# johncai117/Meta-Fine-Tuning

Measured on AMD Instinct MI355X. Metric: episodes/sec at 5-way N-shot (ResNet10+GNN) per GPU and 1/2/4/8-GPU node, higher is better.
Workload: dtype f32

## Files before the change

include/mft_hip.h:

```cpp
#ifndef MFT_HIP_H
#define MFT_HIP_H

#ifdef __cplusplus
extern "C" {
#endif

#define MFT_EINVAL (-22)

enum { MFT_ACT_NONE = 0, MFT_ACT_RELU = 1, MFT_ACT_LRELU = 2 };
enum { MFT_BN_AFFINE_FMA = 0x100 };

int mft_version(void);
int mft_device_info(int* cu_count, int* gcn_arch_is_gfx950);

int mft_stream_create_cumask(const unsigned* mask_words, int n_words, void** stream_out);
int mft_stream_create_priority(int priority, void** stream_out, int* range_out);
int mft_stream_destroy(void* stream);
int mft_stream_probe(float* w, float* m, float* v, long long n, void* stream);
int mft_event_create(void** event_out);
int mft_event_record(void* event, void* stream);
int mft_event_elapsed_ms(void* start, void* stop, float* ms_out);
int mft_event_destroy(void* event);
int mft_probe_placement(unsigned* out, int n_blocks, int spin_cycles, void* stream);

int mft_augment_views(const unsigned char* src, int n_img, int Hs, int Ws, const float* params, int n_views, float* out,
                      long long view_stride, long long img_stride, int size, const float* mean3, const float* std3,
                      void* stream);

int mft_nchw_to_nhwc(const float* src, float* dst, int n_img, int C, int H, int W, void* stream);

long long mft_conv2d_wgrad_adam_dgrad_ws_floats(int n_img, int H, int W, int Cin);
int mft_conv2d_wgrad_adam_dgrad_nhwc(const float* x, int ldx, const float* dy, int ldy, float* w, float* m, float* v,
                                     float* dx_partials, int n_img, int H, int W, int Cin, int Cout, int imgs_per_group,
                                     long long group_stride, int step, float lr, float beta1, float beta2, float eps, void* stream);
int mft_conv2d_wgrad_adam_dgrad_nhwc_dev(const float* x, int ldx, const float* dy, int ldy, float* w, float* m, float* v,
                                         float* dx_partials, int n_img, int H, int W, int Cin, int Cout, int imgs_per_group,
                                         long long group_stride, const float* hyper, float beta1, float beta2, float eps,
                                         void* stream);
int mft_col2im_bn_backward_small(const float* dx_partials, const float* x_raw, const float* relu_out, float* dx, int n_img, int H,
                                 int W, int C, int imgs_per_group, const float* mean, const float* rstd, const float* gamma,
                                 long long gb_group_stride, float* dgamma, float* dbeta, void* stream);

int mft_ce_pool_bn_backward2(const float* feat, const int* labels, int imgs_per_group, int n_groups, int C, int hw,
                             const float* out, const float* xa, const float* xb, float* dxa, float* dxb, const float* mean_a,
                             const float* rstd_a, const float* gamma_a, const float* mean_b, const float* rstd_b,
                             const float* gamma_b, long long gb_group_stride, float* dgamma_a, float* dbeta_a, float* dgamma_b,
                             float* dbeta_b, float* loss, void* stream);

int mft_stem_cache_fill(const float* in, const float* w, int w_ld, int n_img, int H, int W, float* pmax, float* pmin,
                        float* mean_img, float* m2_img, void* stream);
int mft_pool_window_minmax(const float* x, float* ymax, float* ymin, long long n_img, int H, int W, int C, void* stream);
int mft_bn_relu_pooled_gather(const float* pmax, const float* pmin, const int* src_idx, float* y, int n_img, int OH, int OW, int C,
                              int imgs_per_group, const float* mean, const float* rstd, const float* gamma, const float* beta,
                              void* stream);

int mft_bn_apply_planes(const float* x, int ldx, float* y, int ldy, unsigned short* planes, long long plane_stride, int C,
                        int rows_per_group, int n_groups, const float* mean, const float* rstd, const float* gamma,
                        const float* beta, long long gb_group_stride, const float* res, int ldr, const float* res_mean,
                        const float* res_rstd, const float* res_gamma, const float* res_beta, int act, float slope,
                        void* stream);
int mft_bn_relu_maxpool_gather_planes(const float* x, const int* src_idx, float* y, unsigned short* planes,
                                      long long plane_stride, int n_img, int H, int W, int C, int imgs_per_group,
                                      const float* mean, const float* rstd, const float* gamma, const float* beta, void* stream);
int mft_conv2d_nhwc_x3p_bnstats(const unsigned short* in_planes, long long in_plane_elems, int ldi, const unsigned short* w3,
                                long long plane_elems, float* out, int ldo, int n_img, int H, int W, int Cin, int Cout, int KH,
                                int KW, int stride, int pad, int imgs_per_group, float eps, float* stats_ws, float* mean,
                                float* rstd, void* stream);

int mft_ingest_episode_views(const float* const* views, int n_views, int double_first, int n_way, int per_class, int n_support,
                             int C, int H, int W, float* support_store, float* all_store, void* stream);
int mft_pack_oihw(const float* w_oihw, float* w_pk, int Cout, int Cin, int KH, int KW, int k_pad, void* stream);
int mft_pack_oihw_multi(const void* jobs, int n_jobs, long long total_elements, void* stream);
int mft_unpack_oihw(const float* w_pk, float* w_oihw, int Cout, int Cin, int KH, int KW, int k_pad, void* stream);
int mft_pack_dgrad(const float* w_pk, float* wt_pk, int Cout, int Cin, int KH, int KW,
                   int groups, long long w_stride, long long wt_stride, void* stream);

int mft_conv2d_nhwc(const float* in, int ldi, const float* w, const float* bias, float* out, int ldo,
                    int n_img, int H, int W, int Cin, int Cout, int KH, int KW, int stride, int pad,
                    int imgs_per_group, long long w_group_stride, void* stream);

int mft_split_bf16x3(const float* w, unsigned short* planes, long long n, void* stream);
int mft_split_bf16x3_multi(const void* jobs, int n_jobs, long long total_elements, void* stream);
int mft_conv2d_nhwc_x3(const float* in, int ldi, const unsigned short* w3, long long plane_elems, float* out, int ldo,
                       int n_img, int H, int W, int Cin, int Cout, int KH, int KW, int stride, int pad, void* stream);
long long mft_conv2d_x3_stats_ws_floats(int n_img, int H, int W, int Cout, int KH, int KW, int stride, int pad);
int mft_conv2d_nhwc_x3_bnstats(const float* in, int ldi, const unsigned short* w3, long long plane_elems, float* out, int ldo,
                               int n_img, int H, int W, int Cin, int Cout, int KH, int KW, int stride, int pad,
                               int imgs_per_group, float eps, float* stats_ws, float* mean, float* rstd, void* stream);
int mft_conv2d_nhwc_x3_bnin_bnstats(const float* in, int ldi, const float* in_ws, const float* in_gamma, const float* in_beta,
                                    const unsigned short* w3, long long plane_elems, float* out, int ldo, int n_img, int H, int W,
                                    int Cin, int Cout, int imgs_per_group, float eps, float* stats_ws, float* mean, float* rstd,
                                    void* stream);
int mft_split_f16x2(const float* w, unsigned short* planes, long long n, void* stream);
int mft_conv2d_nhwc_h2(const float* in, int ldi, const unsigned short* w2, long long plane_elems, float* out, int ldo,
                       int n_img, int H, int W, int Cin, int Cout, int KH, int KW, int stride, int pad, void* stream);
int mft_conv2d_nhwc_h2_bnstats(const float* in, int ldi, const unsigned short* w2, long long plane_elems, float* out, int ldo,
                               int n_img, int H, int W, int Cin, int Cout, int KH, int KW, int stride, int pad,
                               int imgs_per_group, float eps, float* stats_ws, float* mean, float* rstd, void* stream);
int mft_conv2d_nhwc_h2_bnin_bnstats(const float* in, int ldi, const float* in_ws, const float* in_gamma, const float* in_beta,
                                    const unsigned short* w2, long long plane_elems, float* out, int ldo, int n_img, int H, int W,
                                    int Cin, int Cout, int imgs_per_group, float eps, float* stats_ws, float* mean, float* rstd,
                                    void* stream);
int mft_bn_apply_x3ws(const float* x, int ldx, float* y, int ldy, int C, int rows_per_group, int n_groups, const float* ws,
                      const float* gamma, const float* beta, const float* res, int ldr, const float* res_ws,
                      const float* res_gamma, const float* res_beta, int act, float slope, float eps, float* mean, float* rstd,
                      float* res_mean, float* res_rstd, void* stream);
int mft_bn_running_ema(const float* mean_a, const float* rstd_a, int rows_a, const float* mean_b, const float* rstd_b, int rows_b,
                       const int* order, int n_steps, int C, float eps, float momentum, float* running_mean, float* running_var,
                       void* stream);
int mft_bn_apply_x3ws_fits(int C, int rows_per_group, int with_res_bn);
int mft_bn_relu_pooled_gather_moments(const float* pmax, const float* pmin, const int* src_idx, float* y, int n_img, int OH, int OW,
                                      int C, int imgs_per_group, const float* mean_img, const float* m2_img, int rows_per_img,
                                      float eps, const float* gamma, const float* beta, float* mean, float* rstd, void* stream);

int mft_has_experiments(void);

int mft_conv2d_dgrad_nhwc(const float* dy, int ldy, const float* w, float* dx, int ldx,
                          int n_img, int H, int W, int Cin, int Cout, int KH, int KW, int stride, int pad,
                          int imgs_per_group, long long w_group_stride, void* stream);

long long mft_conv_ksplit_ws_floats(long long rows, int cols, int K);
long long mft_conv_ksplit_grouped_ws_floats(long long rows_per_group, int cols, int K, int groups);
int mft_conv2d_nhwc_ksplit_grouped(const float* in, int ldi, const float* w, float* out, int ldo, int n_img, int H, int W, int Cin,
                                   int Cout, int KH, int KW, int stride, int pad, int imgs_per_group, long long w_group_stride,
                                   float* ws, void* stream);
int mft_conv2d_dgrad_nhwc_ksplit_grouped(const float* dy, int ldy, const float* w, float* dx, int ldx, int n_img, int H, int W, int Cin,
                                         int Cout, int KH, int KW, int stride, int pad, int imgs_per_group, long long w_group_stride,
                                         float* ws, void* stream);
int mft_conv2d_nhwc_ksplit(const float* in, int ldi, const float* w, const float* bias, float* out, int ldo, int n_img, int H, int W,
                           int Cin, int Cout, int KH, int KW, int stride, int pad, float* ws, void* stream);
int mft_conv2d_dgrad_nhwc_ksplit(const float* dy, int ldy, const float* w, float* dx, int ldx, int n_img, int H, int W, int Cin,
                                 int Cout, int KH, int KW, int stride, int pad, float* ws, void* stream);
long long mft_conv2d_wgrad_ws_floats(int n_img, int H, int W, int Cin, int Cout, int KH, int KW, int stride, int pad,
                                     int imgs_per_group);
int mft_conv2d_wgrad_nhwc(const float* in, int ldi, const float* dy, int ldy, float* dw,
                          int n_img, int H, int W, int Cin, int Cout, int KH, int KW, int stride, int pad,
                          int imgs_per_group, long long dw_group_stride, float* ws, void* stream);

long long mft_conv2d_wgrad_oihw_ws_floats(int n_img, int H, int W, int Cin, int Cout, int KH, int KW, int stride, int pad);
int mft_conv2d_wgrad_oihw(const float* in, int ldi, const float* dy, int ldy, float* dw_oihw, int n_img, int H, int W, int Cin,
                          int Cout, int KH, int KW, int stride, int pad, int cin_valid, int cout_valid, float* ws, void* stream);

typedef struct MftWgradJob {
    const float* in; const float* dy; float* dw_oihw; float* ws;
    int ldi, ldy, n_img, H, W, Cin, Cout, KH, KW, stride, pad, cin_valid, cout_valid, reserved;
} MftWgradJob;
int mft_conv2d_wgrad_oihw_multi(const MftWgradJob* jobs, int n_jobs, void* stream);

int mft_conv2d_wgrad_adam_nhwc(const float* in, int ldi, const float* dy, int ldy, float* w, float* m, float* v,
                               float* dw_or_null, int n_img, int H, int W, int Cin, int Cout, int KH, int KW,
                               int stride, int pad, int imgs_per_group, long long group_stride,
                               int step, float lr, float beta1, float beta2, float eps, void* stream);

int mft_wgrad_adam_next_forward(const float* x, int ldx, const float* dy, int ldy, float* w, float* m, float* v,
                                float* dw_or_null, int n_img, int H, int W, int Cin, int Cout, int KH, int KW, int stride,
                                int pad, int imgs_per_group, long long group_stride, int step, const float* hyper, float lr,
                                float beta1, float beta2, float eps, const float* x_next, int mode, float* raw, float* act,
                                const float* gamma, const float* beta, long long gb_group_stride, float* mean, float* rstd,
                                const float* sc_raw, const float* gamma_s, const float* beta_s, float* mean_s, float* rstd_s,
                                float* pooled, float bn_eps, void* stream);


// ... 211 lines not shown
```

meta-fine-tuning_amd/_lib.py:

```python
import ctypes
import os

PKG = os.path.dirname(os.path.abspath(__file__))
LIB_PATH = os.path.join(PKG, "libmft_hip.so")

_P = ctypes.c_void_p
_I = ctypes.c_int
_L = ctypes.c_longlong
_F = ctypes.c_float

SIGNATURES = {
    "mft_version": [],
    "mft_device_info": [_P, _P],
    "mft_stream_create_cumask": [_P, _I, _P],
    "mft_stream_destroy": [_P],
    "mft_stream_probe": [_P, _P, _P, _L, _P],
    "mft_probe_placement": [_P, _I, _I, _P],
    "mft_event_create": [_P],
    "mft_event_record": [_P, _P],
    "mft_event_elapsed_ms": [_P, _P, _P],
    "mft_event_destroy": [_P],
    "mft_augment_views": [_P, _I, _I, _I, _P, _I, _P, _L, _L, _I, _P, _P, _P],
    "mft_nchw_to_nhwc": [_P, _P, _I, _I, _I, _I, _P],
    "mft_pack_oihw": [_P, _P, _I, _I, _I, _I, _I, _P],
# ... 14 lines not shown
    "mft_conv2d_nhwc_ksplit": [_P, _I, _P, _P, _P, _I, _I, _I, _I, _I, _I, _I, _I, _I, _I, _P, _P],
    "mft_conv2d_dgrad_nhwc_ksplit": [_P, _I, _P, _P, _I, _I, _I, _I, _I, _I, _I, _I, _I, _I, _P, _P],
    "mft_conv2d_wgrad_oihw_ws_floats": [_I, _I, _I, _I, _I, _I, _I, _I, _I],
    "mft_conv2d_wgrad_oihw": [_P, _I, _P, _I, _P, _I, _I, _I, _I, _I, _I, _I, _I, _I, _I, _I, _P, _P],
    "mft_conv2d_wgrad_oihw_multi": [_P, _I, _P],
    "mft_conv2d_wgrad_ws_floats": [_I, _I, _I, _I, _I, _I, _I, _I, _I, _I],
    "mft_conv2d_wgrad_nhwc": [_P, _I, _P, _I, _P, _I, _I, _I, _I, _I, _I, _I, _I, _I, _I, _L, _P, _P],
    "mft_conv2d_wgrad_adam_nhwc": [_P, _I, _P, _I, _P, _P, _P, _P, _I, _I, _I, _I, _I, _I, _I, _I, _I, _I, _L, _I, _F, _F, _F,
                                   _F, _P],
    "mft_pair_softmax_ut_backward": [_P, _P, _P, _P, _P, _I, _I, _I, _P, _P],
    "mft_pair_bwd_stats_ws_floats": [_L, _I],
    "mft_pair_bn_act_backward": [_P, _I, _P, _I, _P, _P, _P, _P, _P, _P, _I, _L, _I, _L, _F, _P, _P, _P, _P, _P, _P],
    "mft_pair_absdiff_ut": [_P, _I, _P, _P, _I, _I, _I, _L, _L, _P],
    "mft_pair_dx_gather": [_P, _I, _P, _I, _P, _I, _I, _I, _I, _L, _L, _P],
    "mft_pack_oihw_multi": [_P, _I, _L, _P],
    "mft_wgrad_adam_next_forward": [_P, _I, _P, _I, _P, _P, _P, _P, _I, _I, _I, _I, _I, _I, _I, _I, _I, _I, _L, _I, _P, _F, _F, _F,
                                    _F, _P, _I, _P, _P, _P, _P, _L, _P, _P, _P, _P, _P, _P, _P, _P, _F, _P],
    "mft_bn_stats_ws_floats": [_I, _I, _I],
    "mft_bn_stats": [_P, _I, _I, _I, _I, _F, _P, _P, _P, _P, _P, _F, _P, _P],
    "mft_bn_apply": [_P, _I, _P, _I, _I, _I, _I, _P, _P, _P, _P, _L, _P, _I, _P, _P, _P, _P, _I, _F, _P],
    "mft_bn_apply_multi": [_P, _I, _P],
    "mft_bn_stats_multi": [_P, _I, _P],
    "mft_bn_relu_maxpool": [_P, _P, _I, _I, _I, _I, _I, _P, _P, _P, _P, _P],
    "mft_bn_relu_maxpool_gather": [_P, _P, _P, _I, _I, _I, _I, _I, _P, _P, _P, _P, _P],
    "mft_bn_image_moments": [_P, _I, _I, _I, _L, _P, _P, _P],
    "mft_bn_combine_moments": [_P, _P, _P, _I, _I, _I, _I, _F, _P, _P, _P],
    "mft_global_avgpool": [_P, _P, _I, _I, _I, _P],
    "mft_bn_small_forward": [_P, _I, _P, _I, _P, _I, _P, _I, _I, _I, _I, _P, _P, _P, _P, _L, _P, _P, _P, _P, _I, _F, _F, _P, _I, _P],
    "mft_bn_backward2": [_P, _P, _I, _P, _I, _P, _P, _I, _I, _I, _I, _P, _P, _P, _P, _P, _P, _L, _P, _P, _P, _P, _P],
    "mft_ce_pool_backward": [_P, _P, _I, _I, _I, _I, _P, _P, _P, _P],
    "mft_bn_backward": [_P, _I, _P, _I, _P, _I, _P, _I, _I, _I, _I, _P, _P, _P, _L, _P, _P, _P],
    "mft_avgpool_relu_backward": [_P, _P, _P, _I, _I, _I, _P],
    "mft_cross_entropy": [_P, _I, _P, _I, _I, _I, _P, _P, _P],
    "mft_softmax_rows": [_P, _I, _P, _I, _I, _I, _P],
    "mft_proto_scores": [_P, _I, _I, _I, _I, _I, _I, _P, _I, _P],
    "mft_proto_backward": [_P, _I, _I, _I, _I, _I, _I, _P, _I, _P, _I, _P],
    "mft_dist_linear_forward": [_P, _I, _I, _I, _P, _P, _I, _I, _F, _P, _I, _P],
    "mft_dist_linear_backward": [_P, _I, _I, _P, _P, _I, _I, _F, _P, _I, _P, _I, _P, _P, _P],
    "mft_dist_head_sgd_run": [_P, _P, _P, _I, _I, _I, _I, _I, _I, _P, _P, _F, _F, _F, _F, _F, _P],
    "mft_dist_head_step": [_P, _I, _P, _I, _I, _I, _I, _F, _P, _P, _P, _P, _P, _P, _P, _I, _P, _I, _F, _F, _F, _F, _F, _P],
    "mft_cross_entropy_mean": [_P, _I, _P, _I, _I, _I, _P, _P, _P],
    "mft_cross_entropy_mean_backward": [_P, _I, _P, _I, _I, _I, _P, _P, _I, _P],
    "mft_adam_step": [_P, _P, _P, _P, _L, _I, _F, _F, _F, _F, _F, _P],
    "mft_sgd_step": [_P, _P, _P, _L, _I, _F, _F, _F, _F, _P],
    "mft_maml_delta": [_P, _P, _P, _L, _P],
    "mft_conv2d_wgrad_adam_dgrad_ws_floats": [_I, _I, _I, _I],
    "mft_conv2d_wgrad_adam_dgrad_nhwc": [_P, _I, _P, _I, _P, _P, _P, _P, _I, _I, _I, _I, _I, _I, _L, _I, _F, _F, _F, _F, _P],
    "mft_conv2d_wgrad_adam_dgrad_nhwc_dev": [_P, _I, _P, _I, _P, _P, _P, _P, _I, _I, _I, _I, _I, _I, _L, _P, _F, _F, _F, _P],
    "mft_col2im_bn_backward_small": [_P, _P, _P, _P, _I, _I, _I, _I, _I, _P, _P, _P, _L, _P, _P, _P],
    "mft_stream_create_priority": [_I, _P, _P],
    "mft_ce_pool_bn_backward2": [_P, _P, _I, _I, _I, _I, _P, _P, _P, _P, _P, _P, _P, _P, _P, _P, _P, _L, _P, _P, _P, _P, _P, _P],
    "mft_pool_window_minmax": [_P, _P, _P, _L, _I, _I, _I, _P],
    "mft_stem_cache_fill": [_P, _P, _I, _I, _I, _I, _P, _P, _P, _P, _P],
    "mft_conv2d_nhwc_x3_bnin_bnstats": [_P, _I, _P, _P, _P, _P, _L, _P, _I, _I, _I, _I, _I, _I, _I, _F, _P, _P, _P, _P],
    "mft_split_f16x2": [_P, _P, _L, _P],
    "mft_conv2d_nhwc_h2": [_P, _I, _P, _L, _P, _I, _I, _I, _I, _I, _I, _I, _I, _I, _I, _P],
    "mft_conv2d_nhwc_h2_bnstats": [_P, _I, _P, _L, _P, _I, _I, _I, _I, _I, _I, _I, _I, _I, _I, _I, _F, _P, _P, _P, _P],
    "mft_conv2d_nhwc_h2_bnin_bnstats": [_P, _I, _P, _P, _P, _P, _L, _P, _I, _I, _I, _I, _I, _I, _I, _F, _P, _P, _P, _P],
    "mft_bn_apply_x3ws": [_P, _I, _P, _I, _I, _I, _I, _P, _P, _P, _P, _I, _P, _P, _P, _I, _F, _F, _P, _P, _P, _P, _P],
    "mft_bn_apply_x3ws_fits": [_I, _I, _I],
    "mft_bn_running_ema": [_P, _P, _I, _P, _P, _I, _P, _I, _I, _F, _F, _P, _P, _P],
    "mft_bn_relu_pooled_gather_moments": [_P, _P, _P, _P, _I, _I, _I, _I, _I, _P, _P, _I, _F, _P, _P, _P, _P, _P],
    "mft_bn_relu_pooled_gather": [_P, _P, _P, _P, _I, _I, _I, _I, _I, _P, _P, _P, _P, _P],
    "mft_bn_apply_planes": [_P, _I, _P, _I, _P, _L, _I, _I, _I, _P, _P, _P, _P, _L, _P, _I, _P, _P, _P, _P, _I, _F, _P],
    "mft_bn_relu_maxpool_gather_planes": [_P, _P, _P, _P, _L, _I, _I, _I, _I, _I, _P, _P, _P, _P, _P],
    "mft_conv2d_nhwc_x3p_bnstats": [_P, _L, _I, _P, _L, _P, _I, _I, _I, _I, _I, _I, _I, _I, _I, _I, _I, _F, _P, _P, _P, _P],
    "mft_ingest_episode_views": [_P, _I, _I, _I, _I, _I, _I, _I, _I, _P, _P, _P],
    "mft_block_entry_small_forward": [_P, _I, _P, _L, _P, _L, _P, _P, _P, _I, _I, _I, _I, _I, _I, _I, _P, _P, _L, _P, _P, _F, _P],
    "mft_block_exit_small_forward": [_P, _P, _L, _P, _P, _P, _P, _I, _I, _I, _I, _I, _P, _P, _P, _P, _L, _P, _P, _P, _P, _F, _P],
    "mft_conv2d_dgrad_bn_backward_small": [_P, _I, _P, _P, _I, _I, _I, _I, _I, _I, _I, _I, _I, _I, _L, _P, _P, _P, _P, _P, _L,
                                           _P, _P, _P],
    "mft_linear_head_sgd_run": [_P, _P, _P, _I, _I, _I, _I, _I, _I, _P, _P, _F, _F, _F, _F, _P],
    "mft_linear_head_adam_run": [_P, _P, _P, _I, _I, _I, _I, _I, _I, _P, _P, _F, _F, _F, _F, _F, _P],
    "mft_adam_multi": [_P, _I, _I, _F, _F, _F, _F, _F, _F, _P],
    "mft_adam_hyper_advance": [_P, _P, _F, _F, _F, _P],
    "mft_adam_step_dev": [_P, _P, _P, _P, _L, _P, _F, _F, _F, _F, _P],
    "mft_conv2d_wgrad_adam_nhwc_dev": [_P, _I, _P, _I, _P, _P, _P, _P, _I, _I, _I, _I, _I, _I, _I, _I, _I, _I, _L, _P, _F, _F,
                                       _F, _P],
    "mft_linear_head_step": [_P, _I, _P, _I, _I, _I, _I, _P, _P, _P, _P, _P, _P, _P, _I, _P, _I, _F, _F, _F, _F, _F, _P],
    "mft_linear_head_scores": [_P, _I, _I, _I, _I, _I, _P, _P, _P, _P],
    "mft_pair_absdiff": [_P, _I, _P, _I, _I, _I, _I, _P],
    "mft_masked_softmax": [_P, _I, _P, _I, _I, _P],
    "mft_pair_mlp_tiles_m": [_I, _I],
    "mft_pair_mlp_layer": [_P, _I, _I, _P, _P, _P, _P, _I, _I, _P, _P, _I, _I, _I, _I, _F, _P, _P, _P, _I, _P],
    "mft_bn_forward_small": [_P, _P],
    "mft_bn_forward_small_max_rows": [],
    "mft_gemm_rk": [_P, _I, _P, _I, _I, _P, _P, _I, _I, _I, _P],
    "mft_pair_mlp_tiles_m_rk": [_I, _I],
    "mft_pair_mlp_layer_rk": [_P, _I, _I, _P, _P, _P, _P, _I, _I, _P, _P, _I, _I, _I, _I, _F, _P, _P, _P, _P],
    "mft_pair_mlp_stats_finalize_rk": [_P, _P, _P, _I, _I, _I, _P, _P, _F, _P, _P, _P, _P, _P],
    "mft_pair_mlp_stats_finalize": [_P, _P, _P, _I, _I, _I, _P, _P, _F, _P, _P, _P, _P, _P],
    "mft_pair_mlp_score": [_P, _I, _P, _P, _P, _P, _F, _P, _I, _I, _I, _P],
    "mft_masked_softmax_ut": [_P, _P, _I, _I, _P],
    "mft_graph_aggregate": [_P, _P, _I, _P, _I, _I, _I, _I, _P],
    "mft_copy_cols": [_P, _I, _P, _I, _I, _I, _I, _I, _F, _P],
    "mft_build_graph_nodes": [_P, _I, _P, _I, _I, _I, _I, _I, _I, _P],
    "mft_gather_query_scores": [_P, _I, _P, _I, _I, _I, _I, _P],
    "mft_gather_rows": [_P, _P, _P, _I, _L, _P],
    "mft_var_to_rstd": [_P, _P, _I, _F, _P],
    "mft_bn_backward_ws_floats": [_I, _I, _I],
    "mft_bn_backward_act": [_P, _I, _P, _I, _P, _I, _P, _I, _I, _I, _I, _P, _P, _P, _L, _P, _P, _I, _F, _P, _P, _P, _P, _P],
    "mft_bn_backward_act_multi": [_P, _I, _P],
    "mft_act_backward": [_P, _I, _P, _I, _P, _I, _I, _L, _I, _F, _I, _P],
    "mft_colsum": [_P, _I, _I, _L, _P, _P, _P],
    "mft_bn_relu_maxpool_arg": [_P, _P, _P, _I, _I, _I, _I, _I, _P, _P, _P, _P, _P],
    "mft_maxpool_relu_backward": [_P, _P, _P, _P, _I, _I, _I, _I, _P],
# ... 120 lines not shown
```

meta-fine-tuning_amd/csrc/bn.hip:

```cpp
#include "mft_common.h"
#include "bn_fold.h"

namespace {

constexpr int ST_ROWS = 16;

__device__ __forceinline__ void bn_stats_partial_body(const float* __restrict__ x, int ldx, int C,
                                                      int rows_per_group, int rows_per_chunk, int chunks,
                                                      float* __restrict__ ws, const int bx, const int by, const int bz) {
    const int cq = threadIdx.x & 15;
    const int rl = threadIdx.x >> 4;
    const int c = by * 64 + cq * 4;
    const int g = bz;
    const int chunk = bx;
    const long long row0 = (long long)g * rows_per_group;
    __shared__ f32x4 red1[ST_ROWS][16];
    __shared__ f32x4 red2[ST_ROWS][16];
    f32x4 s1 = {0.f, 0.f, 0.f, 0.f}, s2 = {0.f, 0.f, 0.f, 0.f};
    if (c < C) {
        const f32x4 sh = *(const f32x4*)(x + row0 * ldx + c);
        const int rbeg = chunk * rows_per_chunk;
        const int rend = min(rbeg + rows_per_chunk, rows_per_group);
#pragma unroll 4
        for (int rr = rbeg + rl; rr < rend; rr += ST_ROWS) {
// ... 159 lines not shown
                const f32x4 rga = *(const f32x4*)(p.rgamma + g * p.gbs + c);
                const f32x4 rbe = *(const f32x4*)(p.rbeta + g * p.gbs + c);
                if (folded) {
                    mft_bn_fold4(rmu, rrs, rga, rbe, sc, sh);
                    rv = mft_bn_affine4(rv, sc, sh);
                } else {
                    rv = (rv - rmu) * rrs * rga + rbe;
                }
            }
            o += rv;
        }
#pragma unroll
        for (int e = 0; e < 4; ++e) o[e] = act_f(o[e], act, p.slope);
        if (!PLANES || p.y) *(f32x4*)(p.y + row * p.ldy + c) = o;
        if constexpr (PLANES) {
            mft_u32x2 p1, p2, p3;
            mft_split4_bf16(o, p1, p2, p3);
            unsigned short* q = p.planes + row * p.C + c;
            *(mft_u32x2*)(q) = p1;
            *(mft_u32x2*)(q + p.plane_stride) = p2;
            *(mft_u32x2*)(q + 2 * p.plane_stride) = p3;
        }
    }
}

template <bool PLANES>
__global__ __launch_bounds__(256) void bn_apply_kernel(ApplyArgs p) {
    bn_apply_blocks<PLANES>(p, blockIdx.x, gridDim.x);
}

constexpr int BA_MULTI = 16;
struct ApplyMultiArgs {
    ApplyArgs job[BA_MULTI];
    int start[BA_MULTI + 1];
    int n;
};
static_assert(sizeof(ApplyMultiArgs) <= 4000, "kernarg segment");

__global__ __launch_bounds__(256) void bn_apply_multi_kernel(ApplyMultiArgs a) {
    int j = 0;
#pragma unroll 1
    while (j + 1 < a.n && (int)blockIdx.x >= a.start[j + 1]) ++j;
    const ApplyArgs p = a.job[j];
    bn_apply_blocks<false>(p, blockIdx.x - a.start[j], a.start[j + 1] - a.start[j]);
}

struct ApplyWsArgs {
    const float* x; float* y; int ldx, ldy, C, rows_per_group, n_groups, M, BM;
    const float* ws; const float* gamma; const float* beta;
    const float* res; int ldr; const float* rws; const float* rgamma; const float* rbeta;
    int act; float slope, eps;
    float* mean; float* rstd; float* rmean; float* rrstd;
    int max_tiles;
};

__global__ __launch_bounds__(256) void bn_apply_ws_kernel(ApplyWsArgs p) {
    extern __shared__ __attribute__((aligned(16))) float tab[];
    const int g = blockIdx.y, C = p.C;
    char* stage = reinterpret_cast<char*>(tab + 4 * C);
    char* rstage = stage + mft_x3_stage_bytes(p.max_tiles, C);
    mft_x3_stats_stage(p.ws, C, g, p.M, p.rows_per_group, p.BM, p.max_tiles, stage, threadIdx.x, 256);
    if (p.rws) mft_x3_stats_stage(p.rws, C, g, p.M, p.rows_per_group, p.BM, p.max_tiles, rstage, threadIdx.x, 256);
    __syncthreads();
    for (int c = threadIdx.x; c < C; c += 256) {
        float mu, rs, sc, sh;
        mft_x3_stats_staged(stage, p.max_tiles, C, c, g, p.M, p.rows_per_group, p.BM, p.eps, mu, rs);
        mft_bn_fold(mu, rs, p.gamma[c], p.beta[c], sc, sh);
        tab[c] = sc; tab[C + c] = sh;
        if (blockIdx.x == 0 && p.mean) { p.mean[(long long)g * C + c] = mu; p.rstd[(long long)g * C + c] = rs; }
        if (p.rws) {
            mft_x3_stats_staged(rstage, p.max_tiles, C, c, g, p.M, p.rows_per_group, p.BM, p.eps, mu, rs);
            mft_bn_fold(mu, rs, p.rgamma[c], p.rbeta[c], sc, sh);
            tab[2 * C + c] = sc; tab[3 * C + c] = sh;
            if (blockIdx.x == 0 && p.rmean) { p.rmean[(long long)g * C + c] = mu; p.rrstd[(long long)g * C + c] = rs; }
        }
    }
    __syncthreads();
    const int cq = C >> 2;
    const int total = p.rows_per_group * cq;
    const long long row0 = (long long)g * p.rows_per_group;
    for (int i = blockIdx.x * 256 + threadIdx.x; i < total; i += gridDim.x * 256) {
        const int rr = i / cq;
        const int c = (i - rr * cq) * 4;
        const long long row = row0 + rr;
        const f32x4 v = *(const f32x4*)(p.x + row * p.ldx + c);
        f32x4 o = mft_bn_affine4(v, *(const f32x4*)(tab + c), *(const f32x4*)(tab + C + c));
        if (p.res) {
            f32x4 rv = *(const f32x4*)(p.res + row * p.ldr + c);
            if (p.rws) rv = mft_bn_affine4(rv, *(const f32x4*)(tab + 2 * C + c), *(const f32x4*)(tab + 3 * C + c));
            o += rv;
        }
#pragma unroll
        for (int e = 0; e < 4; ++e) o[e] = act_f(o[e], p.act, p.slope);
        *(f32x4*)(p.y + row * p.ldy + c) = o;
    }
}

template <bool PLANES>
__global__ __launch_bounds__(256) void bn_relu_maxpool_kernel(const float* __restrict__ x, float* __restrict__ y,
                                                              int n_img, int H, int W, int C, int OH, int OW,
                                                              int imgs_per_group, const float* __restrict__ mean,
                                                              const float* __restrict__ rstd,
                                                              const float* __restrict__ gamma,
                                                              const float* __restrict__ beta,
                                                              const int* __restrict__ src_idx,
                                                              unsigned short* __restrict__ planes, long long plane_stride) {
    const int cq = C >> 2;
    const long long total = (long long)n_img * OH * OW * cq;
    for (long long i = (long long)blockIdx.x * blockDim.x + threadIdx.x; i < total;
         i += (long long)gridDim.x * blockDim.x) {
        const int c = (int)(i % cq) * 4;
        long long t = i / cq;
        const int ow = (int)(t % OW); t /= OW;
        const int oh = (int)(t % OH);
        const int n = (int)(t / OH);
        const int g = n / imgs_per_group;
        const long long ns = src_idx ? (long long)src_idx[n] : (long long)n;
        const f32x4 mu = *(const f32x4*)(mean + (long long)g * C + c);
        const f32x4 rs = *(const f32x4*)(rstd + (long long)g * C + c);
        const f32x4 ga = *(const f32x4*)(gamma + c);
        const f32x4 be = *(const f32x4*)(beta + c);
        f32x4 best = {-3.4e38f, -3.4e38f, -3.4e38f, -3.4e38f};
#pragma unroll
        for (int dh = 0; dh < 3; ++dh) {
            const int ih = oh * 2 - 1 + dh;
            if (ih < 0 || ih >= H) continue;
#pragma unroll
            for (int dw = 0; dw < 3; ++dw) {
                const int iw = ow * 2 - 1 + dw;
                if (iw < 0 || iw >= W) continue;
                const f32x4 v = *(const f32x4*)(x + ((ns * H + ih) * W + iw) * C + c);
                const f32x4 o = __builtin_elementwise_fma((v - mu) * rs, ga, be);
#pragma unroll
                for (int e = 0; e < 4; ++e) best[e] = fmaxf(best[e], o[e]);
            }
        }
#pragma unroll
        for (int e = 0; e < 4; ++e) best[e] = fmaxf(best[e], 0.f);
        *(f32x4*)(y + i * 4) = best;
        if constexpr (PLANES) {
// ... 100 lines not shown
        f32x4 d = *(const f32x4*)(p.dy + (row0 + rr) * p.lddy + c);
        if (p.ro) {
            const f32x4 o = *(const f32x4*)(p.ro + (row0 + rr) * p.ldro + c);
#pragma unroll
            for (int e = 0; e < 4; ++e) d[e] = o[e] > 0.f ? d[e] : 0.f;
        }
        const f32x4 xh = (*(const f32x4*)(p.x + (row0 + rr) * p.ldx + c) - mu) * rs;
        *(f32x4*)(p.dx + (row0 + rr) * p.lddx + c) = k * (d - m1 - xh * m2);
    }
}

__global__ __launch_bounds__(256) void bn_image_moments_kernel(const float* __restrict__ x, int ldx, int C, int rows,
                                                               float* __restrict__ mean_img,
                                                               float* __restrict__ m2_img) {
    const int cq = threadIdx.x & 15;
    const int rl = threadIdx.x >> 4;
    const int c = blockIdx.y * 64 + cq * 4;
    const long long img = blockIdx.x;
    const long long row0 = img * rows;
    __shared__ f32x4 red1[ST_ROWS][16];
    __shared__ f32x4 red2[ST_ROWS][16];
    f32x4 s1 = {0.f, 0.f, 0.f, 0.f}, s2 = {0.f, 0.f, 0.f, 0.f}, sh = s1;
    if (c < C) {
        sh = *(const f32x4*)(x + row0 * ldx + c);
        for (int rr = rl; rr < rows; rr += ST_ROWS) {
            f32x4 v = *(const f32x4*)(x + (row0 + rr) * ldx + c);
            v -= sh;
            s1 += v;
            s2 += v * v;
        }
    }
    red1[rl][cq] = s1;
    red2[rl][cq] = s2;
    __syncthreads();
    if (rl == 0 && c < C) {
#pragma unroll
        for (int k = 1; k < ST_ROWS; ++k) {
            s1 += red1[k][cq];
            s2 += red2[k][cq];
        }
        const float inv = 1.f / (float)rows;
        f32x4 mu, m2;
#pragma unroll
        for (int e = 0; e < 4; ++e) {
            const float d = s1[e] * inv;
            mu[e] = sh[e] + d;
            m2[e] = fmaxf(s2[e] - s1[e] * d, 0.f);
        }
        *(f32x4*)(mean_img + img * C + c) = mu;
        *(f32x4*)(m2_img + img * C + c) = m2;
    }
}

template <class MeanOf, class M2Of>
__device__ __forceinline__ void combine_moments_impl(MeanOf mean_of, M2Of m2_of, int rows_per_img, int imgs_per_group, float eps,
                                                     float& mean, float& rstd) {
    float mu = 0.f;
    for (int i = 0; i < imgs_per_group; ++i) mu += mean_of(i);
    mu /= (float)imgs_per_group;
    float m2 = 0.f, dev = 0.f;
    for (int i = 0; i < imgs_per_group; ++i) {
        const float d = mean_of(i) - mu;
        m2 += m2_of(i);
        dev += d * d;
    }
    const float var = (m2 + (float)rows_per_img * dev) / ((float)rows_per_img * (float)imgs_per_group);
    mean = mu;
    rstd = 1.0f / sqrtf(var + eps);
}

__device__ __forceinline__ void combine_moments(const float* __restrict__ mean_img, const float* __restrict__ m2_img,
                                                const int* __restrict__ id, int C, int c, int rows_per_img, int imgs_per_group,
                                                float eps, float& mean, float& rstd) {
    combine_moments_impl([&](int i) { return mean_img[(long long)id[i] * C + c]; },
                         [&](int i) { return m2_img[(long long)id[i] * C + c]; }, rows_per_img, imgs_per_group, eps, mean, rstd);
}

__device__ __forceinline__ void combine_moments_lds(const float* smean, const float* sm2, int C, int c, int rows_per_img,
                                                    int imgs_per_group, float eps, float& mean, float& rstd) {
    combine_moments_impl([&](int i) { return smean[i * C + c]; }, [&](int i) { return sm2[i * C + c]; }, rows_per_img,
                         imgs_per_group, eps, mean, rstd);
}

__global__ void bn_combine_moments_kernel(const float* __restrict__ mean_img, const float* __restrict__ m2_img,
                                          const int* __restrict__ idx, int C, int rows_per_img, int imgs_per_group,
                                          float eps, float* __restrict__ mean, float* __restrict__ rstd) {
    const int c = blockIdx.x * blockDim.x + threadIdx.x;
    const int g = blockIdx.y;
    if (c >= C) return;
    float mu, rs;
    combine_moments(mean_img, m2_img, idx + (long long)g * imgs_per_group, C, c, rows_per_img, imgs_per_group, eps, mu, rs);
    mean[(long long)g * C + c] = mu;
    rstd[(long long)g * C + c] = rs;
}

inline int grid_for(long long total, int block = 256, int cap = 256 * 8) {
    long long b = (total + block - 1) / block;
    if (b < 1) b = 1;
    if (b > cap) b = cap;
    return (int)b;
}

inline int stats_chunks(int rows_per_group, int n_groups, int C) {
    const int tiles = (C + 63) / 64;
    long long want = (1024 + (long long)n_groups * tiles - 1) / ((long long)n_groups * tiles);
    int maxc = (rows_per_group + 63) / 64;
    if (want > maxc) want = maxc;
    if (want < 1) want = 1;
    return (int)want;
}

struct BnFwdSmallArgs {
    const float* x; float* y; const float* gamma; const float* beta; float* mean; float* rstd;
    float* running_mean; float* running_var; long long* nbt;
    const float* res; const float* rgamma; const float* rbeta; float* rmean; float* rrstd;
    float* rrunning_mean; float* rrunning_var; long long* rnbt;
    int ldx, ldy, ldr, C, rows_per_group, n_groups, act;
    float eps, momentum, slope;
    int y_scalar;
};

__device__ __forceinline__ void bn_small_block_sum(f32x4& a, f32x4& b, float (*red)[8]) {
    const int lane = threadIdx.x & 63, wave = threadIdx.x >> 6;
#pragma unroll
    for (int off = 32; off > 0; off >>= 1)
#pragma unroll
        for (int e = 0; e < 4; ++e) {
            a[e] += __shfl_xor(a[e], off, 64);
            b[e] += __shfl_xor(b[e], off, 64);
        }
    if (lane == 0) {
#pragma unroll
        for (int e = 0; e < 4; ++e) { red[wave][e] = a[e]; red[wave][4 + e] = b[e]; }
    }
// ... 168 lines not shown

extern "C" int mft_bn_apply(const float* x, int ldx, float* y, int ldy, int C, int rows_per_group, int n_groups,
                            const float* mean, const float* rstd, const float* gamma, const float* beta,
                            long long gb_group_stride, const float* res, int ldr, const float* res_mean,
                            const float* res_rstd, const float* res_gamma, const float* res_beta, int act, float slope,
                            void* stream) {
    if (C % 4 != 0 || ldx % 4 != 0 || ldy % 4 != 0 || (res && ldr % 4 != 0)) return MFT_EINVAL;
    ApplyArgs p{x, y, ldx, ldy, C, rows_per_group, n_groups, mean, rstd, gamma, beta, gb_group_stride,
                res, ldr, res_mean, res_rstd, res_gamma, res_beta, act, slope, nullptr, 0};
    const long long total = (long long)n_groups * rows_per_group * (C / 4);
    hipLaunchKernelGGL(bn_apply_kernel<false>, dim3(grid_for(total)), dim3(256), 0, (hipStream_t)stream, p);
    return mft_launch_status();
}

extern "C" int mft_bn_apply_multi(const MftBnApplyJob* jobs, int n_jobs, void* stream) {
    if (jobs == nullptr || n_jobs < 1) return MFT_EINVAL;
    for (int j0 = 0; j0 < n_jobs;) {
        ApplyMultiArgs a = {};
        int cnt = 0, blocks = 0;
        for (; j0 < n_jobs && cnt < BA_MULTI; ++j0, ++cnt) {
            const MftBnApplyJob& jb = jobs[j0];
            if (jb.C % 4 != 0 || jb.ldx % 4 != 0 || jb.ldy % 4 != 0 || jb.rows_per_group < 1 || jb.n_groups < 1) return MFT_EINVAL;
            a.job[cnt] = ApplyArgs{jb.x, jb.y, jb.ldx, jb.ldy, jb.C, jb.rows_per_group, jb.n_groups, jb.mean, jb.rstd, jb.gamma, jb.beta, 0,
                                   nullptr, 0, nullptr, nullptr, nullptr, nullptr, jb.act, jb.slope, nullptr, 0};
            a.start[cnt] = blocks;
            blocks += grid_for((long long)jb.n_groups * jb.rows_per_group * (jb.C / 4));
        }
        a.start[cnt] = blocks;
        a.n = cnt;
        hipLaunchKernelGGL(bn_apply_multi_kernel, dim3(blocks), dim3(256), 0, (hipStream_t)stream, a);
    }
    return mft_launch_status();
}

extern "C" int mft_bn_apply_x3ws(const float* x, int ldx, float* y, int ldy, int C, int rows_per_group, int n_groups, const float* ws,
                                 const float* gamma, const float* beta, const float* res, int ldr, const float* res_ws,
                                 const float* res_gamma, const float* res_beta, int act, float slope, float eps, float* mean,
                                 float* rstd, float* res_mean, float* res_rstd, void* stream) {
    if (C % 4 != 0 || C > 1024 || ldx % 4 != 0 || ldy % 4 != 0 || (res && ldr % 4 != 0) || !ws || !y || rows_per_group < 128 ||
        n_groups <= 0 || (res_ws && (!res || !res_gamma || !res_beta)) || (mean == nullptr) != (rstd == nullptr) ||
        (res_mean == nullptr) != (res_rstd == nullptr))
        return MFT_EINVAL;
    const long long M = (long long)n_groups * rows_per_group;
    const long long per_group = (long long)rows_per_group * (C / 4);
    if (M > 0x7fffffffLL) return MFT_EINVAL;
    const int max_tiles = mft_x3_max_group_tiles(rows_per_group, 128);
    const size_t lds = (size_t)4 * C * sizeof(float) + (res_ws ? 2 : 1) * mft_x3_stage_bytes_host(max_tiles, C);
    if (lds > 64 * 1024) return MFT_EINVAL;
    int sub = (int)((per_group + 256 * 16 - 1) / (256 * 16));
    const int cap = (2048 + n_groups - 1) / n_groups;
    if (sub > cap) sub = cap;
    if (sub < 1) sub = 1;
    ApplyWsArgs p{x, y, ldx, ldy, C, rows_per_group, n_groups, (int)M, 128, ws, gamma, beta, res, ldr, res_ws, res_gamma, res_beta,
                  act, slope, eps, mean, rstd, res_mean, res_rstd, max_tiles};
    hipLaunchKernelGGL(bn_apply_ws_kernel, dim3(sub, n_groups), dim3(256), lds, (hipStream_t)stream, p);
    return mft_launch_status();
}

namespace {
__global__ void bn_running_ema_kernel(const float* __restrict__ mean_a, const float* __restrict__ rstd_a, float unb_a,
                                      const float* __restrict__ mean_b, const float* __restrict__ rstd_b, float unb_b,
                                      const int* __restrict__ order, int n_steps, int C, float eps, float momentum,
                                      float* __restrict__ running_mean, float* __restrict__ running_var) {
    const int c = blockIdx.x * blockDim.x + threadIdx.x;
    if (c >= C) return;
    float rm = running_mean[c], rv = running_var[c];
    for (int t = 0; t < n_steps; ++t) {
        const int o = order[t], g = o & 0xffffff;
        const bool b = (o >> 24) != 0;
        const float m = (b ? mean_b : mean_a)[(long long)g * C + c];
        const float rs = (b ? rstd_b : rstd_a)[(long long)g * C + c];
        const float var = fmaxf(1.0f / (rs * rs) - eps, 0.f);
        rm = (1.f - momentum) * rm + momentum * m;
        rv = (1.f - momentum) * rv + momentum * (var * (b ? unb_b : unb_a));
    }
    running_mean[c] = rm;
    running_var[c] = rv;
}
}

extern "C" int mft_bn_running_ema(const float* mean_a, const float* rstd_a, int rows_a, const float* mean_b, const float* rstd_b,
                                  int rows_b, const int* order, int n_steps, int C, float eps, float momentum, float* running_mean,
                                  float* running_var, void* stream) {
    if (!mean_a || !rstd_a || rows_a < 1 || !order || n_steps < 1 || C < 1 || !running_mean || !running_var) return MFT_EINVAL;
    const float ua = (float)rows_a / (float)(rows_a > 1 ? rows_a - 1 : 1);
    const float ub = (float)rows_b / (float)(rows_b > 1 ? rows_b - 1 : 1);
    hipLaunchKernelGGL(bn_running_ema_kernel, dim3((C + 63) / 64), dim3(64), 0, (hipStream_t)stream, mean_a, rstd_a, ua, mean_b, rstd_b, ub,
                       order, n_steps, C, eps, momentum, running_mean, running_var);
    return mft_launch_status();
}

extern "C" int mft_bn_apply_x3ws_fits(int C, int rows_per_group, int with_res_bn) {
    if (C % 4 != 0 || C > 1024 || rows_per_group < 128) return 0;
    return (size_t)4 * C * sizeof(float) + (with_res_bn ? 2 : 1) * mft_x3_stage_bytes_host(mft_x3_max_group_tiles(rows_per_group, 128), C) <=
           64 * 1024;
}

extern "C" int mft_bn_apply_planes(const float* x, int ldx, float* y, int ldy, unsigned short* planes, long long plane_stride,
                                   int C, int rows_per_group, int n_groups, const float* mean, const float* rstd,
                                   const float* gamma, const float* beta, long long gb_group_stride, const float* res, int ldr,
                                   const float* res_mean, const float* res_rstd, const float* res_gamma,
                                   const float* res_beta, int act, float slope, void* stream) {
    if (C % 4 != 0 || ldx % 4 != 0 || (y && ldy % 4 != 0) || (res && ldr % 4 != 0) || !planes) return MFT_EINVAL;
    if (plane_stride < (long long)n_groups * rows_per_group * C) return MFT_EINVAL;
    ApplyArgs p{x, y, ldx, ldy, C, rows_per_group, n_groups, mean, rstd, gamma, beta, gb_group_stride,
                res, ldr, res_mean, res_rstd, res_gamma, res_beta, act, slope, planes, plane_stride};
    const long long total = (long long)n_groups * rows_per_group * (C / 4);
    hipLaunchKernelGGL(bn_apply_kernel<true>, dim3(grid_for(total)), dim3(256), 0, (hipStream_t)stream, p);
    return mft_launch_status();
}

namespace {
__global__ __launch_bounds__(256) void pool_window_minmax_kernel(const float* __restrict__ x, float* __restrict__ ymax,
                                                                 float* __restrict__ ymin, long long n_img, int H, int W, int C,
                                                                 int OH, int OW) {
    const int cq = C >> 2;
    const long long total = n_img * OH * OW * cq;
    for (long long i = (long long)blockIdx.x * blockDim.x + threadIdx.x; i < total; i += (long long)gridDim.x * blockDim.x) {
        const int c = (int)(i % cq) * 4;
        long long t = i / cq;
        const int ow = (int)(t % OW); t /= OW;
        const int oh = (int)(t % OH);
        const long long n = t / OH;
        f32x4 hi = {-3.4e38f, -3.4e38f, -3.4e38f, -3.4e38f}, lo = {3.4e38f, 3.4e38f, 3.4e38f, 3.4e38f};
#pragma unroll
        for (int dh = 0; dh < 3; ++dh) {
            const int ih = oh * 2 - 1 + dh;
            if (ih < 0 || ih >= H) continue;
#pragma unroll
            for (int dw = 0; dw < 3; ++dw) {
                const int iw = ow * 2 - 1 + dw;
                if (iw < 0 || iw >= W) continue;
                const f32x4 v = *(const f32x4*)(x + ((n * H + ih) * W + iw) * C + c);
#pragma unroll
                for (int e = 0; e < 4; ++e) { hi[e] = fmaxf(hi[e], v[e]); lo[e] = fminf(lo[e], v[e]); }
            }
        }
        *(f32x4*)(ymax + i * 4) = hi;
        *(f32x4*)(ymin + i * 4) = lo;
    }
}

__device__ __forceinline__ f32x4 pooled_bn_relu(const float* __restrict__ pmax, const float* __restrict__ pmin, long long src,
                                                const f32x4 mu, const f32x4 rs, const f32x4 ga, const f32x4 be) {
    const bool all_pos = ga[0] >= 0.f && ga[1] >= 0.f && ga[2] >= 0.f && ga[3] >= 0.f;
    const bool all_neg = ga[0] < 0.f && ga[1] < 0.f && ga[2] < 0.f && ga[3] < 0.f;
    f32x4 v;
    if (all_pos) v = *(const f32x4*)(pmax + src);
    else if (all_neg) v = *(const f32x4*)(pmin + src);
    else {
        const f32x4 a = *(const f32x4*)(pmax + src), b = *(const f32x4*)(pmin + src);
#pragma unroll
        for (int e = 0; e < 4; ++e) v[e] = ga[e] >= 0.f ? a[e] : b[e];
    }
    f32x4 o = __builtin_elementwise_fma((v - mu) * rs, ga, be);
#pragma unroll
    for (int e = 0; e < 4; ++e) o[e] = fmaxf(o[e], 0.f);
    return o;
}

__global__ __launch_bounds__(256) void bn_relu_pooled_gather_kernel(const float* __restrict__ pmax, const float* __restrict__ pmin,
                                                                    const int* __restrict__ src_idx, float* __restrict__ y,
                                                                    int n_img, int HW, int C, int imgs_per_group,
                                                                    const float* __restrict__ mean, const float* __restrict__ rstd,
                                                                    const float* __restrict__ gamma, const float* __restrict__ beta) {
    const int cq = C >> 2;
    const long long total = (long long)n_img * HW * cq;
    for (long long i = (long long)blockIdx.x * blockDim.x + threadIdx.x; i < total; i += (long long)gridDim.x * blockDim.x) {
        const int c = (int)(i % cq) * 4;
        const long long t = i / cq;
        const int pix = (int)(t % HW);
        const int n = (int)(t / HW);
        const int g = n / imgs_per_group;
        const long long src = ((long long)src_idx[n] * HW + pix) * C + c;
        const f32x4 mu = *(const f32x4*)(mean + (long long)g * C + c);
        const f32x4 rs = *(const f32x4*)(rstd + (long long)g * C + c);
        *(f32x4*)(y + i * 4) = pooled_bn_relu(pmax, pmin, src, mu, rs, *(const f32x4*)(gamma + c), *(const f32x4*)(beta + c));
    }
}

__global__ __launch_bounds__(256) void bn_relu_pooled_gather_moments_kernel(
    const float* __restrict__ pmax, const float* __restrict__ pmin, const int* __restrict__ src_idx, float* __restrict__ y, int HW,
    int C, int imgs_per_group, const float* __restrict__ mean_img, const float* __restrict__ m2_img, int rows_per_img, float eps,
    const float* __restrict__ gamma, const float* __restrict__ beta, float* __restrict__ mean, float* __restrict__ rstd) {
    extern __shared__ __attribute__((aligned(16))) float tab[];
    const int g = blockIdx.y;
    const int* id = src_idx + (long long)g * imgs_per_group;
    float* smean = tab + 2 * C;
    float* sm2 = smean + imgs_per_group * C;
    for (int i = threadIdx.x; i < imgs_per_group * C; i += 256) {
        const int im = i / C, c = i - im * C;
        const long long src = (long long)id[im] * C + c;
        smean[i] = mean_img[src];
        sm2[i] = m2_img[src];
    }
    __syncthreads();
    for (int c = threadIdx.x; c < C; c += 256) {
        float mu, rs;
        combine_moments_lds(smean, sm2, C, c, rows_per_img, imgs_per_group, eps, mu, rs);
        tab[c] = mu; tab[C + c] = rs;
        if (blockIdx.x == 0 && mean) { mean[(long long)g * C + c] = mu; rstd[(long long)g * C + c] = rs; }
    }
    __syncthreads();
    const int cq = C >> 2;
    const int total = imgs_per_group * HW * cq;
    for (int i = blockIdx.x * 256 + threadIdx.x; i < total; i += gridDim.x * 256) {
        const int c = (i % cq) * 4;
        const int t = i / cq;
        const int pix = t % HW;
        const int n = t / HW;
        const long long src = ((long long)id[n] * HW + pix) * C + c;
        const long long dst = ((long long)g * imgs_per_group * HW * cq + i) * 4;
        *(f32x4*)(y + dst) = pooled_bn_relu(pmax, pmin, src, *(const f32x4*)(tab + c), *(const f32x4*)(tab + C + c),
                                            *(const f32x4*)(gamma + c), *(const f32x4*)(beta + c));
    }
}
}

extern "C" int mft_pool_window_minmax(const float* x, float* ymax, float* ymin, long long n_img, int H, int W, int C, void* stream) {
    if (C % 4 != 0 || n_img <= 0) return MFT_EINVAL;
    const int OH = (H + 2 - 3) / 2 + 1, OW = (W + 2 - 3) / 2 + 1;
    const long long total = n_img * OH * OW * (C / 4);
    hipLaunchKernelGGL(pool_window_minmax_kernel, dim3(grid_for(total, 256, 256 * 16)), dim3(256), 0, (hipStream_t)stream, x, ymax,
                       ymin, n_img, H, W, C, OH, OW);
    return mft_launch_status();
}

extern "C" int mft_bn_relu_pooled_gather(const float* pmax, const float* pmin, const int* src_idx, float* y, int n_img, int OH,
                                         int OW, int C, int imgs_per_group, const float* mean, const float* rstd,
                                         const float* gamma, const float* beta, void* stream) {
    if (C % 4 != 0 || !src_idx) return MFT_EINVAL;
    if (imgs_per_group <= 0) imgs_per_group = n_img;
    const long long total = (long long)n_img * OH * OW * (C / 4);
    hipLaunchKernelGGL(bn_relu_pooled_gather_kernel, dim3(grid_for(total, 256, 256 * 16)), dim3(256), 0, (hipStream_t)stream, pmax,
                       pmin, src_idx, y, n_img, OH * OW, C, imgs_per_group, mean, rstd, gamma, beta);
    return mft_launch_status();
}

extern "C" int mft_bn_relu_pooled_gather_moments(const float* pmax, const float* pmin, const int* src_idx, float* y, int n_img,
                                                 int OH, int OW, int C, int imgs_per_group, const float* mean_img,
                                                 const float* m2_img, int rows_per_img, float eps, const float* gamma,
                                                 const float* beta, float* mean, float* rstd, void* stream) {
    if (C % 4 != 0 || C > 1024 || !src_idx || imgs_per_group <= 0 || n_img % imgs_per_group != 0 || rows_per_img <= 0 ||
        (mean == nullptr) != (rstd == nullptr))
        return MFT_EINVAL;
    const int groups = n_img / imgs_per_group;
    const long long per_group = (long long)imgs_per_group * OH * OW * (C / 4);
    if (per_group > 0x7fffffffLL) return MFT_EINVAL;
    int sub = (int)((per_group + 256 * 16 - 1) / (256 * 16));
    const int cap = (2048 + groups - 1) / groups;
    if (sub > cap) sub = cap;
    if (sub < 1) sub = 1;
    const size_t lds = (size_t)(2 + 2 * imgs_per_group) * C * sizeof(float);
    if (lds > 64 * 1024) return MFT_EINVAL;
    hipLaunchKernelGGL(bn_relu_pooled_gather_moments_kernel, dim3(sub, groups), dim3(256), lds, (hipStream_t)stream,
                       pmax, pmin, src_idx, y, OH * OW, C, imgs_per_group, mean_img, m2_img, rows_per_img, eps, gamma, beta, mean,
                       rstd);
    return mft_launch_status();
}

extern "C" int mft_bn_relu_maxpool_gather_planes(const float* x, const int* src_idx, float* y, unsigned short* planes,
                                                 long long plane_stride, int n_img, int H, int W, int C, int imgs_per_group,
                                                 const float* mean, const float* rstd, const float* gamma, const float* beta,
                                                 void* stream) {
    if (C % 4 != 0) return MFT_EINVAL;
    if (imgs_per_group <= 0) imgs_per_group = n_img;
    const int OH = (H + 2 - 3) / 2 + 1, OW = (W + 2 - 3) / 2 + 1;
    const long long total = (long long)n_img * OH * OW * (C / 4);
    if (planes)
        hipLaunchKernelGGL(bn_relu_maxpool_kernel<true>, dim3(grid_for(total, 256, 256 * 16)), dim3(256), 0, (hipStream_t)stream,
                           x, y, n_img, H, W, C, OH, OW, imgs_per_group, mean, rstd, gamma, beta, src_idx, planes, plane_stride);
    else
        hipLaunchKernelGGL(bn_relu_maxpool_kernel<false>, dim3(grid_for(total, 256, 256 * 16)), dim3(256), 0, (hipStream_t)stream,
                           x, y, n_img, H, W, C, OH, OW, imgs_per_group, mean, rstd, gamma, beta, src_idx, planes, plane_stride);
    return mft_launch_status();
}

// ... 352 lines not shown
```

meta-fine-tuning_amd/csrc/bn_fold.h:

```cpp
#pragma once
#include "mft_common.h"

typedef float mft_f32x2 __attribute__((ext_vector_type(2)));

struct MftTileSpan { int t0, t1; };
struct MftTileW { float inv_nt, w1, w2, pad; };

__device__ __forceinline__ MftTileSpan mft_x3_group_tiles(int g, int M, int R, int BM) {
    const int r0 = g * R, r1 = min(r0 + R, M);
    return {r0 / BM, (r1 - 1) / BM};
}

__device__ __forceinline__ int mft_x3_tile_seg(int t, int g, int R, int BM) { return ((t * BM) / R == g) ? 0 : 1; }

__device__ __forceinline__ MftTileW mft_x3_tile_weights(int t, int g, int M, int R, int BM) {
    const int r0 = g * R, r1 = min(r0 + R, M);
    const int lo = max(t * BM, r0), hi = min(t * BM + BM, r1);
    const float nt = (float)(hi - lo), n = (float)(lo - r0), tot = (float)(hi - r0);
    return {1.0f / nt, nt / tot, n * nt / tot, 0.f};
}

template <class Get, class Weights>
__device__ __forceinline__ void mft_x3_stats_chain(Get get, Weights weights, int g, int M, int R, int BM, float eps, float& mean,
                                                   float& rstd) {
// ... 13 lines not shown
    rstd = 1.0f / sqrtf(m2 / (float)(r1 - r0) + eps);
}

__device__ __forceinline__ void mft_x3_stats_merge(const float* __restrict__ ws, int C, int c, int g, int M, int R, int BM,
                                                   float eps, float& mean, float& rstd) {
    mft_x3_stats_chain([&](int t, int seg) { return *(const mft_f32x2*)(ws + (((long long)t * 2 + seg) * C + c) * 2); },
                       [&](int t) { return mft_x3_tile_weights(t, g, M, R, BM); }, g, M, R, BM, eps, mean, rstd);
}

__device__ __forceinline__ size_t mft_x3_stage_bytes(int max_tiles, int C) {
    return (size_t)max_tiles * (sizeof(MftTileW) + (size_t)C * sizeof(mft_f32x2));
}

__device__ __forceinline__ void mft_x3_stats_stage(const float* __restrict__ ws, int C, int g, int M, int R, int BM, int max_tiles,
                                                   void* stage, int tid, int nthreads) {
    MftTileW* wt = reinterpret_cast<MftTileW*>(stage);
    mft_f32x2* part = reinterpret_cast<mft_f32x2*>(wt + max_tiles);
    const MftTileSpan sp = mft_x3_group_tiles(g, M, R, BM);
    const int nt = sp.t1 - sp.t0 + 1;
    for (int i = tid; i < nt; i += nthreads) wt[i] = mft_x3_tile_weights(sp.t0 + i, g, M, R, BM);
    const int total = nt * C;
    for (int i = tid; i < total; i += nthreads) {
        const int tt = i / C, c = i - tt * C, t = sp.t0 + tt;
        part[i] = *(const mft_f32x2*)(ws + (((long long)t * 2 + mft_x3_tile_seg(t, g, R, BM)) * C + c) * 2);
    }
}

__device__ __forceinline__ void mft_x3_stats_staged(const void* stage, int max_tiles, int C, int c, int g, int M, int R, int BM,
                                                    float eps, float& mean, float& rstd) {
    const MftTileW* wt = reinterpret_cast<const MftTileW*>(stage);
    const mft_f32x2* part = reinterpret_cast<const mft_f32x2*>(wt + max_tiles);
    const int t0 = mft_x3_group_tiles(g, M, R, BM).t0;
    mft_x3_stats_chain([&](int t, int) { return part[(t - t0) * C + c]; }, [&](int t) { return wt[t - t0]; }, g, M, R, BM, eps, mean,
                       rstd);
}

inline int mft_x3_max_group_tiles(int R, int BM) { return (R + BM - 1) / BM + 1; }
inline size_t mft_x3_stage_bytes_host(int max_tiles, int C) { return (size_t)max_tiles * (16 + (size_t)C * 8); }

__device__ __forceinline__ void mft_bn_fold(float mean, float rstd, float gamma, float beta, float& scale, float& shift) {
    scale = rstd * gamma;
    shift = __builtin_fmaf(-mean, scale, beta);
}

__device__ __forceinline__ f32x4 mft_bn_affine4(const f32x4 v, const f32x4 scale, const f32x4 shift) {
    return __builtin_elementwise_fma(v, scale, shift);
}

__device__ __forceinline__ void mft_bn_fold4(const f32x4 mean, const f32x4 rstd, const f32x4 gamma, const f32x4 beta, f32x4& scale,
                                             f32x4& shift) {
    scale = rstd * gamma;
    shift = __builtin_elementwise_fma(-mean, scale, beta);
}
```

meta-fine-tuning_amd/csrc/conv_x3.hip:

```cpp
#include "mft_common.h"
#include "bn_fold.h"

namespace {

typedef __bf16 bf16x8 __attribute__((ext_vector_type(8)));
typedef __bf16 bf16x2 __attribute__((ext_vector_type(2)));
typedef _Float16 f16x8 __attribute__((ext_vector_type(8)));
typedef _Float16 f16x4 __attribute__((ext_vector_type(4)));
typedef float f32x2 __attribute__((ext_vector_type(2)));
typedef unsigned u32x2 __attribute__((ext_vector_type(2)));
typedef unsigned u32x4 __attribute__((ext_vector_type(4)));

struct X3Args {
    const float* in;
    const unsigned short* w3;
    long long plane;
    float* out;
    int ldi, ldo;
    int H, W, Cin, OH, OW, Cout, KH, KW, stride, pad;
    int Kpad;
    int M;
    int tiles_n;
    unsigned in_bytes, w_bytes;
    int xcd_swizzle;
    int row_swz;
    const unsigned short* in3;
    unsigned in_plane_bytes;
    float* stats_ws;
    int rows_per_group;
    int s1_rows;
    const float* bn_ws; const float* bn_gamma; const float* bn_beta;
    float bn_eps;
    int bn_max_tiles;
};

constexpr int X3_RS = 40;

__device__ __forceinline__ unsigned pk_bf16(float a, float b) {
    f32x2 v = {a, b};
    return __builtin_bit_cast(unsigned, __builtin_convertvector(v, bf16x2));
}

__device__ __forceinline__ void split4(const f32x4 x, u32x2& p1, u32x2& p2, u32x2& p3) {
    f32x4 r;
    p1[0] = pk_bf16(x[0], x[1]);
    p1[1] = pk_bf16(x[2], x[3]);
    r[0] = x[0] - __builtin_bit_cast(float, p1[0] << 16);
    r[1] = x[1] - __builtin_bit_cast(float, p1[0] & 0xffff0000u);
    r[2] = x[2] - __builtin_bit_cast(float, p1[1] << 16);
    r[3] = x[3] - __builtin_bit_cast(float, p1[1] & 0xffff0000u);
    p2[0] = pk_bf16(r[0], r[1]);
    p2[1] = pk_bf16(r[2], r[3]);
    r[0] -= __builtin_bit_cast(float, p2[0] << 16);
    r[1] -= __builtin_bit_cast(float, p2[0] & 0xffff0000u);
    r[2] -= __builtin_bit_cast(float, p2[1] << 16);
    r[3] -= __builtin_bit_cast(float, p2[1] & 0xffff0000u);
    p3[0] = pk_bf16(r[0], r[1]);
    p3[1] = pk_bf16(r[2], r[3]);
}

__device__ __forceinline__ void split4_h2(const f32x4 x, u32x2& p1, u32x2& p2) {
    const f16x4 hi = __builtin_convertvector(x, f16x4);
    const f32x4 r = (x - __builtin_convertvector(hi, f32x4)) * 2048.f;
    const f16x4 lo = __builtin_convertvector(r, f16x4);
    p1 = __builtin_bit_cast(u32x2, hi);
    p2 = __builtin_bit_cast(u32x2, lo);
}
constexpr float X3_H2_LO_SCALE = 1.0f / 2048.f;

template <int BM, int BN, bool AP, bool DB, int HOIST = 0, int DBG = 0, bool XS = false, int NP = 3>
__global__ __launch_bounds__(256) __attribute__((amdgpu_waves_per_eu(NP == 2 ? 3 : 1))) void conv_x3_kernel(X3Args p) {
    static_assert(NP == 3 || (NP == 2 && !AP && !DB && HOIST == 0 && DBG == 0 && !XS), "f16x2: the plain single-buffer form only");
    constexpr int NACC = NP == 3 ? 1 : 2;
    constexpr int TM = BM / 64;
    constexpr int TN = BN / 64;
    constexpr int PA = AP ? BM / 64 : BM / 32;
    constexpr int PB = BN / 64;
    constexpr int RS = XS ? 32 : X3_RS;
    constexpr int A_PLANE = BM * RS;
    constexpr int B_PLANE = BN * RS;
    auto lo = [](int row, int c) -> int {
        if constexpr (XS) return row * 32 + ((((c >> 3) ^ (row >> 2)) & 3) << 3) + (c & 7);
        else return row * X3_RS + c;
    };
    extern __shared__ __attribute__((aligned(16))) unsigned short smem[];
    unsigned short* As = smem;
// ... 295 lines not shown
#pragma unroll
            for (int e = 0; e < 16; ++e) {
                const int row = (e & 3) + 8 * (e >> 2) + 4 * h;
                const int m = m0 + wm * (BM / 2) + i * 32 + row;
                if (m < p.M) p.out[(long long)m * p.ldo + n] = val(i, j, e);
            }
        }
    if (p.stats_ws != nullptr) {
        static_assert(TN == 1 || TN == 2, "stats epilogue");
        const int split = (m0 / p.rows_per_group + 1) * p.rows_per_group;
        float* sred = reinterpret_cast<float*>(smem);
        __syncthreads();
#pragma unroll
        for (int j = 0; j < TN; ++j) {
            float a1 = 0.f, a2 = 0.f, b1 = 0.f, b2 = 0.f;
#pragma unroll
            for (int i = 0; i < TM; ++i)
#pragma unroll
                for (int e = 0; e < 16; ++e) {
                    const int m = m0 + wm * (BM / 2) + i * 32 + (e & 3) + 8 * (e >> 2) + 4 * h;
                    const float v = val(i, j, e);
                    if (m < p.M) {
                        if (m < split) { a1 += v; a2 += v * v; }
                        else { b1 += v; b2 += v * v; }
                    }
                }
            a1 += __shfl_xor(a1, 32, 64); a2 += __shfl_xor(a2, 32, 64);
            b1 += __shfl_xor(b1, 32, 64); b2 += __shfl_xor(b2, 32, 64);
            if (h == 0) {
                float* o = sred + ((((wm * 2 + wn) * TN + j) * 32 + r) << 2);
                o[0] = a1; o[1] = a2; o[2] = b1; o[3] = b2;
            }
        }
        __syncthreads();
        if (wm == 0 && h == 0) {
#pragma unroll
            for (int j = 0; j < TN; ++j) {
                const float* o0 = sred + ((((0 * 2 + wn) * TN + j) * 32 + r) << 2);
                const float* o1 = sred + ((((1 * 2 + wn) * TN + j) * 32 + r) << 2);
                const int n = n0 + wn * (BN / 2) + j * 32 + r;
                float* w0 = p.stats_ws + (((long long)mt * 2 + 0) * p.Cout + n) * 2;
                float* w1 = p.stats_ws + (((long long)mt * 2 + 1) * p.Cout + n) * 2;
                w0[0] = o0[0] + o1[0]; w0[1] = o0[1] + o1[1];
                w1[0] = o0[2] + o1[2]; w1[1] = o0[3] + o1[3];
            }
        }
    }
}

#ifdef MFT_EXPERIMENTS
#include "../../tools/experiments/conv_x3_pingpong.inc"
#endif

template <int BM, int BN, bool BNIN, int NP = 3, bool BDB = true>
__device__ __forceinline__ void conv_x3_s1_body(const X3Args& p) {
    static_assert(NP == 3 || NP == 2, "3 bf16 pieces (six products) or 2 fp16 pieces (three products)");
    constexpr int NACC = NP == 3 ? 1 : 2;
    constexpr int TM = BM / 64, TN = BN / 64;
    constexpr int PA = BM / 32, PB = BN / 64;
    constexpr int RS = X3_RS;
    constexpr int B_PLANE = BN * RS;
    const int A_PLANE = p.s1_rows * RS;
    extern __shared__ __attribute__((aligned(16))) unsigned short smem[];
    constexpr int NBB = (NP == 2 && BDB) ? 2 : 1;
    unsigned short* As = smem;
    unsigned short* Bs = smem + NP * A_PLANE;
    float* bn_tab = reinterpret_cast<float*>(Bs + NBB * NP * B_PLANE);

    const int tid = threadIdx.x;
    const int lane = tid & 63, wave = tid >> 6;
    const int wm = wave >> 1, wn = wave & 1;
    const int r = lane & 31, h = lane >> 5;
    int tile_id = blockIdx.x;
    if (p.xcd_swizzle) {
        const int nwg = gridDim.x, q = nwg >> 3, rmd = nwg & 7;
        const int xcd = tile_id & 7, slot = tile_id >> 3;
        tile_id = xcd * q + (xcd < rmd ? xcd : rmd) + slot;
    }
    const int nt = tile_id % p.tiles_n;
    const int mt = tile_id / p.tiles_n;
    const int m0 = mt * BM, n0 = nt * BN;
    const int W = p.W, H = p.H;
    const int fr0 = m0 / W;
    const int g0 = BNIN ? m0 / p.rows_per_group : 0;
    const bool bn_two = BNIN && (m0 + (BM < p.M - m0 ? BM : p.M - m0) - 1) / p.rows_per_group > g0;
    if constexpr (BNIN) {
        char* stage = reinterpret_cast<char*>(smem);
        const size_t gstride = mft_x3_stage_bytes(p.bn_max_tiles, p.Cin);
        const bool two = bn_two;
        mft_x3_stats_stage(p.bn_ws, p.Cin, g0, p.M, p.rows_per_group, BM, p.bn_max_tiles, stage, tid, 256);
        if (two) mft_x3_stats_stage(p.bn_ws, p.Cin, g0 + 1, p.M, p.rows_per_group, BM, p.bn_max_tiles, stage + gstride, tid, 256);
        __syncthreads();
        for (int i = tid; i < 2 * p.Cin; i += 256) {
            const int gi = i >= p.Cin ? 1 : 0, c = i - gi * p.Cin;
            if (gi == 0 || two) {
                float mu, rs, sc, sh;
                mft_x3_stats_staged(stage + gi * gstride, p.bn_max_tiles, p.Cin, c, g0 + gi, p.M, p.rows_per_group, BM, p.bn_eps, mu, rs);
                mft_bn_fold(mu, rs, p.bn_gamma[c], p.bn_beta[c], sc, sh);
                bn_tab[(gi * 2 + 0) * p.Cin + c] = sc;
                bn_tab[(gi * 2 + 1) * p.Cin + c] = sh;
            }
        }
        __syncthreads();
    }
    const int g_id = tid >> 5, g_rr = (tid >> 3) & 3;
    const int lrow = p.row_swz ? g_rr * 4 + (g_id & 3) + 16 * (g_id >> 2) : tid >> 3;
    const int c4 = (tid & 7) * 4;
    const __amdgpu_buffer_rsrc_t rA = __builtin_amdgcn_make_buffer_rsrc((void*)p.in, 0, p.in_bytes, 0x00020000);
    const __amdgpu_buffer_rsrc_t rB = __builtin_amdgcn_make_buffer_rsrc((void*)p.w3, 0, p.w_bytes, 0x00020000);
    int a_off[PA], a_oh[PA], a_lds[PA], a_tab[PA];
    bool a_ok[PA];
#pragma unroll
    for (int j = 0; j < PA; ++j) {
        const int t = lrow + 32 * j, m = m0 + t;
        const int fr = m / W;
        a_ok[j] = m < p.M;
        a_oh[j] = fr - (fr / H) * H;
        a_off[j] = ((a_ok[j] ? m : 0) * p.ldi + c4) * 4;
        a_lds[j] = (t + 1) * RS + c4;
        a_tab[j] = BNIN ? ((a_ok[j] ? m / p.rows_per_group - g0 : 0) * 2 * p.Cin + c4) : 0;
    }
    const int hside = (tid >> 3) & 1;
    const int mh = hside ? m0 + BM : m0 - 1;
    const int frh = (mh > 0 ? mh : 0) / W;
    const bool h_ok = tid < 16 && (hside ? (mh < p.M && mh - frh * W != 0) : (m0 > 0 && m0 - fr0 * W != 0));
    const int h_oh = frh - (frh / H) * H;
    const int h_off = ((h_ok ? mh : 0) * p.ldi + c4) * 4;
    const int h_lds = (hside ? BM + 1 : 0) * RS + c4;
    const int h_tab = BNIN ? (((hside && h_ok) ? (m0 + BM - 1) / p.rows_per_group - g0 : 0) * 2 * p.Cin + c4) : 0;

    const int bseg = tid & 3;
    const int brow = p.row_swz ? ((tid >> 2) & 3) * 4 + ((tid >> 4) & 3) + 16 * (tid >> 6) : tid >> 2;
    int b_off[PB];
#pragma unroll
    for (int j = 0; j < PB; ++j) b_off[j] = ((n0 + brow + 64 * j) * p.Kpad + bseg * 8) * 2;
    const int plane_bytes = (int)(p.plane * 2);

    int fa[TM], fl[TM], fr_[TM];
    constexpr int Z0 = BM + 2;
#pragma unroll
    for (int i = 0; i < TM; ++i) {
        const int t = wm * (BM / 2) + i * 32 + r;
        const int ow = (m0 + t) - ((m0 + t) / W) * W;
        fa[i] = (t + 1) * RS;
        fl[i] = ow == 0 ? (Z0 + ((t - Z0) & 15)) * RS : fa[i] - RS;
        fr_[i] = ow == W - 1 ? (Z0 + ((t + 2 - Z0) & 15)) * RS : fa[i] + RS;
    }

    f32x16 acc[NACC][TM][TN];
#pragma unroll
    for (int q = 0; q < NACC; ++q)
#pragma unroll
        for (int i = 0; i < TM; ++i)
#pragma unroll
            for (int j = 0; j < TN; ++j)
#pragma unroll
                for (int e = 0; e < 16; ++e) acc[q][i][j][e] = 0.f;
    auto val = [&](int i, int j, int e) -> float {
        if constexpr (NP == 3) return acc[0][i][j][e];
        else return __builtin_fmaf(acc[1][i][j][e], X3_H2_LO_SCALE, acc[0][i][j][e]);
    };

    struct Stage {
        f32x4 ra[PA];
        f32x4 rh;
        u32x4 rb[PB][NP];
    };
    Stage st;
    const int n_ci = p.Cin / 32;
    const int n_ms = 3 * n_ci;
    auto load_a = [&](int ms, Stage& S) {
        const int kh = ms / n_ci, ci0 = (ms - kh * n_ci) * 32;
        const int shift = ((kh - 1) * W * p.ldi + ci0) * 4;
#pragma unroll
        for (int j = 0; j < PA; ++j) {
            const bool ok = a_ok[j] && (unsigned)(a_oh[j] + kh - 1) < (unsigned)H;
            S.ra[j] = __builtin_bit_cast(f32x4, __builtin_amdgcn_raw_buffer_load_b128(rA, ok ? (unsigned)(a_off[j] + shift) : 0x80000000u, 0, 0));
        }
        const bool okh = h_ok && (unsigned)(h_oh + kh - 1) < (unsigned)H;
        S.rh = __builtin_bit_cast(f32x4, __builtin_amdgcn_raw_buffer_load_b128(rA, okh ? (unsigned)(h_off + shift) : 0x80000000u, 0, 0));
    };
    auto load_b = [&](int ms, int kw, Stage& S) {
        const int kh = ms / n_ci, ci0 = (ms - kh * n_ci) * 32;
        const int k0 = (kh * 3 + kw) * p.Cin + ci0;
#pragma unroll
        for (int j = 0; j < PB; ++j)
#pragma unroll
            for (int pl = 0; pl < NP; ++pl)
                S.rb[j][pl] = __builtin_amdgcn_raw_buffer_load_b128(rB, b_off[j] + pl * plane_bytes, k0 * 2, 0);
    };
    auto put_a = [&](const f32x4 v, int off) {
        if constexpr (NP == 3) {
            u32x2 p1, p2, p3;
            split4(v, p1, p2, p3);
            *(u32x2*)(As + off) = p1;
            *(u32x2*)(As + A_PLANE + off) = p2;
            *(u32x2*)(As + 2 * A_PLANE + off) = p3;
        } else {
            u32x2 p1, p2;
            split4_h2(v, p1, p2);
            *(u32x2*)(As + off) = p1;
            *(u32x2*)(As + A_PLANE + off) = p2;
        }
    };
    auto bn_relu = [&](const f32x4 v, const f32x4 sc, const f32x4 sh, bool ok) {
        f32x4 o = mft_bn_affine4(v, sc, sh);
#pragma unroll
        for (int e = 0; e < 4; ++e) o[e] = ok ? fmaxf(o[e], 0.f) : 0.f;
        return o;
    };
    auto store_a = [&](const Stage& S, int ms) {
        if constexpr (BNIN) {
            const int kh = ms / n_ci, ci0 = (ms - kh * n_ci) * 32;
            const bool okh = h_ok && (unsigned)(h_oh + kh - 1) < (unsigned)H;
            if (!bn_two) {
                const f32x4 sc = *(const f32x4*)(bn_tab + ci0 + c4), sh = *(const f32x4*)(bn_tab + p.Cin + ci0 + c4);
#pragma unroll
                for (int j = 0; j < PA; ++j)
                    put_a(bn_relu(S.ra[j], sc, sh, a_ok[j] && (unsigned)(a_oh[j] + kh - 1) < (unsigned)H), a_lds[j]);
                if (tid < 16) put_a(bn_relu(S.rh, sc, sh, okh), h_lds);
            } else {
#pragma unroll
                for (int j = 0; j < PA; ++j)
                    put_a(bn_relu(S.ra[j], *(const f32x4*)(bn_tab + a_tab[j] + ci0), *(const f32x4*)(bn_tab + a_tab[j] + p.Cin + ci0),
                                  a_ok[j] && (unsigned)(a_oh[j] + kh - 1) < (unsigned)H), a_lds[j]);
                if (tid < 16)
                    put_a(bn_relu(S.rh, *(const f32x4*)(bn_tab + h_tab + ci0), *(const f32x4*)(bn_tab + h_tab + p.Cin + ci0), okh), h_lds);
            }
        } else {
#pragma unroll
            for (int j = 0; j < PA; ++j) put_a(S.ra[j], a_lds[j]);
            if (tid < 16) put_a(S.rh, h_lds);
        }
    };
    auto store_b = [&](const Stage& S, int bb = 0) {
#pragma unroll
        for (int j = 0; j < PB; ++j)
#pragma unroll
            for (int pl = 0; pl < NP; ++pl)
                *(u32x4*)(Bs + (bb * NP + pl) * B_PLANE + (brow + 64 * j) * RS + bseg * 8) = S.rb[j][pl];
    };
    auto compute = [&](int kw, int bb = 0) {
        const unsigned short* const Bc = Bs + bb * NP * B_PLANE;
#pragma unroll
        for (int kk = 0; kk < 2; ++kk) {
            if constexpr (NP == 3) {
                bf16x8 a[TM][3], b[TN][3];
#pragma unroll
                for (int i = 0; i < TM; ++i)
#pragma unroll
                    for (int pl = 0; pl < 3; ++pl)
                        a[i][pl] = *(const bf16x8*)(As + pl * A_PLANE + (kw == 0 ? fl[i] : (kw == 1 ? fa[i] : fr_[i])) + kk * 16 + h * 8);
#pragma unroll
                for (int j = 0; j < TN; ++j)
#pragma unroll
                    for (int pl = 0; pl < 3; ++pl)
                        b[j][pl] = *(const bf16x8*)(Bc + pl * B_PLANE + (wn * (BN / 2) + j * 32 + r) * RS + kk * 16 + h * 8);
                constexpr int TA[6] = {2, 0, 1, 1, 0, 0};
                constexpr int TB[6] = {0, 2, 1, 0, 1, 0};
#pragma unroll
                for (int t = 0; t < 6; ++t)
#pragma unroll
                    for (int i = 0; i < TM; ++i)
#pragma unroll
                        for (int j = 0; j < TN; ++j)
// ... 89 lines not shown
        }
    if (p.stats_ws != nullptr) {
        static_assert(TN == 1 || TN == 2, "stats epilogue");
        const int split = (m0 / p.rows_per_group + 1) * p.rows_per_group;
        float* sred = reinterpret_cast<float*>(smem);
        __syncthreads();
#pragma unroll
        for (int j = 0; j < TN; ++j) {
            float a1 = 0.f, a2 = 0.f, b1 = 0.f, b2 = 0.f;
#pragma unroll
            for (int i = 0; i < TM; ++i)
#pragma unroll
                for (int e = 0; e < 16; ++e) {
                    const int m = m0 + wm * (BM / 2) + i * 32 + (e & 3) + 8 * (e >> 2) + 4 * h;
                    const float v = val(i, j, e);
                    if (m < p.M) {
                        if (m < split) { a1 += v; a2 += v * v; }
                        else { b1 += v; b2 += v * v; }
                    }
                }
            a1 += __shfl_xor(a1, 32, 64); a2 += __shfl_xor(a2, 32, 64);
            b1 += __shfl_xor(b1, 32, 64); b2 += __shfl_xor(b2, 32, 64);
            if (h == 0) {
                float* o = sred + ((((wm * 2 + wn) * TN + j) * 32 + r) << 2);
                o[0] = a1; o[1] = a2; o[2] = b1; o[3] = b2;
            }
        }
        __syncthreads();
        if (wm == 0 && h == 0) {
#pragma unroll
            for (int j = 0; j < TN; ++j) {
                const float* o0 = sred + ((((0 * 2 + wn) * TN + j) * 32 + r) << 2);
                const float* o1 = sred + ((((1 * 2 + wn) * TN + j) * 32 + r) << 2);
                const int n = n0 + wn * (BN / 2) + j * 32 + r;
                float* w0 = p.stats_ws + (((long long)mt * 2 + 0) * p.Cout + n) * 2;
                float* w1 = p.stats_ws + (((long long)mt * 2 + 1) * p.Cout + n) * 2;
                w0[0] = o0[0] + o1[0]; w0[1] = o0[1] + o1[1];
                w1[0] = o0[2] + o1[2]; w1[1] = o0[3] + o1[3];
            }
        }
    }
}

template <int BM, int BN, int NP = 3, bool BDB = true>
__global__ __launch_bounds__(256) __attribute__((amdgpu_waves_per_eu(NP == 2 ? 3 : 1))) void conv_x3_s1_kernel(X3Args p) {
    conv_x3_s1_body<BM, BN, false, NP, BDB>(p);
}

template <int BM, int BN, int NP = 3, bool BDB = true>
__global__ __launch_bounds__(256) __attribute__((amdgpu_waves_per_eu(3, 3))) void conv_x3_s1_bnin_kernel(X3Args p) {
    conv_x3_s1_body<BM, BN, true, NP, BDB>(p);
}

__global__ void x3_stats_finalize_kernel(const float* __restrict__ ws, int C, int M, int R, int BM, float eps,
                                         float* __restrict__ mean, float* __restrict__ rstd) {
    const int c = blockIdx.x * blockDim.x + threadIdx.x;
    const int g = blockIdx.y;
    if (c >= C) return;
    float mu, rs;
    mft_x3_stats_merge(ws, C, c, g, M, R, BM, eps, mu, rs);
    mean[(long long)g * C + c] = mu;
    rstd[(long long)g * C + c] = rs;
}

__global__ __launch_bounds__(256) void split_bf16x3_kernel(const float* __restrict__ w, unsigned short* __restrict__ out,
                                                           long long n) {
    for (long long i = (long long)blockIdx.x * blockDim.x + threadIdx.x; i < n; i += (long long)gridDim.x * blockDim.x) {
        const float x = w[i];
        const unsigned q1 = pk_bf16(x, 0.f) & 0xffffu;
        const float r1 = x - __builtin_bit_cast(float, q1 << 16);
        const unsigned q2 = pk_bf16(r1, 0.f) & 0xffffu;
        const float r2 = r1 - __builtin_bit_cast(float, q2 << 16);
        const unsigned q3 = pk_bf16(r2, 0.f) & 0xffffu;
        out[i] = (unsigned short)q1;
        out[n + i] = (unsigned short)q2;
        out[2 * n + i] = (unsigned short)q3;
    }
}

struct SplitJob { const float* src; unsigned short* dst; long long n, Cout, Cin, taps, transposed, start; };

__global__ __launch_bounds__(256) void split_bf16x3_multi_kernel(const SplitJob* __restrict__ jobs, int n_jobs, long long total) {
    for (long long i = (long long)blockIdx.x * blockDim.x + threadIdx.x; i < total; i += (long long)gridDim.x * blockDim.x) {
        int lo = 0, hi = n_jobs - 1;
        while (lo < hi) {
            const int mid = (lo + hi + 1) >> 1;
            if (jobs[mid].start <= i) lo = mid; else hi = mid - 1;
        }
        const SplitJob j = jobs[lo];
        const long long l = i - j.start;
        long long src = l;
        if (j.transposed) {
            const long long co = l % j.Cout, t = l / j.Cout;
            const long long tp = t % j.taps, ci = t / j.taps;
            src = (co * j.taps + (j.taps - 1 - tp)) * j.Cin + ci;
        }
        const float x = j.src[src];
        const unsigned q1 = pk_bf16(x, 0.f) & 0xffffu;
        const float r1 = x - __builtin_bit_cast(float, q1 << 16);
        const unsigned q2 = pk_bf16(r1, 0.f) & 0xffffu;
        const float r2 = r1 - __builtin_bit_cast(float, q2 << 16);
        const unsigned q3 = pk_bf16(r2, 0.f) & 0xffffu;
        j.dst[l] = (unsigned short)q1;
        j.dst[j.n + l] = (unsigned short)q2;
        j.dst[2 * j.n + l] = (unsigned short)q3;
    }
// ... 137 lines not shown
int g_x3_patch = 0;
int g_x3_tile = 0;

}

extern "C" int mft_split_bf16x3(const float* w, unsigned short* planes, long long n, void* stream) {
    if (n <= 0) return MFT_EINVAL;
    long long blocks = (n + 255) / 256;
    if (blocks > 4096) blocks = 4096;
    hipLaunchKernelGGL(split_bf16x3_kernel, dim3((unsigned)blocks), dim3(256), 0, (hipStream_t)stream, w, planes, n);
    return mft_launch_status();
}

extern "C" int mft_split_bf16x3_multi(const void* jobs, int n_jobs, long long total_elements, void* stream) {
    if (n_jobs < 1 || total_elements < 1) return MFT_EINVAL;
    long long blocks = (total_elements + 255) / 256;
    if (blocks > 4096) blocks = 4096;
    hipLaunchKernelGGL(split_bf16x3_multi_kernel, dim3((unsigned)blocks), dim3(256), 0, (hipStream_t)stream, (const SplitJob*)jobs, n_jobs,
                       total_elements);
    return mft_launch_status();
}

extern "C" int mft_debug_set_x3_tile(int t) {
#ifndef MFT_EXPERIMENTS
    const bool off = (t == 10 || t == 60 || t == 70 || t == 80 || t == 100 || t == 200);
    if (!off && ((t >= 10 && t < 20) || t == 42 || (t >= 60 && t < 90) || t >= 100)) return MFT_EINVAL;
#endif
    if (t >= 200) g_x3_dbg = t - 200;
    else if (t >= 100) g_x3_min_lds_kb = t - 100;
    else if (t >= 90) g_x3_s1 = t - 90;
    else if (t >= 80) g_x3_hoist = t - 80;
    else if (t >= 70) g_x3_pp = t - 70;
    else if (t >= 60) g_x3_db = t - 60;
    else if (t >= 40) g_x3_row_swz = t - 40;
    else if (t >= 30) g_x3_bdb = t - 30;
    else if (t >= 20) g_x3_xcd = t - 20;
    else if (t >= 10) g_x3_patch = t - 10;
    else g_x3_tile = t;
    return 0;
}

static int x3_dispatch(const float* in, int ldi, const unsigned short* w3, long long plane_elems, float* out, int ldo,
                       int n_img, int H, int W, int Cin, int Cout, int KH, int KW, int stride, int pad, float* stats_ws,
                       int rows_per_group, void* stream, const unsigned short* in3 = nullptr, long long in_plane_elems = 0,
                       const float* bn_ws = nullptr, const float* bn_gamma = nullptr, const float* bn_beta = nullptr,
                       float bn_eps = 0.f, int np = 3) {
    if (n_img <= 0 || Cin % 32 != 0 || Cout % 64 != 0 || ldi % 4 != 0 || (np != 3 && np != 2)) return MFT_EINVAL;
    if (np == 2 && (in3 != nullptr || g_x3_tile > 1 || g_x3_db || g_x3_pp || g_x3_dbg || g_x3_hoist || g_x3_row_swz == 2 || g_x3_min_lds_kb ||
                    g_x3_patch))
        return MFT_EINVAL;
    X3Args p;
    p.bn_ws = bn_ws; p.bn_gamma = bn_gamma; p.bn_beta = bn_beta; p.bn_eps = bn_eps;
    p.bn_max_tiles = bn_ws ? mft_x3_max_group_tiles(rows_per_group, 128) : 0;
    if (bn_ws != nullptr && (in3 != nullptr || !bn_gamma || !bn_beta || rows_per_group < 128 || KH != 3 || KW != 3 || stride != 1 ||
                             pad != 1 || x3_s1_lds(128, 64, W, Cin, np) > X3_S1_LDS_3PER_CU ||
                             2 * mft_x3_stage_bytes_host(p.bn_max_tiles, Cin) >
                                 (size_t)np * (128 + 18) * X3_RS * sizeof(unsigned short)))
        return MFT_EINVAL;
    p.in3 = in3;
    p.in_plane_bytes = 0;
    p.stats_ws = stats_ws;
    p.rows_per_group = rows_per_group;
    p.in = in; p.w3 = w3; p.plane = plane_elems; p.out = out; p.ldi = ldi; p.ldo = ldo;
    p.H = H; p.W = W; p.Cin = Cin; p.Cout = Cout; p.KH = KH; p.KW = KW; p.stride = stride; p.pad = pad;
    p.OH = (H + 2 * pad - KH) / stride + 1;
    p.OW = (W + 2 * pad - KW) / stride + 1;
    p.Kpad = KH * KW * Cin;
    const long long M = (long long)n_img * p.OH * p.OW;
    if (M > 0x7fffffffLL) return MFT_EINVAL;
    p.M = (int)M;
    p.tiles_n = 0;
    hipStream_t s = (hipStream_t)stream;
    int G = 0, R = 0;
    double eff = 0.0;
    if (in3 != nullptr) {
        const long long need = (long long)n_img * H * W * ldi;
        if (ldi % 8 != 0 || in_plane_elems < need || 3 * in_plane_elems * 2 >= 0x7fff0000LL || 3 * plane_elems * 2 >= 0x7fff0000LL)
            return MFT_EINVAL;
        if (stats_ws != nullptr && rows_per_group < 128) return MFT_EINVAL;
        p.in_plane_bytes = (unsigned)(in_plane_elems * 2);
        p.in_bytes = 0;
        p.w_bytes = (unsigned)(3 * plane_elems * 2);
        return launch_x3<128, 64, true, false>(p, (hipStream_t)stream);
    }
#ifdef MFT_EXPERIMENTS
    if (stats_ws == nullptr && g_x3_patch && KH == 3 && KW == 3 && stride == 1 && pad == 1 && ldi == Cin && ldo == Cout &&
        patch_geometry(H, W, &G, &R, &eff) && (g_x3_patch >= 2 || eff >= 0.9)) {
        P3Args q;
        q.in = in; q.w3 = w3; q.plane = plane_elems; q.out = out;
        q.n_img = n_img; q.H = H; q.W = W; q.Cin = Cin; q.Cout = Cout; q.G = G; q.R = R;
        q.row_blocks = (H + R - 1) / R;
        q.tiles_n = Cout / 64;
        const int img_groups = (n_img + G - 1) / G;
        const size_t lds = (size_t)3 * G * (R + 2) * (W + 2) * X3_RS * sizeof(unsigned short);
        static MftPerDeviceOnce attr_once;
        if (attr_once.need()) {
            hipError_t e = hipFuncSetAttribute((const void*)conv3x3_patch_x3_kernel, hipFuncAttributeMaxDynamicSharedMemorySize,
                                               64 * 1024);
            if (e != hipSuccess) return (int)e;
            attr_once.mark();
        }
        if (lds <= 64 * 1024) {
            hipLaunchKernelGGL(conv3x3_patch_x3_kernel, dim3((unsigned)(img_groups * q.row_blocks * q.tiles_n)), dim3(256), lds, s, q);
            return mft_launch_status();
        }
    }
// ... 75 lines not shown
    hipLaunchKernelGGL(x3_stats_finalize_kernel, dim3((Cout + 63) / 64, groups), dim3(64), 0, (hipStream_t)stream,
                       (const float*)stats_ws, Cout, n_img * OH * OW, R, g_x3_tile == 3 ? 64 : 128, eps, mean, rstd);
    return mft_launch_status();
}

extern "C" int mft_conv2d_nhwc_x3_bnstats(const float* in, int ldi, const unsigned short* w3, long long plane_elems,
                                          float* out, int ldo, int n_img, int H, int W, int Cin, int Cout, int KH, int KW,
                                          int stride, int pad, int imgs_per_group, float eps, float* stats_ws,
                                          float* mean, float* rstd, void* stream) {
    return x3_bnstats(3, in, ldi, w3, plane_elems, out, ldo, n_img, H, W, Cin, Cout, KH, KW, stride, pad, imgs_per_group, eps, stats_ws, mean,
                      rstd, stream);
}

extern "C" int mft_conv2d_nhwc_h2_bnstats(const float* in, int ldi, const unsigned short* w2, long long plane_elems,
                                          float* out, int ldo, int n_img, int H, int W, int Cin, int Cout, int KH, int KW,
                                          int stride, int pad, int imgs_per_group, float eps, float* stats_ws,
                                          float* mean, float* rstd, void* stream) {
    return x3_bnstats(2, in, ldi, w2, plane_elems, out, ldo, n_img, H, W, Cin, Cout, KH, KW, stride, pad, imgs_per_group, eps, stats_ws, mean,
                      rstd, stream);
}

static int x3_bnin_bnstats(int np, const float* in, int ldi, const float* in_ws, const float* in_gamma,
                           const float* in_beta, const unsigned short* w3, long long plane_elems, float* out,
                           int ldo, int n_img, int H, int W, int Cin, int Cout, int imgs_per_group, float eps,
                           float* stats_ws, float* mean, float* rstd, void* stream) {
    if (imgs_per_group <= 0 || n_img % imgs_per_group != 0 || stats_ws == nullptr || in_ws == nullptr ||
        (mean == nullptr) != (rstd == nullptr) || g_x3_tile == 3)
        return MFT_EINVAL;
    const int R = imgs_per_group * H * W;
    const int rc = x3_dispatch(in, ldi, w3, plane_elems, out, ldo, n_img, H, W, Cin, Cout, 3, 3, 1, 1, stats_ws, R, stream, nullptr, 0,
                               in_ws, in_gamma, in_beta, eps, np);
    if (rc != 0 || mean == nullptr) return rc;
    hipLaunchKernelGGL(x3_stats_finalize_kernel, dim3((Cout + 63) / 64, n_img / imgs_per_group), dim3(64), 0, (hipStream_t)stream,
                       (const float*)stats_ws, Cout, n_img * H * W, R, 128, eps, mean, rstd);
    return mft_launch_status();
}

extern "C" int mft_conv2d_nhwc_x3_bnin_bnstats(const float* in, int ldi, const float* in_ws, const float* in_gamma,
                                               const float* in_beta, const unsigned short* w3, long long plane_elems, float* out,
                                               int ldo, int n_img, int H, int W, int Cin, int Cout, int imgs_per_group, float eps,
                                               float* stats_ws, float* mean, float* rstd, void* stream) {
    return x3_bnin_bnstats(3, in, ldi, in_ws, in_gamma, in_beta, w3, plane_elems, out, ldo, n_img, H, W, Cin, Cout, imgs_per_group, eps,
                           stats_ws, mean, rstd, stream);
}

extern "C" int mft_conv2d_nhwc_h2_bnin_bnstats(const float* in, int ldi, const float* in_ws, const float* in_gamma,
                                               const float* in_beta, const unsigned short* w2, long long plane_elems, float* out,
                                               int ldo, int n_img, int H, int W, int Cin, int Cout, int imgs_per_group, float eps,
                                               float* stats_ws, float* mean, float* rstd, void* stream) {
    return x3_bnin_bnstats(2, in, ldi, in_ws, in_gamma, in_beta, w2, plane_elems, out, ldo, n_img, H, W, Cin, Cout, imgs_per_group, eps,
                           stats_ws, mean, rstd, stream);
}

extern "C" int mft_conv2d_nhwc_x3p_bnstats(const unsigned short* in_planes, long long in_plane_elems, int ldi,
                                           const unsigned short* w3, long long plane_elems, float* out, int ldo, int n_img,
                                           int H, int W, int Cin, int Cout, int KH, int KW, int stride, int pad,
                                           int imgs_per_group, float eps, float* stats_ws, float* mean, float* rstd,
                                           void* stream) {
    if (imgs_per_group <= 0 || n_img % imgs_per_group != 0 || stats_ws == nullptr || in_planes == nullptr) return MFT_EINVAL;
    const int OH = (H + 2 * pad - KH) / stride + 1, OW = (W + 2 * pad - KW) / stride + 1;
    const int R = imgs_per_group * OH * OW;
    const int rc = x3_dispatch(nullptr, ldi, w3, plane_elems, out, ldo, n_img, H, W, Cin, Cout, KH, KW, stride, pad, stats_ws, R,
                               stream, in_planes, in_plane_elems);
    if (rc != 0) return rc;
    const int groups = n_img / imgs_per_group;
    hipLaunchKernelGGL(x3_stats_finalize_kernel, dim3((Cout + 63) / 64, groups), dim3(64), 0, (hipStream_t)stream,
                       (const float*)stats_ws, Cout, n_img * OH * OW, R, 128, eps, mean, rstd);
    return mft_launch_status();
}
```

meta-fine-tuning_amd/csrc/stem.hip:

```cpp
#include "mft_common.h"

namespace {

template <int W_>
__global__ __launch_bounds__(256) void stem_conv_kernel(const float* __restrict__ in, const float* __restrict__ w_pk,
                                                        float* __restrict__ out, int H, int w_ld, int tiles_per_img,
                                                        int total_tiles) {
    constexpr int OW = W_ / 2;
    constexpr int PL = (W_ + 8) * 3;
    constexpr int SPAN = (127 + OW - 1) / OW;
    constexpr int PR = 2 * SPAN + 7;
    constexpr int PQ = PR * PL / 4;
    constexpr int NLD = (PQ + 255) / 256;
    constexpr int ROWQ = PL / 4;
    static_assert(PL % 4 == 0, "patch rows must be float4 multiples");
    extern __shared__ __attribute__((aligned(16))) float smem[];

    const int tid = threadIdx.x;
    const int lane = tid & 63, wave = tid >> 6;
    const int wm = wave >> 1, wn = wave & 1;
    const int r = lane & 31, h = lane >> 5;
    const int OH = H / 2;
    const int OHW = OH * OW;

    float breg[77];
    {
        const float* wrow = w_pk + (long long)(wn * 32 + r) * w_ld;
#pragma unroll
        for (int kh = 0; kh < 7; ++kh)
#pragma unroll
            for (int p = 0; p < 11; ++p) {
                const int j = 2 * p + h;
                breg[kh * 11 + p] = (j < 21) ? wrow[kh * 21 + j] : 0.f;
            }
    }

    f32x4 pre[NLD];
    auto load_patch = [&](int tile) {
        const int img = tile / tiles_per_img;
        const int mt = tile - img * tiles_per_img;
        const int oh0 = (mt * 128) / OW;
        const int ih0 = 2 * oh0 - 3;
        const float* src = in + (long long)img * H * W_ * 3;
#pragma unroll
        for (int i = 0; i < NLD; ++i) {
            const int q = tid + i * 256;
            f32x4 v = {0.f, 0.f, 0.f, 0.f};
            if (q < PQ) {
                const int pr = q / ROWQ;
                const int cf = (q - pr * ROWQ) * 4 - 12;
                const int ih = ih0 + pr;
                if (ih >= 0 && ih < H && cf >= 0 && cf < W_ * 3) v = *(const f32x4*)(src + (long long)ih * W_ * 3 + cf);
            }
// ... 38 lines not shown
#pragma unroll
        for (int kh = 0; kh < 7; ++kh)
#pragma unroll
            for (int p = 0; p < 11; ++p) {
                const float a0 = P[mb[0] + kh * PL + 2 * p];
                const float a1 = P[mb[1] + kh * PL + 2 * p];
                acc0 = __builtin_amdgcn_mfma_f32_32x32x2f32(a0, breg[kh * 11 + p], acc0, 0, 0, 0);
                acc1 = __builtin_amdgcn_mfma_f32_32x32x2f32(a1, breg[kh * 11 + p], acc1, 0, 0, 0);
            }
        float* obase = out + ((long long)img * OHW) * 64 + wn * 32 + r;
        const int m00 = mt * 128 + wm * 64;
#pragma unroll
        for (int e = 0; e < 16; ++e) {
            const int row = (e & 3) + 8 * (e >> 2) + 4 * h;
            const int m0 = m00 + row, m1 = m00 + 32 + row;
            if (m0 < OHW) obase[(long long)m0 * 64] = acc0[e];
            if (m1 < OHW) obase[(long long)m1 * 64] = acc1[e];
        }
        (void)mrow;
        if (next < total_tiles) store_patch(buf ^ 1);
        __syncthreads();
        buf ^= 1;
    }
}

template <int W_>
int launch_stem(const float* in, const float* w, float* out, int n_img, int H, int w_ld, hipStream_t s) {
    constexpr int OW = W_ / 2;
    constexpr int PL = (W_ + 8) * 3;
    constexpr int SPAN = (127 + OW - 1) / OW;
    constexpr int PR = 2 * SPAN + 7;
    const int OHW = (H / 2) * OW;
    const int tpi = (OHW + 127) / 128;
    const long long total = (long long)n_img * tpi;
    if (total > 0x7fffffffLL) return MFT_EINVAL;
    const size_t lds = 2ull * PR * PL * sizeof(float);
    auto kern = stem_conv_kernel<W_>;
    if (lds > 64 * 1024) {
        static bool attr_done = false;
        if (!attr_done) {
            hipError_t e = hipFuncSetAttribute((const void*)kern, hipFuncAttributeMaxDynamicSharedMemorySize, (int)lds);
            if (e != hipSuccess) return (int)e;
            attr_done = true;
        }
    }
    const int wg_per_cu = 2;
    long long grid = 256LL * wg_per_cu;
    if (grid > total) grid = total;
    hipLaunchKernelGGL(kern, dim3((unsigned)grid), dim3(256), lds, s, in, w, out, H, w_ld, tpi, (int)total);
    return mft_launch_status();
}


template <int W_>
__global__ __launch_bounds__(256) __attribute__((amdgpu_waves_per_eu(2, 2))) void stem_cache_kernel(const float* __restrict__ in, const float* __restrict__ w_pk,
                                                         float* __restrict__ pmax, float* __restrict__ pmin,
                                                         float* __restrict__ mean_img, float* __restrict__ m2_img, int w_ld,
                                                         int n_img) {
    constexpr int H_ = W_;
    constexpr int OW = W_ / 2, OH = H_ / 2;
    constexpr int PH = (OH + 2 - 3) / 2 + 1, PW = (OW + 2 - 3) / 2 + 1;
    constexpr int TR = 3, TILES = OH / TR, TPX = TR * OW;
    static_assert(OH % TR == 0 && TPX <= 128, "tiles of three whole output rows");
    constexpr int PL = (W_ + 8) * 3;
    constexpr int PR = 2 * TR + 5;
    constexpr int PQ = PR * PL / 4;
    constexpr int NLD = (PQ + 255) / 256;
    constexpr int ROWQ = PL / 4;
    constexpr int SROW = OW * 64;
    static_assert(PL % 4 == 0 && 2 * 256 * 4 <= PR * PL, "patch rows are float4 multiples; the moment scratch fits a patch buffer");
    extern __shared__ __attribute__((aligned(16))) float smem[];
    float* const S = smem + 2 * PR * PL;

    const int tid = threadIdx.x;
    const int lane = tid & 63, wave = tid >> 6;
    const int wm = wave >> 1, wn = wave & 1;
    const int r = lane & 31, h = lane >> 5;
    const int cq = tid & 15, rl = tid >> 4;

    float breg[77];
    {
        const float* wrow = w_pk + (long long)(wn * 32 + r) * w_ld;
#pragma unroll
        for (int kh = 0; kh < 7; ++kh)
#pragma unroll
            for (int p = 0; p < 11; ++p) {
                const int j = 2 * p + h;
                breg[kh * 11 + p] = (j < 21) ? wrow[kh * 21 + j] : 0.f;
            }
    }
    f32x4 pre[NLD];
    auto load_patch = [&](long long img, int t) {
        const int ih0 = 2 * TR * t - 3;
        const float* src = in + img * H_ * W_ * 3;
#pragma unroll
        for (int i = 0; i < NLD; ++i) {
            const int q = tid + i * 256;
            f32x4 v = {0.f, 0.f, 0.f, 0.f};
            if (q < PQ) {
                const int pr = q / ROWQ;
                const int cf = (q - pr * ROWQ) * 4 - 12;
                const int ih = ih0 + pr;
                if (ih >= 0 && ih < H_ && cf >= 0 && cf < W_ * 3) v = *(const f32x4*)(src + (long long)ih * W_ * 3 + cf);
            }
            pre[i] = v;
        }
    };
    auto store_patch = [&](int buf) {
        float* P = smem + buf * (PR * PL);
#pragma unroll
        for (int i = 0; i < NLD; ++i) {
// ... 27 lines not shown
            if (more) load_patch(nimg, last_t ? 0 : t + 1);
            const float* P = smem + buf * (PR * PL);
            f32x16 acc0, acc1;
#pragma unroll
            for (int e = 0; e < 16; ++e) { acc0[e] = 0.f; acc1[e] = 0.f; }
#pragma unroll
            for (int kh = 0; kh < 7; ++kh)
#pragma unroll
                for (int p = 0; p < 11; ++p) {
                    const float a0 = P[mb[0] + kh * PL + 2 * p];
                    const float a1 = P[mb[1] + kh * PL + 2 * p];
                    acc0 = __builtin_amdgcn_mfma_f32_32x32x2f32(a0, breg[kh * 11 + p], acc0, 0, 0, 0);
                    acc1 = __builtin_amdgcn_mfma_f32_32x32x2f32(a1, breg[kh * 11 + p], acc1, 0, 0, 0);
                }
            __syncthreads();
            const int row0 = TR * t;
            const int sl0 = row0 % 5, sl1 = (row0 + 1) % 5, sl2 = (row0 + 2) % 5;
#pragma unroll
            for (int e = 0; e < 16; ++e) {
#pragma unroll
                for (int i = 0; i < 2; ++i) {
                    const int mo = mo_base + i * 32 + (e & 3) + 8 * (e >> 2);
                    if (mo < TPX) {
                        const int ol = (mo >= OW) + (mo >= 2 * OW);
                        const int slot = ol == 0 ? sl0 : (ol == 1 ? sl1 : sl2);
                        S[slot * SROW + (mo - ol * OW) * 64 + ch] = i == 0 ? acc0[e] : acc1[e];
                    }
                }
            }
            if (more) store_patch(buf ^ 1);
            __syncthreads();
            const int i_first = t == 0 ? 0 : (TR * t - 2) / 2 + 1;
            int i_last = (TR * t + 1) / 2;
            if (i_last > PH - 1 || last_t) i_last = PH - 1;
            const int n_items = (i_last - i_first + 1) * PW * 16;
            for (int it = tid; it < n_items; it += 256) {
                const int c4 = (it & 15) * 4;
                const int j = (it >> 4) % PW, i = i_first + (it >> 4) / PW;
                f32x4 hi = {-3.4e38f, -3.4e38f, -3.4e38f, -3.4e38f}, lo = {3.4e38f, 3.4e38f, 3.4e38f, 3.4e38f};
#pragma unroll
                for (int dh = 0; dh < 3; ++dh) {
                    const int ih = 2 * i - 1 + dh;
                    if (ih < 0 || ih >= OH) continue;
#pragma unroll
                    for (int dw = 0; dw < 3; ++dw) {
                        const int iw = 2 * j - 1 + dw;
                        if (iw < 0 || iw >= OW) continue;
                        const f32x4 v = *(const f32x4*)(S + (ih % 5) * SROW + iw * 64 + c4);
#pragma unroll
                        for (int e = 0; e < 4; ++e) { hi[e] = fmaxf(hi[e], v[e]); lo[e] = fminf(lo[e], v[e]); }
                    }
                }
                const long long o = ((img * PH + i) * PW + j) * 64 + c4;
                *(f32x4*)(pmax + o) = hi;
                *(f32x4*)(pmin + o) = lo;
            }
            if (t == 0) sh = *(const f32x4*)(S + cq * 4);
            const int p0 = TPX * t;
            for (int pp = p0 + ((rl - p0) & 15); pp < p0 + TPX; pp += 16) {
                const int orow = pp / OW, ow = pp - orow * OW;
                f32x4 v = *(const f32x4*)(S + (orow % 5) * SROW + ow * 64 + cq * 4);
                v -= sh;
                s1 += v;
                s2 += v * v;
            }
            buf ^= 1;
        }
        f32x4* red = (f32x4*)(smem + (buf ^ 1) * (PR * PL));
        red[rl * 16 + cq] = s1;
        red[256 + rl * 16 + cq] = s2;
        __syncthreads();
        if (rl == 0) {
#pragma unroll
            for (int k = 1; k < 16; ++k) {
                s1 += red[k * 16 + cq];
                s2 += red[256 + k * 16 + cq];
            }
            const float inv = 1.f / (float)(OH * OW);
            f32x4 mu, m2;
#pragma unroll
            for (int e = 0; e < 4; ++e) {
                const float d = s1[e] * inv;
                mu[e] = sh[e] + d;
                m2[e] = fmaxf(s2[e] - s1[e] * d, 0.f);
            }
            *(f32x4*)(mean_img + img * 64 + cq * 4) = mu;
            *(f32x4*)(m2_img + img * 64 + cq * 4) = m2;
        }
    }
}

}

int mft_stem_conv_dispatch(const float* in, const float* w, float* out, int n_img, int H, int W, int w_ld,
                           hipStream_t s) {
    if (H % 2 != 0 || H < 8) return MFT_EINVAL;
    if (W == 84) return launch_stem<84>(in, w, out, n_img, H, w_ld, s);
    if (W == 224) return launch_stem<224>(in, w, out, n_img, H, w_ld, s);
    return MFT_EINVAL;
}

extern "C" int mft_stem_cache_fill(const float* in, const float* w, int w_ld, int n_img, int H, int W, float* pmax, float* pmin,
                                   float* mean_img, float* m2_img, void* stream) {
    if (H != 84 || W != 84 || n_img <= 0 || w_ld < 147) return MFT_EINVAL;
    constexpr int W_ = 84, PL = (W_ + 8) * 3, PR = 11, SROW = (W_ / 2) * 64;
    const size_t lds = (2ull * PR * PL + 5ull * SROW) * sizeof(float);
    auto kern = stem_cache_kernel<W_>;
    static MftPerDeviceOnce attr_once;
    if (attr_once.need()) {
        hipError_t e = hipFuncSetAttribute((const void*)kern, hipFuncAttributeMaxDynamicSharedMemorySize, (int)lds);
        if (e != hipSuccess) return (int)e;
        attr_once.mark();
    }
    long long grid = 256LL * 2;
    if (grid > n_img) grid = n_img;
    hipLaunchKernelGGL(kern, dim3((unsigned)grid), dim3(256), lds, (hipStream_t)stream, in, w, pmax, pmin, mean_img, m2_img, w_ld,
                       n_img);
    return mft_launch_status();
}
```

meta-fine-tuning_amd/engine.py:

```python
import os

import ctypes

import numpy as np
import torch

from . import functional as Fn
from . import ops
from . import settings


_DEBUG_SKIP_TRUNK = settings.current().debug_skip_trunk


def pick_slab_buffers(rates, K):
    import itertools
    best, best_score = None, -1.0
    for m_, v_ in itertools.combinations(range(K), 2):
        ws = sorted((rates[tuple(sorted((w_, m_, v_)))], w_) for w_ in range(K) if w_ not in (m_, v_))
        score = min(ws[-1][0], ws[-2][0])
        if score > best_score:
            best, best_score = (ws[-1][1], m_, v_, ws[-2][1]), score
    return best

# ... 267 lines not shown
            self.cls = {k: torch.zeros((self.E, n_way, 512) if k.endswith("W") else (self.E, n_way), device=self.dev)
                        for k in ("W", "b", "mW", "vW", "mb", "vb")}
        if mode == "dist":
            self.cls = {k: torch.zeros((self.E, n_way, 512) if k.endswith("V") else (self.E, n_way), device=self.dev)
                        for k in ("V", "g", "mV", "vV", "mg", "vg")}
            self.dist_scale = 2.0 if n_way <= 200 else 10.0
        self.arena = Fn.Arena(self.dev)
        self.arena_trunk = Fn.Arena(self.dev)
        self.adapt = AdaptState(self.E, self.dev)
        self.step_dev = torch.zeros(1, dtype=torch.int32, device=self.dev)
        self.hyper = torch.zeros(2, device=self.dev)
        self.pipeline = pipeline
        cfg = settings.current()
        self._fuse_next_setting = cfg.fuse_next
        self.fuse_next = False
        _set_wgrad_fwd_xcd_once()
        self.trunk_chunk = (int(trunk_chunk) if trunk_chunk is not None else
                            cfg.trunk_chunk if cfg.trunk_chunk is not None else (32 if episodes_per_batch == 1 else 1))
        prio = cfg.trunk_priority
        self.s_trunk = None
        self._raw_last = None
        n_tr = cfg.trunk_cus_per_xcd
        if pipeline and 0 < n_tr < 32:
            def masked(bits):
                words = (ctypes.c_uint * 8)()
                for b in bits:
                    words[b // 32] |= (1 << (b % 32))
                out = ctypes.c_void_p()
                ops._lib.check(ops._lib.lib().mft_stream_create_cumask(ctypes.cast(words, ctypes.c_void_p), 8, ctypes.byref(out)),
                               "mft_stream_create_cumask")
                return out.value
            self._raw_stream = masked([i for i in range(256) if (i // 8) >= 32 - n_tr])
            self.s_trunk = torch.cuda.ExternalStream(self._raw_stream, device=self.dev)
            if not cfg.trunk_cus_only:
                self._raw_last = masked([i for i in range(256) if (i // 8) < 32 - n_tr])
                self.s_last = torch.cuda.ExternalStream(self._raw_last, device=self.dev)
        elif pipeline and prio > 0:
            out = ctypes.c_void_p()
            with torch.cuda.device(self.dev):
                ops._lib.check(ops._lib.lib().mft_stream_create_priority(prio, ctypes.byref(out), None), "mft_stream_create_priority")
            self._raw_stream = out.value
            self.s_trunk = torch.cuda.ExternalStream(out.value, device=self.dev)
        elif pipeline:
            self.s_trunk = torch.cuda.Stream(device=self.dev, priority=prio)
        if self._raw_last is None:
            self.s_last = torch.cuda.Stream(device=self.dev, priority=cfg.last_priority) if pipeline else None
        px = image_size * image_size * 3
        self.Xs = torch.empty((self.E * self.n_total, px), device=self.dev)
        self.Xall = torch.empty((self.E * self.n_all, image_size, image_size, 3), device=self.dev)
        ya = np.repeat(np.arange(n_way), n_support)
        self.y_support = (np.tile(ya, n_views + 1) if self.views else ya).astype(np.int32)
        if stem_cache:
            pooled_pref = False if Fn.X3_PLANES else None
            need = Fn.StemCache.bytes_needed(self.E * self.n_total, image_size, pooled=pooled_pref)
            total = torch.cuda.get_device_properties(self.dev).total_memory
            stem_cache = need <= 0.35 * total
        self._stem_pooled = False if Fn.X3_PLANES else None
        self.stem = Fn.StemCache(self.W, self.E * self.n_total, image_size, self.dev, pooled=self._stem_pooled) if stem_cache else None
        self.fuse_next = fuse_next_policy(self._fuse_next_setting, self.E, self.stem is not None, image_size, self.W.f16x2)

    @_on_device
    def load_episode(self, slot, liz_x, Xs=None, Xall=None):
        Xs = self.Xs if Xs is None else Xs
        Xall = self.Xall if Xall is None else Xall
        ns, npv, H = self.n_support, self.n_per_view, self.size
        assert len(liz_x) == self.n_views
        views = [liz_x[0].to(self.dev, non_blocking=True)]
        assert views[0].shape[1] == ns + self.n_query
        if self.views:
            views += [xv.to(self.dev, non_blocking=True) for xv in liz_x[1:]]
        views = [v if (v.dtype == torch.float32 and v.is_contiguous()) else v.float().contiguous() for v in views]
        ptrs = (ctypes.c_void_p * len(views))(*[v.data_ptr() for v in views])
        rc = ops._lib.lib().mft_ingest_episode_views(ptrs, len(views), 1 if self.views else 0, self.n_way,
                                                     ns + self.n_query, ns, 3, H, H, ops._p(Xs[slot * self.n_total]),
                                                     ops._p(Xall[slot * self.n_all]), ops._stream())
        ops._lib.check(rc, "mft_ingest_episode_views")

    @_on_device
    def load_episode_source(self, slot, src_u8, params, Xs=None, Xall=None):
        from . import augment
        Xs = self.Xs if Xs is None else Xs
        Xall = self.Xall if Xall is None else Xall
        ns, npv, H = self.n_support, self.n_per_view, self.size
        assert self.views and params.shape[0] == self.n_views
        src = src_u8.to(self.dev)
        n_way, per, Hs, Ws, _ = src.shape
        assert n_way == self.n_way and per == ns + self.n_query
        P = torch.as_tensor(params, dtype=torch.float32).view(self.n_views, n_way, per, augment.NPARAM)
        px = H * H * 3
        sup_src = src[:, :ns].reshape(npv, Hs, Ws, 3).contiguous()
        Ps = P[:, :, :ns].reshape(self.n_views, npv, augment.NPARAM)
        Ps = torch.cat([Ps[:1], Ps], 0)
        augment.augment_views(sup_src, Ps, H, out=Xs[slot * self.n_total], view_stride=npv * px, img_stride=px)
        all_src = src.reshape(self.n_all, Hs, Ws, 3).contiguous()
        augment.augment_views(all_src, P[:1].reshape(1, self.n_all, augment.NPARAM), H, out=Xall[slot * self.n_all],
                              view_stride=self.n_all * px, img_stride=px)

    def step_tables(self, perms, n_active):
        E, bs, nt = self.E, self.bs, self.n_total
        P = np.empty((E, self.epochs, nt), dtype=np.int64)
        for e in range(E):
            pe = perms[min(e, n_active - 1)]
            for ep in range(self.epochs):
                P[e, ep] = pe[ep]
        base = (np.arange(E, dtype=np.int64) * nt)[:, None]
        tables = []
        for ep in range(self.epochs):
            sel_all = P[:, ep]
            idx_all = (sel_all + base).astype(np.int32)
            lab_all = self.y_support[sel_all]
            for j in range(0, nt, bs):
# ... 217 lines not shown
        ns = self.n_support // 2 if self.fold50 else self.n_support
        scores = Fn.gnnnet_scores(self.G, feats, self.E, self.n_way, ns, self.n_query, arena, fold=self.fold50)
        return ops.softmax_rows(scores).view(self.E, self.n_way * self.n_query, self.n_way), feats

    def set_classifier(self, w0, b0, n_active):
        c = self.cls
        for k in ("mW", "vW", "mb", "vb"):
            c[k].zero_()
        w0 = torch.as_tensor(w0, dtype=torch.float32).to(self.dev).view(-1, self.n_way, 512)
        b0 = torch.as_tensor(b0, dtype=torch.float32).to(self.dev).view(-1, self.n_way)
        idx = torch.clamp(torch.arange(self.E, device=self.dev), max=n_active - 1)
        c["W"].copy_(w0[idx])
        c["b"].copy_(b0[idx])

    def set_dist_head(self, v0, g0, n_active):
        c = self.cls
        for k in ("mV", "vV", "mg", "vg"):
            c[k].zero_()
        v0 = torch.as_tensor(v0, dtype=torch.float32).to(self.dev).view(-1, self.n_way, 512)
        g0 = torch.as_tensor(g0, dtype=torch.float32).to(self.dev).view(-1, self.n_way)
        idx = torch.clamp(torch.arange(self.E, device=self.dev), max=n_active - 1)
        c["V"].copy_(v0[idx])
        c["g"].copy_(g0[idx])

    def _flip_buffers(self):
        if self._alt is None:
            self._alt = [(self.adapt.w, self.Xall),
                         (Fn.LastBlockSlab(self.E, self.dev, zero=False, flat=self.adapt.w_alt_flat), torch.empty_like(self.Xall))]
            self._final_done = [None, None]
            self._bi = 0
            self.arena_final = Fn.Arena(self.dev)
            self.s_final = torch.cuda.Stream(device=self.dev)
        self._bi ^= 1
        self.adapt.w, self.Xall = self._alt[self._bi]
        if self._final_done[self._bi] is not None:
            torch.cuda.current_stream(self.dev).wait_event(self._final_done[self._bi])

    def _ingest(self, episodes, sources, Xs=None, Xall=None):
        n = len(episodes)
        for slot in range(self.E):
            ep = episodes[min(slot, n - 1)]
            if sources:
                self.load_episode_source(slot, ep[0], ep[1], Xs, Xall)
            else:
                self.load_episode(slot, ep, Xs, Xall)

    def _enqueue_prefetch(self, episodes, sources):
        if self._pre_bufs is None:
            need = self.Xs.numel() * 4 + self.stem.nbytes()
            free, total = torch.cuda.mem_get_info(self.dev)
            if need > 0.8 * free:
                return
            self._pre_bufs = {"Xs": torch.empty_like(self.Xs),
                              "stem": Fn.StemCache(self.W, self.E * self.n_total, self.size, self.dev, pooled=self._stem_pooled),
                              "stream": torch.cuda.Stream(device=self.dev)}
        b = self._pre_bufs
        sp = b["stream"]
        cur = torch.cuda.current_stream(self.dev)
        nxt = self._bi ^ 1
        sp.wait_stream(cur)
        if self._final_done[nxt] is not None:
            sp.wait_event(self._final_done[nxt])
        with torch.cuda.stream(sp):
            self._ingest(episodes, sources, b["Xs"], self._alt[nxt][1])
            b["stem"].fill(b["Xs"].view(self.E * self.n_total, self.size, self.size, 3))
            ev = torch.cuda.Event()
            ev.record(sp)
        self._pre = {"token": episodes, "sources": sources, "done": ev, "n": len(episodes)}

    @_on_device
    def run_batch(self, episodes, perms=None, return_feats=False, classifier_init=None, sources=False, defer_final=False,
                  prefetch=None):
        n = len(episodes)
        assert 0 < n <= self.E
        defer_final = defer_final and self.views and not self.use_graph and not return_feats
        if defer_final:
            self._flip_buffers()
        if perms is None:
            perms = [draw_perms(self.n_total, self.epochs) for _ in range(n)]
        pre, self._pre = self._pre, None
        if pre is not None and defer_final and pre["token"] is episodes and pre["sources"] == sources and pre["n"] == n:
            b = self._pre_bufs
            self.Xs, b["Xs"] = b["Xs"], self.Xs
            self.stem, b["stem"] = b["stem"], self.stem
            torch.cuda.current_stream(self.dev).wait_event(pre["done"])
            prepared = True
        else:
            if pre is not None:
                torch.cuda.current_stream(self.dev).wait_event(pre["done"])
            self._ingest(episodes, sources)
            prepared = False
        self.adapt.reset(self.W)
        self.step_dev.zero_()
        if self.mode == "linear":
            if classifier_init is None:
                raise RuntimeError("mode='linear' needs classifier_init=(w0 [n,n_way,512], b0 [n,n_way])")
            self.set_classifier(classifier_init[0], classifier_init[1], n)
        if self.mode == "dist":
            if classifier_init is None:
                raise RuntimeError("mode='dist' needs classifier_init=(v0 [n,n_way,512], g0 [n,n_way])")
            self.set_dist_head(classifier_init[0], classifier_init[1], n)
        if not prepared:
            self.prepare_batch()
        if prefetch is not None and defer_final and self.stem is not None and self.pipeline:
            self._enqueue_prefetch(prefetch, sources)
        self.inner_loop(self.step_tables(perms, n))
        if defer_final:
# ... 198 lines not shown
```

meta-fine-tuning_amd/functional.py:

```python
import os

import numpy as np

import torch

from . import ops
from . import settings

FUSED_DGRAD = settings.current().fused_dgrad
FUSED_LAST_BLOCK = settings.current().fused_last_block
X3_PLANES = settings.current().x3_planes
X3_FUSED_STATS = settings.current().x3_fused_stats
X3_FOLD_BN = settings.current().x3_fold_bn
TRUNK_F16X2 = settings.current().trunk_f16x2
TRAIN_X3 = settings.current().train_x3
TRAIN_X3_MIN_ROWS = settings.current().train_x3_min_rows
FUSE_NEXT_C2_ONLY = settings.current().fuse_next_c2_only
F16X2_BOUND = 3.0e4
F16X2_FLOOR = 2.0 ** -10
F16X2_MAX_ROWS = 1 << 20


def stem_rows_bound(ipg, image_size):
    oh = (image_size + 6 - 7) // 2 + 1
# ... 167 lines not shown
        off = 0
        for name, n in self.ORDER:
            v = self.flat[off:off + E * n]
            if name.endswith("w"):
                cout = 512
                v = v.view(E, cout, n // cout)
            else:
                v = v.view(E, n)
            setattr(self, name, v)
            off += E * n
        assert off == total

    def load_shared(self, W):
        self.c1w.copy_(W.conv["trunk.7.C1"].unsqueeze(0).expand_as(self.c1w))
        self.c2w.copy_(W.conv["trunk.7.C2"].unsqueeze(0).expand_as(self.c2w))
        self.scw.copy_(W.conv["trunk.7.shortcut"].unsqueeze(0).expand_as(self.scw))
        for nm, bnname in (("bn1", "trunk.7.BN1"), ("bn2", "trunk.7.BN2"), ("bns", "trunk.7.BNshortcut")):
            g, b = W.bn[bnname]
            getattr(self, nm + "g").copy_(g.unsqueeze(0).expand(self.E, -1))
            getattr(self, nm + "b").copy_(b.unsqueeze(0).expand(self.E, -1))

    def export(self, e):
        out = {}
        for name, _ in self.ORDER:
            key = self.KEY[name]
            t = getattr(self, name)[e]
            if name.endswith("w"):
                out[key] = ops.unpack_conv_weight(t.contiguous(), ADAPT_SHAPES[key])
            else:
                out[key] = t.clone()
        return out


def _bn_stats4(arena, tag, x, ipg, groups, running=None, fixed=None):
    if fixed is not None:
        return fixed
    n, H, W, C = x.shape
    mean = arena.get(tag + ".mean", (groups, C))
    rstd = arena.get(tag + ".rstd", (groups, C))
    rows = ipg * H * W
    nws = max(int(ops._lib.lib().mft_bn_stats_ws_floats(C, rows, groups)), 1)
    ws = arena.get("bn.ws", (max(nws, 1 << 16),)) if nws <= (1 << 16) else arena.get(tag + ".ws", (nws,))
    rm = rv = nbt = None
    if running is not None:
        rm, rv, nbt = running if len(running) == 3 else (running + (None,))
    rc = ops._lib.lib().mft_bn_stats(ops._p(x), C, C, rows, groups, ops.BN_EPS, ops._p(mean), ops._p(rstd), ops._p(ws),
                                     ops._p(rm), ops._p(rv), 0.1, ops._p(nbt), ops._stream())
    ops._lib.check(rc, "mft_bn_stats")
    return mean, rstd


class StemCache:

    def __init__(self, W, n_slots, H, device, chunk=8192, pooled=None):
        self.W = W
        self.n_slots = n_slots
        self.OH = (H + 6 - 7) // 2 + 1
        self.PH = (self.OH + 2 - 3) // 2 + 1
        cfg = settings.current()
        self.pooled = cfg.stem_pooled if pooled is None else bool(pooled)
        chunk = chunk if cfg.stem_chunk is None else cfg.stem_chunk
        self.chunk = min(chunk, n_slots)
        self.mean = torch.empty((n_slots, 64), device=device)
        self.m2 = torch.empty((n_slots, 64), device=device)
        self.fused_fill = bool(self.pooled and cfg.stem_fused_fill and H == 84)
        if self.pooled:
            self.c0 = None
            self._buf = None if self.fused_fill else torch.empty((self.chunk, self.OH, self.OH, 64), device=device)
            self.pmax = torch.empty((n_slots, self.PH, self.PH, 64), device=device)
            self.pmin = torch.empty((n_slots, self.PH, self.PH, 64), device=device)
        else:
            self.c0 = torch.empty((n_slots, self.OH, self.OH, 64), device=device)

    def nbytes(self):
        ts = [self.mean, self.m2] + ([self._buf, self.pmax, self.pmin] if self.pooled else [self.c0])
        return sum(t.numel() * 4 for t in ts if t is not None)

    @staticmethod
    def bytes_needed(n_slots, H, pooled=None, chunk=8192):
        cfg = settings.current()
        pooled = cfg.stem_pooled if pooled is None else bool(pooled)
        chunk = min(chunk if cfg.stem_chunk is None else cfg.stem_chunk, n_slots)
        oh = (H + 6 - 7) // 2 + 1
        ph = (oh + 2 - 3) // 2 + 1
        per = 2 * 64 + (2 * ph * ph * 64 if pooled else oh * oh * 64)
        fused = bool(pooled and cfg.stem_fused_fill and H == 84)
        return 4 * (n_slots * per + (chunk * oh * oh * 64 if (pooled and not fused) else 0))

    def fill(self, x_nhwc):
        lib = ops._lib.lib()
        n = x_nhwc.shape[0]
        assert n == self.n_slots
        if self.fused_fill:
            wpk = self.W.conv["trunk.0"]
            rc = lib.mft_stem_cache_fill(ops._p(x_nhwc), ops._p(wpk), wpk.shape[-1], n, x_nhwc.shape[1], x_nhwc.shape[2],
                                         ops._p(self.pmax), ops._p(self.pmin), ops._p(self.mean), ops._p(self.m2), ops._stream())
            if rc != ops._lib.MFT_EINVAL:
                ops._lib.check(rc, "mft_stem_cache_fill")
                return
            self.fused_fill = False
            self._buf = torch.empty((self.chunk, self.OH, self.OH, 64), device=x_nhwc.device)
        for i in range(0, n, self.chunk):
            j = min(i + self.chunk, n)
            c0 = self._buf[:j - i] if self.pooled else self.c0[i:j]
            ops.conv2d(x_nhwc[i:j], self.W.conv["trunk.0"], 64, 7, 7, 2, 3, out=c0)
            ops._lib.check(lib.mft_bn_image_moments(ops._p(c0), 64, 64, self.OH * self.OH, j - i,
                                                    ops._p(self.mean[i:j]), ops._p(self.m2[i:j]), ops._stream()),
                           "mft_bn_image_moments")
            if self.pooled:
                ops._lib.check(lib.mft_pool_window_minmax(ops._p(c0), ops._p(self.pmax[i:j]), ops._p(self.pmin[i:j]), j - i,
                                                          self.OH, self.OH, 64, ops._stream()), "mft_pool_window_minmax")

    def gather(self, idx, n, m, s, g, b, ipg, out, planes=None):
        if self.pooled and planes is None:
            ops._lib.check(ops._lib.lib().mft_bn_relu_pooled_gather(ops._p(self.pmax), ops._p(self.pmin), ops._p(idx), ops._p(out), n,
                                                                    self.PH, self.PH, 64, ipg, ops._p(m), ops._p(s), ops._p(g),
                                                                    ops._p(b), ops._stream()), "mft_bn_relu_pooled_gather")
            return out
        assert self.c0 is not None, "this path needs the full-resolution stem cache (StemCache(pooled=False))"
        return ops.bn_relu_maxpool_gather(self.c0, idx, n, m, s, g, b, ipg, out=out, planes=planes)

    def gather_moments(self, idx, n, g, b, ipg, out, stats=None):
        assert self.pooled
        m, s = stats if stats is not None else (None, None)
        ops._lib.check(ops._lib.lib().mft_bn_relu_pooled_gather_moments(
            ops._p(self.pmax), ops._p(self.pmin), ops._p(idx), ops._p(out), n, self.PH, self.PH, 64, ipg, ops._p(self.mean),
            ops._p(self.m2), self.OH * self.OH, ops.BN_EPS, ops._p(g), ops._p(b), ops._p(m), ops._p(s), ops._stream()),
            "mft_bn_relu_pooled_gather_moments")
        return out


def resnet10_trunk(W, x, arena, ipg, upto=7, running=None, tag="t", stem=None, fixed=None):

    def run(name):
        return None if running is None else running.get(name)

    def fix(name):
        return None if fixed is None else fixed[name]

    g, b = W.bn["trunk.1"]
    if stem is not None:
        cache, idx = stem
        n = idx.numel()
        groups = n // ipg
        PH = (cache.OH + 2 - 3) // 2 + 1
        fold = X3_FOLD_BN and cache.pooled and not X3_PLANES and running is None and fixed is None
        if not fold:
            m = arena.get(tag + ".bn0.mean", (groups, 64))
            s = arena.get(tag + ".bn0.rstd", (groups, 64))
            ops.bn_combine_moments(cache.mean, cache.m2, idx, cache.OH * cache.OH, ipg, groups, mean=m, rstd=s)
        if (X3_PLANES and cache.c0 is not None and X3_FUSED_STATS and upto == 7 and running is None and fixed is None and ipg * ((PH + 3) // 4) ** 2 >= 128
                and all(("trunk.%d.C1" % i) in W.conv3 for i in (4, 5, 6))):
            ap = arena.get(tag + ".p0p", (3, n * PH * PH, 64), torch.int16)
            a = cache.gather(idx, n, m, s, g, b, ipg, arena.get(tag + ".p0", (n, PH, PH, 64)), planes=ap)
            shape = (n, PH, PH, 64)
            for bi in (4, 5, 6):
                cin, cout, stride = STAGES[bi]
                p = "trunk.%d" % bi
                mode = "f32" if bi == 6 else "planes"
                r = simple_block(W, p, a if bi == 4 else None, arena, ipg, cin, cout, stride, None, tag + "." + p, xp=ap,
                                 xshape=shape, out_mode=mode)
                if mode == "f32":
                    return r
                _, ap = r
                OHb = (shape[1] + 2 - 3) // stride + 1
                shape = (n, OHb, OHb, cout)
        if fold:
            a = cache.gather_moments(idx, n, g, b, ipg, arena.get(tag + ".p0", (n, PH, PH, 64)))
        else:
            a = cache.gather(idx, n, m, s, g, b, ipg, arena.get(tag + ".p0", (n, PH, PH, 64)))
    else:
        n = x.shape[0]
        groups = n // ipg
        c0 = ops.conv2d(x, W.conv["trunk.0"], 64, 7, 7, 2, 3, out=arena.get(tag + ".c0", (n, (x.shape[1] + 6 - 7) // 2 + 1, (x.shape[2] + 6 - 7) // 2 + 1, 64)))
        m, s = _bn_stats4(arena, tag + ".bn0", c0, ipg, groups, run("trunk.1"), fix("trunk.1"))
        a = ops.bn_relu_maxpool(c0, m, s, g, b, imgs_per_group=ipg)
    for idx in (4, 5, 6, 7):
        if idx >= upto:
            break
        cin, cout, stride = STAGES[idx]
        p = "trunk.%d" % idx
        a = simple_block(W, p, a, arena, ipg, cin, cout, stride, running, tag + "." + p, fixed=fixed)
    return a


def _bn_small(arena, tag, x1, g1, b1, rows, groups, C, gbs, out, x2=None, g2=None, b2=None, res=None, pooled=None, hw=0, stats=None,
              stats2=None):
    m1, s1 = stats if stats is not None else (arena.get(tag + ".mean", (groups, C)), arena.get(tag + ".rstd", (groups, C)))
    m2 = s2 = None
    if x2 is not None:
        m2, s2 = stats2 if stats2 is not None else (arena.get(tag + ".mean2", (groups, C)), arena.get(tag + ".rstd2", (groups, C)))
    rc = ops._lib.lib().mft_bn_small_forward(ops._p(x1), C, ops._p(x2), C, ops._p(res), C, ops._p(out), C, C, rows, groups,
                                             ops._p(g1), ops._p(b1), ops._p(g2), ops._p(b2), gbs, ops._p(m1), ops._p(s1),
                                             ops._p(m2), ops._p(s2), ops.ACT_RELU, 0.0, ops.BN_EPS, ops._p(pooled), hw,
                                             ops._stream())
    ops._lib.check(rc, "mft_bn_small_forward")
    return m1, s1, m2, s2


def simple_block(W, p, x, arena, ipg, cin, cout, stride, running=None, tag="b", slab=None, tape=None, pooled=None, fixed=None,
                 xp=None, xshape=None, out_mode="f32", stats_out=None):
    n, H, Wd, _ = x.shape if x is not None else xshape
    groups = n // ipg
    OH = (H + 2 - 3) // stride + 1

    def run(name):
        return None if running is None else running.get(name)

    def fix(name):
        return None if fixed is None else fixed[name]

    if slab is None:
        c1w, c2w = W.conv[p + ".C1"], W.conv[p + ".C2"]
        (g1, b1), (g2, b2) = W.bn[p + ".BN1"], W.bn[p + ".BN2"]
        scw = W.conv.get(p + ".shortcut")
        gs, bs = W.bn.get(p + ".BNshortcut", (None, None))
        gbs = 0
    else:
        c1w, c2w, scw = slab.c1w, slab.c2w, slab.scw
        g1, b1, g2, b2, gs, bs = slab.bn1g, slab.bn1b, slab.bn2g, slab.bn2b, slab.bnsg, slab.bnsb
        gbs = cout
    wipg = ipg if slab is not None else 0
    w3 = W.planes(p, ipg, H, fixed, running) if slab is None else {}

    def conv(name, inp, wpk, k, s, pd, out):
        if (p + name) in w3:
            return ops.conv2d_x3(inp, w3[p + name], cout, k, k, s, pd, out=out)
        return ops.conv2d(inp, wpk, cout, k, k, s, pd, imgs_per_group=wipg, out=out)

    rows = ipg * OH * OH
    if slab is not None and rows <= 64 and cout % 64 == 0 and cin != cout and running is None:
        so = stats_out or {}
        c1 = arena.get(tag + ".c1", (n, OH, OH, cout))
        r1 = arena.get(tag + ".r1", (n * OH * OH, cout))
# ... 60 lines not shown
        def conv_bn_p(name, inp_p, h_in, k, s, pd, obuf, stag):
            nws = int(ops._lib.lib().mft_conv2d_x3_stats_ws_floats(n, h_in, h_in, cout, k, k, s, pd))
            ws = arena.get("x3.statws", (max(nws, 1 << 20),)) if nws <= (1 << 20) else arena.get(stag + ".statws", (nws,))
            mean = arena.get(stag + ".mean", (groups, cout))
            rstd = arena.get(stag + ".rstd", (groups, cout))
            return ops.conv2d_x3p_bnstats(inp_p, n, h_in, h_in, w3[p + name], cout, k, k, s, pd, ipg, obuf, ws, mean, rstd)

        c1, m1, s1 = conv_bn_p(".C1", xp, H, 3, stride, 1, arena.get(tag + ".c1", (n, OH, OH, cout)), tag + ".bn1")
        r1p = arena.get(tag + ".r1p", (3, n * OH * OH, cout), torch.int16)
        ops.bn_apply(c1.view(-1, cout), cout, rows, groups, m1, s1, g1, b1, act=ops.ACT_RELU, fma_affine=True, gb_group_stride=gbs, planes=r1p,
                     write_y=False)
        c2, m2, s2 = conv_bn_p(".C2", r1p, OH, 3, 1, 1, arena.get(tag + ".c2", (n, OH, OH, cout)), tag + ".bn2")
        want_f32 = out_mode in ("f32", "both")
        out = arena.get(tag + ".out", (n * OH * OH, cout)) if want_f32 else None
        outp = arena.get(tag + ".outp", (3, n * OH * OH, cout), torch.int16) if out_mode in ("planes", "both") else None
        if cin != cout:
            sc, ms, ss = conv_bn_p(".shortcut", xp, H, 1, stride, 0, arena.get(tag + ".sc", (n, OH, OH, cout)), tag + ".bns")
            res, res_bn = sc.view(-1, cout), (ms, ss, gs, bs)
        else:
            res, res_bn = x.view(-1, cin), None
        if outp is not None:
            ops.bn_apply(c2.view(-1, cout), cout, rows, groups, m2, s2, g2, b2, act=ops.ACT_RELU, fma_affine=True, res=res, res_bn=res_bn, out=out,
                         gb_group_stride=gbs, planes=outp, write_y=want_f32)
        else:
            ops.bn_apply(c2.view(-1, cout), cout, rows, groups, m2, s2, g2, b2, act=ops.ACT_RELU, fma_affine=True, res=res, res_bn=res_bn, out=out,
                         gb_group_stride=gbs)
        out = out.view(n, OH, OH, cout) if out is not None else None
        return out if out_mode == "f32" else (out, outp)
    assert out_mode == "f32" or xp is None or not fuse_stats, "planes output requested outside the pre-split chain"

    c1, m1, s1 = conv_bn(".C1", ".BN1", x, c1w, 3, stride, 1, arena.get(tag + ".c1", (n, OH, OH, cout)), tag + ".bn1")
    r1 = ops.bn_apply(c1.view(-1, cout), cout, rows, groups, m1, s1, g1, b1, act=ops.ACT_RELU, fma_affine=fuse_stats,
                      out=arena.get(tag + ".r1", (n * OH * OH, cout)), gb_group_stride=gbs).view(n, OH, OH, cout)
    c2, m2, s2 = conv_bn(".C2", ".BN2", r1, c2w, 3, 1, 1, arena.get(tag + ".c2", (n, OH, OH, cout)), tag + ".bn2")
    out = arena.get(tag + ".out", (n * OH * OH, cout))
    sc = ms = ss = None
    if cin != cout:
        sc, ms, ss = conv_bn(".shortcut", ".BNshortcut", x, scw, 1, stride, 0, arena.get(tag + ".sc", (n, OH, OH, cout)),
                             tag + ".bns")
        ops.bn_apply(c2.view(-1, cout), cout, rows, groups, m2, s2, g2, b2, act=ops.ACT_RELU, fma_affine=fuse_stats, res=sc.view(-1, cout),
                     res_bn=(ms, ss, gs, bs), out=out, gb_group_stride=gbs)
    else:
        ops.bn_apply(c2.view(-1, cout), cout, rows, groups, m2, s2, g2, b2, act=ops.ACT_RELU, fma_affine=fuse_stats, res=x.view(-1, cin),
                     out=out, gb_group_stride=gbs)
    out = out.view(n, OH, OH, cout)
    if tape is not None:
        tape.update(x=x, c1=c1, m1=m1, s1=s1, r1=r1, c2=c2, m2=m2, s2=s2, sc=sc, ms=ms, ss=ss, out=out)
    return out


_X3WS_FITS = {}


def _frozen_block_folded(W, p, x, arena, ipg, cin, cout, stride, tag):
    n, H, _, _ = x.shape
    groups = n // ipg
    OH = (H + 2 - 3) // stride + 1
    rows = ipg * OH * OH
    lib = ops._lib.lib()
    fits = _X3WS_FITS.get((cout, rows))
    if fits is None:
        fits = _X3WS_FITS[(cout, rows)] = bool(lib.mft_bn_apply_x3ws_fits(cout, rows, 1))
    if not fits:
        return None
    (g1, b1), (g2, b2) = W.bn[p + ".BN1"], W.bn[p + ".BN2"]
    w3 = W.conv3

    def partials(name, inp, k, s, pd, obuf, stag):
        ws = arena.get(stag + ".statws", (int(lib.mft_conv2d_x3_stats_ws_floats(n, inp.shape[1], inp.shape[1], cout, k, k, s, pd)),))
        r = ops.conv2d_x3_bnstats(inp, w3[p + name], cout, k, k, s, pd, ipg, obuf, ws, None, None)
        return None if r is None else ws

    c1 = arena.get(tag + ".c1", (n, OH, OH, cout))
    ws1 = partials(".C1", x, 3, stride, 1, c1, tag + ".bn1")
    if ws1 is None:
        return None
    c2 = arena.get(tag + ".c2", (n, OH, OH, cout))
    ws2 = arena.get(tag + ".bn2.statws", (int(lib.mft_conv2d_x3_stats_ws_floats(n, OH, OH, cout, 3, 3, 1, 1)),))
    if ops.conv2d_x3_bnin_bnstats(c1, ws1, g1, b1, w3[p + ".C2"], cout, ipg, c2, ws2) is None:
        r1 = ops.bn_apply_x3ws(c1.view(-1, cout), cout, rows, groups, ws1, g1, b1, arena.get(tag + ".r1", (n * OH * OH, cout)),
                               act=ops.ACT_RELU).view(n, OH, OH, cout)
        if ops.conv2d_x3_bnstats(r1, w3[p + ".C2"], cout, 3, 3, 1, 1, ipg, c2, ws2, None, None) is None:
            raise RuntimeError("frozen block %s: C2 outside the bf16x3 domain after C1 was inside it" % p)
    out = arena.get(tag + ".out", (n * OH * OH, cout))
    if cin != cout:
        gs, bs = W.bn[p + ".BNshortcut"]
        sc = arena.get(tag + ".sc", (n, OH, OH, cout))
        wss = partials(".shortcut", x, 1, stride, 0, sc, tag + ".bns")
        if wss is None:
            raise RuntimeError("frozen block %s: shortcut outside the bf16x3 domain after C1 was inside it" % p)
        ops.bn_apply_x3ws(c2.view(-1, cout), cout, rows, groups, ws2, g2, b2, out, act=ops.ACT_RELU, res=sc.view(-1, cout),
                          res_ws=wss, res_gamma=gs, res_beta=bs)
    else:
        ops.bn_apply_x3ws(c2.view(-1, cout), cout, rows, groups, ws2, g2, b2, out, act=ops.ACT_RELU, res=x.view(-1, cin))
    return out.view(n, OH, OH, cout)


def last_block_forward(W, a, arena, ipg, slab=None, tape=None, running=None, tag="f", fixed=None, stats_out=None):
    n = a.shape[0]
    feat = arena.get(tag + ".feat", (n, 512))
    info = tape if tape is not None else {}
    out = simple_block(W, "trunk.7", a, arena, ipg, 256, 512, 2, running, tag + ".trunk.7", slab=slab, tape=info, pooled=feat,
                       fixed=fixed, stats_out=stats_out)
    if not info.get("pooled", False):
        ops._lib.check(ops._lib.lib().mft_global_avgpool(ops._p(out), ops._p(feat), n, out.shape[1] * out.shape[2], 512,
                                                         ops._stream()), "mft_global_avgpool")
    return feat


def resnet10_forward(W, x, arena, ipg=0, slab=None, tape=None, running=None, tag="f", fixed=None):
    n = x.shape[0]
    if ipg <= 0 or fixed is not None:
        ipg = n
    a = resnet10_trunk(W, x, arena, ipg, upto=7, running=running, tag=tag, fixed=fixed)
    return last_block_forward(W, a, arena, ipg, slab=slab, tape=tape, running=running, tag=tag, fixed=fixed)


def _dgrad_c2_bn1(lib, tape, params, grads, arena, tag, dc2, c1, r1, n, oh, ow, C, ipg, bn_bwd):
    rc = ops._lib.MFT_EINVAL
    if FUSED_LAST_BLOCK and n // ipg > ops.SMALL_GROUPS:
        dc1 = arena.get(tag + ".dc1", tuple(c1.shape))
        w2 = params.c2w
        rc = lib.mft_conv2d_dgrad_bn_backward_small(ops._p(dc2), C, ops._p(w2), ops._p(dc1), C, n, oh, ow, C, C, 3, 3, 1, ipg,
                                                    w2.shape[1] * w2.shape[2], ops._p(c1), ops._p(r1), ops._p(tape["m1"]),
                                                    ops._p(tape["s1"]), ops._p(params.bn1g), C, ops._p(grads.bn1g),
                                                    ops._p(grads.bn1b), ops._stream())
        if rc != ops._lib.MFT_EINVAL:
            ops._lib.check(rc, "mft_conv2d_dgrad_bn_backward_small")
    if rc == ops._lib.MFT_EINVAL:
        dr1 = ops.conv2d_dgrad(dc2, params.c2w, 512, 3, 3, 1, imgs_per_group=ipg, out=arena.get(tag + ".dr1", (n, oh, ow, C)))
        dc1 = bn_bwd(c1, dr1, tape["m1"], tape["s1"], params.bn1g, grads.bn1g, grads.bn1b, r1, "dc1")
    return dc1


def next_step_tape(arena, tag, n, oh, ow, C, groups):
    rows = n * oh * ow
    t = {k: arena.get(tag + "." + k, (n, oh, ow, C)) for k in ("c1", "r1", "c2", "sc", "out")}
    for k in ("m1", "s1", "m2", "s2", "ms", "ss"):
        t[k] = arena.get(tag + "." + k, (groups, C))
    t["feat"] = arena.get(tag + ".feat", (n, C))
    t["pooled"] = True
    assert t["c1"].numel() == rows * C
    return t


# ... 337 lines not shown
```

meta-fine-tuning_amd/ops.py:

```python
import ctypes
import os

import torch

from . import _lib
from . import settings

ACT_NONE, ACT_RELU, ACT_LRELU = 0, 1, 2
BN_EPS = 1e-5
LRELU_SLOPE = 0.01


import threading

_tls = threading.local()


def _stream(t=None):
    dev = getattr(_tls, "dev", None)
    _tls.dev = None
    if t is not None:
        dev = t.device.index if torch.is_tensor(t) else (t.index if isinstance(t, torch.device) else int(t))
    return ctypes.c_void_p(torch.cuda.current_stream(dev).cuda_stream)

# ... 201 lines not shown

def _x3_fn(w3, stem):
    kind = {3: "x3", 2: "h2"}[int(w3.shape[0])]
    name = "mft_conv2d_nhwc_%s%s" % (kind, stem)
    return getattr(_lib.lib(), name), name


def conv2d_x3(x, w3, Cout, KH, KW, stride, pad, out=None):
    _f32c(x)
    n, H, W, Cin = x.shape
    OH = (H + 2 * pad - KH) // stride + 1
    OW = (W + 2 * pad - KW) // stride + 1
    if out is None:
        out = torch.empty((n, OH, OW, Cout), device=x.device, dtype=torch.float32)
    fn, name = _x3_fn(w3, "")
    rc = fn(_p(x), Cin, _p(w3), w3.shape[1] * w3.shape[2], _p(out), Cout, n, H, W, Cin, Cout, KH, KW, stride, pad, _stream())
    _lib.check(rc, name)
    return out


def conv2d_x3_bnstats(x, w3, Cout, KH, KW, stride, pad, imgs_per_group, out, ws, mean, rstd, eps=BN_EPS):
    _f32c(x)
    n, H, W, Cin = x.shape
    fn, name = _x3_fn(w3, "_bnstats")
    rc = fn(_p(x), Cin, _p(w3), w3.shape[1] * w3.shape[2], _p(out), Cout, n, H, W, Cin, Cout, KH, KW, stride, pad, imgs_per_group, eps,
            _p(ws), _p(mean), _p(rstd), _stream())
    if rc == _lib.MFT_EINVAL:
        return None
    _lib.check(rc, name)
    return out, mean, rstd


def conv2d_x3_bnin_bnstats(c_raw, in_ws, in_gamma, in_beta, w3, Cout, imgs_per_group, out, ws, mean=None, rstd=None, eps=BN_EPS):
    _f32c(c_raw)
    n, H, W, Cin = c_raw.shape
    fn, name = _x3_fn(w3, "_bnin_bnstats")
    rc = fn(_p(c_raw), Cin, _p(in_ws), _p(in_gamma), _p(in_beta), _p(w3), w3.shape[1] * w3.shape[2], _p(out), Cout, n, H, W, Cin, Cout,
            imgs_per_group, eps, _p(ws), _p(mean), _p(rstd), _stream())
    if rc == _lib.MFT_EINVAL:
        return None
    _lib.check(rc, name)
    return out


def bn_apply_x3ws(x2d, C, rows_per_group, n_groups, ws, gamma, beta, out, act=ACT_NONE, res=None, res_ws=None, res_gamma=None,
                  res_beta=None, slope=LRELU_SLOPE, eps=BN_EPS, stats=None, res_stats=None):
    _f32c(x2d)
    m, r = stats if stats is not None else (None, None)
    rm, rr = res_stats if res_stats is not None else (None, None)
    rc = _lib.lib().mft_bn_apply_x3ws(_p(x2d), x2d.shape[-1], _p(out), out.shape[-1], C, rows_per_group, n_groups, _p(ws), _p(gamma),
                                      _p(beta), _p(res), 0 if res is None else res.shape[-1], _p(res_ws), _p(res_gamma),
                                      _p(res_beta), act, slope, eps, _p(m), _p(r), _p(rm), _p(rr), _stream())
    _lib.check(rc, "mft_bn_apply_x3ws")
    return out


def conv2d_x3p_bnstats(xp, n, H, W, w3, Cout, KH, KW, stride, pad, imgs_per_group, out, ws, mean, rstd, eps=BN_EPS):
    Cin = xp.shape[2]
    if w3.shape[0] != 3:
        raise ValueError("pre-split activation planes exist for the bf16x3 kernels only")
    rc = _lib.lib().mft_conv2d_nhwc_x3p_bnstats(_p(xp), xp.shape[1] * Cin, Cin, _p(w3), w3.shape[1] * w3.shape[2], _p(out), Cout,
                                                n, H, W, Cin, Cout, KH, KW, stride, pad, imgs_per_group, eps, _p(ws), _p(mean),
                                                _p(rstd), _stream())
    _lib.check(rc, "mft_conv2d_nhwc_x3p_bnstats")
    return out, mean, rstd


def gemm(a, K, w_pk, N, bias=None, out=None, ldo=None, rows_per_group=0):
    _f32c(a)
    M, lda = a.shape
    if out is None:
        ldo = N if ldo is None else ldo
        out = torch.empty((M, ldo), device=a.device, dtype=torch.float32)
    else:
        ldo = out.shape[1]
    wgs = 0
    if w_pk.dim() == 3:
        wgs = w_pk.shape[1] * w_pk.shape[2]
    rc = _lib.lib().mft_conv2d_nhwc(_p(a), lda, _p(w_pk), _p(bias), _p(out), ldo, M, 1, 1, K, N, 1, 1, 1, 0,
                                    rows_per_group, wgs, _stream())
    _lib.check(rc, "mft_conv2d_nhwc(gemm)")
    return out


def gemm_rk(a, K, w_pk, N, bias=None, out=None, ldo=None):
    _f32c(a)
    M, lda = a.shape
    assert w_pk.dim() == 2 and w_pk.shape[1] == K and w_pk.shape[0] >= N and K % 16 == 0 and K <= 512, (tuple(w_pk.shape), K, N)
    if out is None:
        ldo = N if ldo is None else ldo
        out = torch.empty((M, ldo), device=a.device, dtype=torch.float32)
    else:
        ldo = out.shape[1]
    _lib.check(_lib.lib().mft_gemm_rk(_p(a), lda, _p(w_pk), w_pk.shape[0], K, _p(bias), _p(out), ldo, M, N, _stream()), "mft_gemm_rk")
    return out


def conv2d_dgrad(dy, w_pk, Cin, KH, KW, pad, imgs_per_group=0, out=None, stride=1, in_hw=None):
    _f32c(dy)
    n, OH, OW, Cout = dy.shape
    H, W = (OH, OW) if in_hw is None else in_hw
    if out is None:
        out = torch.empty((n, H, W, Cin), device=dy.device, dtype=torch.float32)
    wgs = w_pk.shape[1] * w_pk.shape[2] if w_pk.dim() == 3 else 0
    if ((wgs == 0 and imgs_per_group <= 0) or (w_pk.dim() == 3 and w_pk.shape[0] == 1)) and Cin % 64 == 0:
        nws = _ksplit_ws(n * H * W, Cin, KH * KW * Cout)
# ... 616 lines not shown
```

meta-fine-tuning_amd/settings.py:

```python
import dataclasses
import os


def _flag(v):
    lv = v.strip().lower()
    if lv in ("1", "true", "yes", "on"):
        return True
    if lv in ("0", "false", "no", "off"):
        return False
    raise ValueError("expected 0 / 1 (or true / false), got %r" % (v,))


def _opt_int(v):
    return None if v in ("", "none", "None") else int(v)


def _fuse(v):
    if v not in ("auto", "0", "1"):
        raise ValueError("expected auto, 0 or 1, got %r" % (v,))
    return v


KNOBS = (
    ("fuse_next", "MFT_FUSE_NEXT", _fuse, "auto", "fused weight-gradient + Adam + next-step forward launches: auto = engine.fuse_next_policy | 1 | 0"),
    ("wf_xcd", "MFT_WF_XCD", _flag, True, "fused launch: all workgroups of an episode on one XCD (A/B hook; read once per process)"),
    ("slab_candidates", "MFT_SLAB_CANDIDATES", _opt_int, None, "candidate buffers of the w/m/v placement scan (None: engine default 12; 0: off)"),
    ("slab_ballast_gb", "MFT_SLAB_BALLAST_GB", float, 12.0, "throw-away allocation between groups of placement candidates, GB"),
    ("slab_hints", "MFT_SLAB_HINTS", _flag, True, "re-use an earlier scan's placement when one probe confirms it"),
    ("trunk_chunk", "MFT_TRUNK_CHUNK", _opt_int, None, "inner steps per frozen-trunk launch set (None: 32 at E = 1, else 1)"),
    ("trunk_priority", "MFT_TRUNK_PRIORITY", int, 1, "HIP priority of the frozen-trunk stream (1 = the device's least)"),
    ("last_priority", "MFT_LAST_PRIORITY", int, -1, "torch priority of the last-block stream"),
    ("trunk_cus_per_xcd", "MFT_TRUNK_CUS_PER_XCD", int, 0, "CU-masked streams: CUs per XCD for the trunk stream (0 = no partition; measured slower)"),
    ("trunk_cus_only", "MFT_TRUNK_CUS_ONLY", _flag, False, "with trunk_cus_per_xcd: confine only the trunk stream"),
    ("debug_skip_trunk", "MFT_DEBUG_SKIP_TRUNK", _flag, False, "measurement aid: reuse one cached trunk output (results are WRONG)"),
    ("adapt_graph", "MFT_ADAPT_GRAPH", _flag, True, "adapt_last_block: replay the meta-fine-tuning inner loop from one hipGraph"),
    ("adapt_batched_trunk", "MFT_ADAPT_BATCHED_TRUNK", _flag, True, "adapt_last_block: frozen trunk of all steps as two grouped passes"),
    ("fused_dgrad", "MFT_FUSED_DGRAD", _flag, False, "one-pass trunk.7.C2 weight gradient + Adam + data gradient (measured slower in the step)"),
    ("x3_planes", "MFT_X3_PLANES", _flag, False, "trunk activations pre-split into bf16x3 planes (measured slower)"),
    ("x3_fused_stats", "MFT_X3_FUSED_STATS", _flag, True, "BatchNorm statistics from the split-precision convolution epilogue"),
    ("x3_fold_bn", "MFT_X3_FOLD_BN", _flag, True, "frozen blocks without helper launches (per-tile partials merged by the consumers)"),
    ("trunk_f16x2", "MFT_TRUNK_F16X2", _flag, True, "frozen trunk.4-6 on two fp16 pieces per operand (0: three bf16 pieces)"),
    ("fuse_next_c2_only", "MFT_FUSE_NEXT_C2_ONLY", _flag, False, "only trunk.7.C2's launch fused (measured slower)"),
    ("stem_pooled", "MFT_STEM_POOLED", _flag, True, "stem cache keeps per-window (max, min) instead of the full-resolution output"),
    ("stem_fused_fill", "MFT_STEM_FUSED_FILL", _flag, True, "stem cache filled by ONE launch (convolution + moments + window min/max; 0: three launches through a full-resolution buffer)"),
    ("stem_chunk", "MFT_STEM_CHUNK", _opt_int, None, "images per stem-cache fill launch (None: StemCache's default)"),
    ("fused_last_block", "MFT_FUSED_LAST_BLOCK", _flag, True, "conv + BatchNorm fusions of the adapted block (csrc/skinny.hip)"),
    ("small_groups", "MFT_SMALL_GROUPS", int, 12, "up to this many per-episode weight sets take the K-sliced GEMM route"),
    ("fused_pair_mlp", "MFT_FUSED_PAIR_MLP", _flag, True, "Wcompute on the fused upper-triangle pair-MLP kernels"),
    ("pair_mlp_gb", "MFT_PAIR_MLP_GB", float, 6.0, "memory budget of the fused pair-MLP's hidden activations per chunk, GB"),
    ("train_graph", "MFT_TRAIN_GRAPH", _flag, True, "MetaTemplate episode loop: loss + backward replayed from one hipGraph"),
    ("train_x3", "MFT_TRAIN_X3", _flag, True, "meta-training: 3x3 layers with >= 8192 output rows on the bf16x3 kernels, forward and stride-1 data gradient (0: fp32 MFMA everywhere)"),
    ("train_x3_min_rows", "MFT_TRAIN_X3_MIN_ROWS", int, 6000, "meta-training: output rows from which a 3x3 layer takes the bf16x3 kernels (below: fp32 MFMA with K slices; measured at 3,780 / 945 rows in profiles/r06_q_train_x3_min_rows.txt)"),
    ("wgrad_batch", "MFT_WGRAD_BATCH", _flag, True, "meta-training backward: every layer's weight gradient deferred to the end of the pass and run in one multi-problem launch pair per 16 layers (0: one launch pair per layer, as round 5; bit-identical)"),
    ("pair_f16x2", "MFT_PAIR_F16X2", _flag, False, "GNN pair-MLP layers (Wcompute) as f16x2 products on the fp16 matrix cores (fp32-accurate; 0: fp32 MFMA)"),
    ("gemm_rk_rows", "MFT_GEMM_RK_ROWS", int, 4096, "meta-training: head linear layers (fc, Gconv.fc) of at most this many rows take the skinny register-K GEMM (0: the tile kernel always)"),
    ("pair_rk_rows", "MFT_PAIR_RK_ROWS", int, 16384, "meta-training: Wcompute layers over at most this many pair rows (all episodes of the step) take the register-K small-problem kernel, 32-row tiles, no LDS staging (0: the 128-row tile kernel always)"),
    ("train_source", "MFT_TRAIN_SOURCE", str, "pool", "train.main --dataset miniImageNet: 'pool' = resident uint8 class pool, 'synthetic' = host fp32 episodes"),
    ("standin_weights", "MFT_STANDIN_WEIGHTS", _flag, False, "allow synthetic stand-in weights when no checkpoint is found (explicit opt-in)"),
    ("image_size", "MFT_IMAGE_SIZE", int, 84, "image side the CLI evaluates at (84 = BASELINE; 224 = the reference's)"),
    ("episodes", "MFT_EPISODES", _opt_int, None, "override of the CLI's episode count (None: 600)"),
    ("episodes_per_batch", "MFT_EPISODES_PER_BATCH", _opt_int, None, "override of the CLI's lockstep batch (None: 128 / 96 / 64 by n_shot)"),
    ("timings", "MFT_TIMINGS", _flag, False, "print the drivers' phase timings to stderr"),
    ("pool_per_class", "MFT_POOL_PER_CLASS", _opt_int, None, "images per class of the dataset-shaped resident pool (None: the dataset's)"),
    ("synth_on_host", "MFT_SYNTH_ON_HOST", _flag, False, "generate synthetic test episodes with numpy on the host instead of on the device"),
    ("balance_batches", "MFT_BALANCE_BATCHES", _flag, True, "equalise the lockstep batch sizes of an evaluation"),
    ("force_collectives", "MFT_FORCE_COLLECTIVES", _flag, False, "run the N-rank collectives even with one rank (1-GPU RCCL tests)"),
    ("one_device", "MFT_ONE_DEVICE", _flag, False, "test hook: W ranks share device 0, gloo for the gathers"),
)


@dataclasses.dataclass(frozen=True)
class Settings:
    fuse_next: str = "auto"
    wf_xcd: bool = True
    slab_candidates: "int | None" = None
    slab_ballast_gb: float = 12.0
    slab_hints: bool = True
    trunk_chunk: "int | None" = None
    trunk_priority: int = 1
    last_priority: int = -1
    trunk_cus_per_xcd: int = 0
    trunk_cus_only: bool = False
    debug_skip_trunk: bool = False
    adapt_graph: bool = True
    adapt_batched_trunk: bool = True
    fused_dgrad: bool = False
    x3_planes: bool = False
    x3_fused_stats: bool = True
    x3_fold_bn: bool = True
    trunk_f16x2: bool = True
    fuse_next_c2_only: bool = False
    stem_pooled: bool = True
    stem_fused_fill: bool = True
    stem_chunk: "int | None" = None
    fused_last_block: bool = True
    small_groups: int = 12
    fused_pair_mlp: bool = True
    pair_mlp_gb: float = 6.0
    train_graph: bool = True
    train_x3: bool = True
    train_x3_min_rows: int = 6000
    wgrad_batch: bool = True
    pair_f16x2: bool = False
    gemm_rk_rows: int = 4096
    pair_rk_rows: int = 16384
    train_source: str = "pool"
    standin_weights: bool = False
    image_size: int = 84
    episodes: "int | None" = None
    episodes_per_batch: "int | None" = None
    timings: bool = False
    pool_per_class: "int | None" = None
    synth_on_host: bool = False
    balance_batches: bool = True
    force_collectives: bool = False
    one_device: bool = False

    @classmethod
    def from_env(cls, env=None):
        env = os.environ if env is None else env
        kw = {}
        for field, var, parse, default, _ in KNOBS:
            raw = env.get(var)
            if raw is None:
                kw[field] = default
                continue
            try:
                kw[field] = parse(raw)
            except (TypeError, ValueError) as e:
                raise ValueError("%s=%r: %s" % (var, raw, e)) from None
        s = cls(**kw)
        if s.train_source not in ("pool", "synthetic"):
            raise ValueError("MFT_TRAIN_SOURCE=%r: expected pool or synthetic" % (s.train_source,))
        if s.image_size < 32 or not 0 <= s.trunk_cus_per_xcd < 32:
            raise ValueError("MFT_IMAGE_SIZE / MFT_TRUNK_CUS_PER_XCD out of range")
        return s


assert tuple(f.name for f in dataclasses.fields(Settings)) == tuple(k[0] for k in KNOBS), "KNOBS and Settings fields must match"
_VARS = tuple(k[1] for k in KNOBS)
_cache = (None, None)


def current():
    global _cache
    key = tuple(os.environ.get(v) for v in _VARS)
    if _cache[0] != key:
# ... 16 lines not shown
```

Baseline: 86.05.

## Keep one gamma-selected stem extremum per window and fuse it into trunk.4

The stem cache now stores a single pooled value per window, the max or min picked by the sign of trunk.1's frozen gamma, in place of a (max, min) pair. trunk.4's first conv reads this cache directly and applies BN+ReLU on the fly with per-group moments. Its residual add recomputes the stem activation inside the BN-apply kernel, so the separate gather launch and the materialized p0 buffer are no longer needed. This halves stem cache memory and traffic and removes launches. The cost is new kernel variants with fallback paths, and more LDS use for the staged moments.

New measurement: 85.98. No clear change (-0.1%).

```diff
diff --git a/include/mft_hip.h b/include/mft_hip.h
--- a/include/mft_hip.h
+++ b/include/mft_hip.h
@@ -50,6 +50,9 @@
 int mft_stem_cache_fill(const float* in, const float* w, int w_ld, int n_img, int H, int W, float* pmax, float* pmin,
                         float* mean_img, float* m2_img, void* stream);
 int mft_pool_window_minmax(const float* x, float* ymax, float* ymin, long long n_img, int H, int W, int C, void* stream);
+int mft_stem_cache_fill_select(const float* in, const float* w, int w_ld, int n_img, int H, int W, const float* gamma, float* psel,
+                               float* mean_img, float* m2_img, void* stream);
+int mft_pool_window_select(const float* x, const float* gamma, float* ysel, long long n_img, int H, int W, int C, void* stream);
 int mft_bn_relu_pooled_gather(const float* pmax, const float* pmin, const int* src_idx, float* y, int n_img, int OH, int OW, int C,
                               int imgs_per_group, const float* mean, const float* rstd, const float* gamma, const float* beta,
                               void* stream);
@@ -108,6 +111,15 @@
 int mft_bn_running_ema(const float* mean_a, const float* rstd_a, int rows_a, const float* mean_b, const float* rstd_b, int rows_b,
                        const int* order, int n_steps, int C, float eps, float momentum, float* running_mean, float* running_var,
                        void* stream);
+int mft_conv2d_nhwc_h2_stem_bnstats(const float* psel, const int* src_idx, const float* mean_img, const float* m2_img,
+                                    int rows_per_img, int imgs_per_group, const float* gamma, const float* beta, float eps,
+                                    const unsigned short* w2, long long plane_elems, float* out, int ldo, int n_img, int H, int W,
+                                    int Cin, int Cout, float* stats_ws, void* stream);
+int mft_bn_apply_x3ws_stemres(const float* x, int ldx, float* y, int ldy, int C, int n_img, int HW, int imgs_per_group,
+                              const float* ws, const float* gamma, const float* beta, const float* psel, const int* src_idx,
+                              const float* mean_img, const float* m2_img, int rows_per_img, const float* res_gamma,
+                              const float* res_beta, int act, float slope, float eps, float* mean, float* rstd, float* res_mean,
+                              float* res_rstd, void* stream);
 int mft_bn_apply_x3ws_fits(int C, int rows_per_group, int with_res_bn);
 int mft_bn_relu_pooled_gather_moments(const float* pmax, const float* pmin, const int* src_idx, float* y, int n_img, int OH, int OW,
                                       int C, int imgs_per_group, const float* mean_img, const float* m2_img, int rows_per_img,
diff --git a/meta-fine-tuning_amd/_lib.py b/meta-fine-tuning_amd/_lib.py
--- a/meta-fine-tuning_amd/_lib.py
+++ b/meta-fine-tuning_amd/_lib.py
@@ -90,6 +90,11 @@
     "mft_ce_pool_bn_backward2": [_P, _P, _I, _I, _I, _I, _P, _P, _P, _P, _P, _P, _P, _P, _P, _P, _P, _L, _P, _P, _P, _P, _P, _P],
     "mft_pool_window_minmax": [_P, _P, _P, _L, _I, _I, _I, _P],
     "mft_stem_cache_fill": [_P, _P, _I, _I, _I, _I, _P, _P, _P, _P, _P],
+    "mft_stem_cache_fill_select": [_P, _P, _I, _I, _I, _I, _P, _P, _P, _P, _P],
+    "mft_pool_window_select": [_P, _P, _P, _L, _I, _I, _I, _P],
+    "mft_conv2d_nhwc_h2_stem_bnstats": [_P, _P, _P, _P, _I, _I, _P, _P, _F, _P, _L, _P, _I, _I, _I, _I, _I, _I, _P, _P],
+    "mft_bn_apply_x3ws_stemres": [_P, _I, _P, _I, _I, _I, _I, _I, _P, _P, _P, _P, _P, _P, _P, _I, _P, _P, _I, _F, _F, _P, _P, _P,
+                                  _P, _P],
     "mft_conv2d_nhwc_x3_bnin_bnstats": [_P, _I, _P, _P, _P, _P, _L, _P, _I, _I, _I, _I, _I, _I, _I, _F, _P, _P, _P, _P],
     "mft_split_f16x2": [_P, _P, _L, _P],
     "mft_conv2d_nhwc_h2": [_P, _I, _P, _L, _P, _I, _I, _I, _I, _I, _I, _I, _I, _I, _I, _P],
diff --git a/meta-fine-tuning_amd/csrc/bn.hip b/meta-fine-tuning_amd/csrc/bn.hip
--- a/meta-fine-tuning_amd/csrc/bn.hip
+++ b/meta-fine-tuning_amd/csrc/bn.hip
@@ -235,8 +235,12 @@
     int act; float slope, eps;
     float* mean; float* rstd; float* rmean; float* rrstd;
     int max_tiles;
+    const float* sr_psel; const int* sr_idx; const float* sr_mean_img; const float* sr_m2_img;
+    const float* sr_gamma; const float* sr_beta;
+    int sr_hw, sr_ipg, sr_rows_per_img;
 };
 
+template <bool STEMRES>
 __global__ __launch_bounds__(256) void bn_apply_ws_kernel(ApplyWsArgs p) {
     extern __shared__ __attribute__((aligned(16))) float tab[];
     const int g = blockIdx.y, C = p.C;
@@ -244,6 +248,18 @@
     char* rstage = stage + mft_x3_stage_bytes(p.max_tiles, C);
     mft_x3_stats_stage(p.ws, C, g, p.M, p.rows_per_group, p.BM, p.max_tiles, stage, threadIdx.x, 256);
     if (p.rws) mft_x3_stats_stage(p.rws, C, g, p.M, p.rows_per_group, p.BM, p.max_tiles, rstage, threadIdx.x, 256);
+    if constexpr (STEMRES) {
+        const int* id = p.sr_idx + (long long)g * p.sr_ipg;
+        float* smom = reinterpret_cast<float*>(rstage);
+        stage_group_moments(p.sr_mean_img, p.sr_m2_img, id, C, p.sr_ipg, smom, threadIdx.x, 256);
+        __syncthreads();
+        for (int c = threadIdx.x; c < C; c += 256) {
+            float mu, rs;
+            combine_moments_lds(smom, smom + p.sr_ipg * C, C, c, p.sr_rows_per_img, p.sr_ipg, p.eps, mu, rs);
+            tab[2 * C + c] = mu; tab[3 * C + c] = rs;
+            if (blockIdx.x == 0 && p.rmean) { p.rmean[(long long)g * C + c] = mu; p.rrstd[(long long)g * C + c] = rs; }
+        }
+    }
     __syncthreads();
     for (int c = threadIdx.x; c < C; c += 256) {
         float mu, rs, sc, sh;
@@ -268,7 +284,12 @@
         const long long row = row0 + rr;
         const f32x4 v = *(const f32x4*)(p.x + row * p.ldx + c);
         f32x4 o = mft_bn_affine4(v, *(const f32x4*)(tab + c), *(const f32x4*)(tab + C + c));
-        if (p.res) {
+        if constexpr (STEMRES) {
+            const int n = rr / p.sr_hw, pix = rr - n * p.sr_hw;
+            const long long src = ((long long)p.sr_idx[(long long)g * p.sr_ipg + n] * p.sr_hw + pix) * C + c;
+            o += pooled_bn_relu_value(*(const f32x4*)(p.sr_psel + src), *(const f32x4*)(tab + 2 * C + c), *(const f32x4*)(tab + 3 * C + c),
+                                      *(const f32x4*)(p.sr_gamma + c), *(const f32x4*)(p.sr_beta + c));
+        } else if (p.res) {
             f32x4 rv = *(const f32x4*)(p.res + row * p.ldr + c);
             if (p.rws) rv = mft_bn_affine4(rv, *(const f32x4*)(tab + 2 * C + c), *(const f32x4*)(tab + 3 * C + c));
             o += rv;
@@ -475,34 +496,11 @@
     }
 }
 
-template <class MeanOf, class M2Of>
-__device__ __forceinline__ void combine_moments_impl(MeanOf mean_of, M2Of m2_of, int rows_per_img, int imgs_per_group, float eps,
-                                                     float& mean, float& rstd) {
-    float mu = 0.f;
-    for (int i = 0; i < imgs_per_group; ++i) mu += mean_of(i);
-    mu /= (float)imgs_per_group;
-    float m2 = 0.f, dev = 0.f;
-    for (int i = 0; i < imgs_per_group; ++i) {
-        const float d = mean_of(i) - mu;
-        m2 += m2_of(i);
-        dev += d * d;
-    }
-    const float var = (m2 + (float)rows_per_img * dev) / ((float)rows_per_img * (float)imgs_per_group);
-    mean = mu;
-    rstd = 1.0f / sqrtf(var + eps);
-}
-
 __device__ __forceinline__ void combine_moments(const float* __restrict__ mean_img, const float* __restrict__ m2_img,
                                                 const int* __restrict__ id, int C, int c, int rows_per_img, int imgs_per_group,
                                                 float eps, float& mean, float& rstd) {
     combine_moments_impl([&](int i) { return mean_img[(long long)id[i] * C + c]; },
                          [&](int i) { return m2_img[(long long)id[i] * C + c]; }, rows_per_img, imgs_per_group, eps, mean, rstd);
-}
-
-__device__ __forceinline__ void combine_moments_lds(const float* smean, const float* sm2, int C, int c, int rows_per_img,
-                                                    int imgs_per_group, float eps, float& mean, float& rstd) {
-    combine_moments_impl([&](int i) { return smean[i * C + c]; }, [&](int i) { return sm2[i * C + c]; }, rows_per_img,
-                         imgs_per_group, eps, mean, rstd);
 }
 
 __global__ void bn_combine_moments_kernel(const float* __restrict__ mean_img, const float* __restrict__ m2_img,
@@ -777,8 +775,37 @@
     if (sub > cap) sub = cap;
     if (sub < 1) sub = 1;
     ApplyWsArgs p{x, y, ldx, ldy, C, rows_per_group, n_groups, (int)M, 128, ws, gamma, beta, res, ldr, res_ws, res_gamma, res_beta,
-                  act, slope, eps, mean, rstd, res_mean, res_rstd, max_tiles};
-    hipLaunchKernelGGL(bn_apply_ws_kernel, dim3(sub, n_groups), dim3(256), lds, (hipStream_t)stream, p);
+                  act, slope, eps, mean, rstd, res_mean, res_rstd, max_tiles, nullptr, nullptr, nullptr, nullptr, nullptr, nullptr, 0, 0, 0};
+    hipLaunchKernelGGL(bn_apply_ws_kernel<false>, dim3(sub, n_groups), dim3(256), lds, (hipStream_t)stream, p);
+    return mft_launch_status();
+}
+
+extern "C" int mft_bn_apply_x3ws_stemres(const float* x, int ldx, float* y, int ldy, int C, int n_img, int HW, int imgs_per_group,
+                                         const float* ws, const float* gamma, const float* beta, const float* psel, const int* src_idx,
+                                         const float* mean_img, const float* m2_img, int rows_per_img, const float* res_gamma,
+                                         const float* res_beta, int act, float slope, float eps, float* mean, float* rstd,
+                                         float* res_mean, float* res_rstd, void* stream) {
+    if (C % 4 != 0 || C > 1024 || ldx % 4 != 0 || ldy % 4 != 0 || !ws || !y || !x || !psel || !src_idx || !mean_img || !m2_img ||
+        !res_gamma || !res_beta || HW <= 0 || rows_per_img <= 0 || imgs_per_group <= 0 || n_img <= 0 || n_img % imgs_per_group != 0 ||
+        (mean == nullptr) != (rstd == nullptr) || (res_mean == nullptr) != (res_rstd == nullptr))
+        return MFT_EINVAL;
+    const long long rows_per_group = (long long)imgs_per_group * HW;
+    const int n_groups = n_img / imgs_per_group;
+    const long long M = (long long)n_img * HW;
+    if (rows_per_group < 128 || M > 0x7fffffffLL) return MFT_EINVAL;
+    const long long per_group = rows_per_group * (C / 4);
+    if (per_group > 0x7fffffffLL) return MFT_EINVAL;
+    const int max_tiles = mft_x3_max_group_tiles((int)rows_per_group, 128);
+    const size_t lds = (size_t)4 * C * sizeof(float) + mft_x3_stage_bytes_host(max_tiles, C) + (size_t)2 * imgs_per_group * C * sizeof(float);
+    if (lds > 64 * 1024) return MFT_EINVAL;
+    int sub = (int)((per_group + 256 * 16 - 1) / (256 * 16));
+    const int cap = (2048 + n_groups - 1) / n_groups;
+    if (sub > cap) sub = cap;
+    if (sub < 1) sub = 1;
+    ApplyWsArgs p{x, y, ldx, ldy, C, (int)rows_per_group, n_groups, (int)M, 128, ws, gamma, beta, nullptr, 0, nullptr, nullptr, nullptr,
+                  act, slope, eps, mean, rstd, res_mean, res_rstd, max_tiles, psel, src_idx, mean_img, m2_img, res_gamma, res_beta,
+                  HW, imgs_per_group, rows_per_img};
+    hipLaunchKernelGGL(bn_apply_ws_kernel<true>, dim3(sub, n_groups), dim3(256), lds, (hipStream_t)stream, p);
     return mft_launch_status();
 }
 
@@ -836,9 +863,10 @@
 }
 
 namespace {
+template <bool SEL>
 __global__ __launch_bounds__(256) void pool_window_minmax_kernel(const float* __restrict__ x, float* __restrict__ ymax,
                                                                  float* __restrict__ ymin, long long n_img, int H, int W, int C,
-                                                                 int OH, int OW) {
+                                                                 int OH, int OW, const float* __restrict__ sel_gamma) {
     const int cq = C >> 2;
     const long long total = n_img * OH * OW * cq;
     for (long long i = (long long)blockIdx.x * blockDim.x + threadIdx.x; i < total; i += (long long)gridDim.x * blockDim.x) {
@@ -861,27 +889,16 @@
                 for (int e = 0; e < 4; ++e) { hi[e] = fmaxf(hi[e], v[e]); lo[e] = fminf(lo[e], v[e]); }
             }
         }
-        *(f32x4*)(ymax + i * 4) = hi;
-        *(f32x4*)(ymin + i * 4) = lo;
-    }
-}
-
-__device__ __forceinline__ f32x4 pooled_bn_relu(const float* __restrict__ pmax, const float* __restrict__ pmin, long long src,
-                                                const f32x4 mu, const f32x4 rs, const f32x4 ga, const f32x4 be) {
-    const bool all_pos = ga[0] >= 0.f && ga[1] >= 0.f && ga[2] >= 0.f && ga[3] >= 0.f;
-    const bool all_neg = ga[0] < 0.f && ga[1] < 0.f && ga[2] < 0.f && ga[3] < 0.f;
-    f32x4 v;
-    if (all_pos) v = *(const f32x4*)(pmax + src);
-    else if (all_neg) v = *(const f32x4*)(pmin + src);
-    else {
-        const f32x4 a = *(const f32x4*)(pmax + src), b = *(const f32x4*)(pmin + src);
-#pragma unroll
-        for (int e = 0; e < 4; ++e) v[e] = ga[e] >= 0.f ? a[e] : b[e];
-    }
-    f32x4 o = __builtin_elementwise_fma((v - mu) * rs, ga, be);
-#pragma unroll
-    for (int e = 0; e < 4; ++e) o[e] = fmaxf(o[e], 0.f);
-    return o;
+        if constexpr (SEL) {
+            const f32x4 ga = *(const f32x4*)(sel_gamma + c);
+#pragma unroll
+            for (int e = 0; e < 4; ++e) hi[e] = pooled_takes_max(ga[e]) ? hi[e] : lo[e];
+            *(f32x4*)(ymax + i * 4) = hi;
+        } else {
+            *(f32x4*)(ymax + i * 4) = hi;
+            *(f32x4*)(ymin + i * 4) = lo;
+        }
+    }
 }
 
 __global__ __launch_bounds__(256) void bn_relu_pooled_gather_kernel(const float* __restrict__ pmax, const float* __restrict__ pmin,
@@ -946,8 +963,18 @@
     if (C % 4 != 0 || n_img <= 0) return MFT_EINVAL;
     const int OH = (H + 2 - 3) / 2 + 1, OW = (W + 2 - 3) / 2 + 1;
     const long long total = n_img * OH * OW * (C / 4);
-    hipLaunchKernelGGL(pool_window_minmax_kernel, dim3(grid_for(total, 256, 256 * 16)), dim3(256), 0, (hipStream_t)stream, x, ymax,
-                       ymin, n_img, H, W, C, OH, OW);
+    hipLaunchKernelGGL(pool_window_minmax_kernel<false>, dim3(grid_for(total, 256, 256 * 16)), dim3(256), 0, (hipStream_t)stream, x, ymax,
+                       ymin, n_img, H, W, C, OH, OW, (const float*)nullptr);
+    return mft_launch_status();
+}
+
+extern "C" int mft_pool_window_select(const float* x, const float* gamma, float* ysel, long long n_img, int H, int W, int C,
+                                      void* stream) {
+    if (C % 4 != 0 || n_img <= 0 || !gamma || !ysel) return MFT_EINVAL;
+    const int OH = (H + 2 - 3) / 2 + 1, OW = (W + 2 - 3) / 2 + 1;
+    const long long total = n_img * OH * OW * (C / 4);
+    hipLaunchKernelGGL(pool_window_minmax_kernel<true>, dim3(grid_for(total, 256, 256 * 16)), dim3(256), 0, (hipStream_t)stream, x, ysel,
+                       (float*)nullptr, n_img, H, W, C, OH, OW, gamma);
     return mft_launch_status();
 }
 
diff --git a/meta-fine-tuning_amd/csrc/bn_fold.h b/meta-fine-tuning_amd/csrc/bn_fold.h
--- a/meta-fine-tuning_amd/csrc/bn_fold.h
+++ b/meta-fine-tuning_amd/csrc/bn_fold.h
@@ -89,3 +89,63 @@
     scale = rstd * gamma;
     shift = __builtin_elementwise_fma(-mean, scale, beta);
 }
+
+template <class MeanOf, class M2Of>
+__device__ __forceinline__ void combine_moments_impl(MeanOf mean_of, M2Of m2_of, int rows_per_img, int imgs_per_group, float eps,
+                                                     float& mean, float& rstd) {
+    float mu = 0.f;
+    for (int i = 0; i < imgs_per_group; ++i) mu += mean_of(i);
+    mu /= (float)imgs_per_group;
+    float m2 = 0.f, dev = 0.f;
+    for (int i = 0; i < imgs_per_group; ++i) {
+        const float d = mean_of(i) - mu;
+        m2 += m2_of(i);
+        dev += d * d;
+    }
+    const float var = (m2 + (float)rows_per_img * dev) / ((float)rows_per_img * (float)imgs_per_group);
+    mean = mu;
+    rstd = 1.0f / sqrtf(var + eps);
+}
+
+__device__ __forceinline__ void combine_moments_lds(const float* smean, const float* sm2, int C, int c, int rows_per_img,
+                                                    int imgs_per_group, float eps, float& mean, float& rstd) {
+    combine_moments_impl([&](int i) { return smean[i * C + c]; }, [&](int i) { return sm2[i * C + c]; }, rows_per_img,
+                         imgs_per_group, eps, mean, rstd);
+}
+
+__device__ __forceinline__ void stage_group_moments(const float* __restrict__ mean_img, const float* __restrict__ m2_img,
+                                                    const int* __restrict__ id, int C, int imgs_per_group, float* stage, int tid,
+                                                    int nthreads) {
+    float* smean = stage;
+    float* sm2 = stage + imgs_per_group * C;
+    for (int i = tid; i < imgs_per_group * C; i += nthreads) {
+        const int im = i / C, c = i - im * C;
+        const long long src = (long long)id[im] * C + c;
+        smean[i] = mean_img[src];
+        sm2[i] = m2_img[src];
+    }
+}
+
+__device__ __forceinline__ bool pooled_takes_max(float gamma) { return gamma >= 0.f; }
+
+__device__ __forceinline__ f32x4 pooled_bn_relu_value(const f32x4 v, const f32x4 mu, const f32x4 rs, const f32x4 ga, const f32x4 be) {
+    f32x4 o = __builtin_elementwise_fma((v - mu) * rs, ga, be);
+#pragma unroll
+    for (int e = 0; e < 4; ++e) o[e] = fmaxf(o[e], 0.f);
+    return o;
+}
+
+__device__ __forceinline__ f32x4 pooled_bn_relu(const float* __restrict__ pmax, const float* __restrict__ pmin, long long src,
+                                                const f32x4 mu, const f32x4 rs, const f32x4 ga, const f32x4 be) {
+    const bool all_pos = pooled_takes_max(ga[0]) && pooled_takes_max(ga[1]) && pooled_takes_max(ga[2]) && pooled_takes_max(ga[3]);
+    const bool all_neg = !pooled_takes_max(ga[0]) && !pooled_takes_max(ga[1]) && !pooled_takes_max(ga[2]) && !pooled_takes_max(ga[3]);
+    f32x4 v;
+    if (all_pos) v = *(const f32x4*)(pmax + src);
+    else if (all_neg) v = *(const f32x4*)(pmin + src);
+    else {
+        const f32x4 a = *(const f32x4*)(pmax + src), b = *(const f32x4*)(pmin + src);
+#pragma unroll
+        for (int e = 0; e < 4; ++e) v[e] = pooled_takes_max(ga[e]) ? a[e] : b[e];
+    }
+    return pooled_bn_relu_value(v, mu, rs, ga, be);
+}
diff --git a/meta-fine-tuning_amd/csrc/conv_x3.hip b/meta-fine-tuning_amd/csrc/conv_x3.hip
--- a/meta-fine-tuning_amd/csrc/conv_x3.hip
+++ b/meta-fine-tuning_amd/csrc/conv_x3.hip
@@ -32,6 +32,8 @@
     const float* bn_ws; const float* bn_gamma; const float* bn_beta;
     float bn_eps;
     int bn_max_tiles;
+    const int* st_idx; const float* st_mean; const float* st_m2;
+    int st_rows_per_img, st_ipg;
 };
 
 constexpr int X3_RS = 40;
@@ -433,8 +435,9 @@
 #include "../../tools/experiments/conv_x3_pingpong.inc"
 #endif
 
-template <int BM, int BN, bool BNIN, int NP = 3, bool BDB = true>
+template <int BM, int BN, bool BNIN, int NP = 3, bool BDB = true, bool STEM = false>
 __device__ __forceinline__ void conv_x3_s1_body(const X3Args& p) {
+    static_assert(!(BNIN && STEM), "one loader-side BatchNorm");
     static_assert(NP == 3 || NP == 2, "3 bf16 pieces (six products) or 2 fp16 pieces (three products)");
     constexpr int NACC = NP == 3 ? 1 : 2;
     constexpr int TM = BM / 64, TN = BN / 64;
@@ -463,8 +466,8 @@
     const int m0 = mt * BM, n0 = nt * BN;
     const int W = p.W, H = p.H;
     const int fr0 = m0 / W;
-    const int g0 = BNIN ? m0 / p.rows_per_group : 0;
-    const bool bn_two = BNIN && (m0 + (BM < p.M - m0 ? BM : p.M - m0) - 1) / p.rows_per_group > g0;
+    const int g0 = (BNIN || STEM) ? m0 / p.rows_per_group : 0;
+    const bool bn_two = (BNIN || STEM) && (m0 + (BM < p.M - m0 ? BM : p.M - m0) - 1) / p.rows_per_group > g0;
     if constexpr (BNIN) {
         char* stage = reinterpret_cast<char*>(smem);
         const size_t gstride = mft_x3_stage_bytes(p.bn_max_tiles, p.Cin);
@@ -484,6 +487,29 @@
         }
         __syncthreads();
     }
+    if constexpr (STEM) {
+        float* stage = reinterpret_cast<float*>(smem);
+        const int gstride = 2 * p.st_ipg * p.Cin;
+        stage_group_moments(p.st_mean, p.st_m2, p.st_idx + (long long)g0 * p.st_ipg, p.Cin, p.st_ipg, stage, tid, 256);
+        if (bn_two)
+            stage_group_moments(p.st_mean, p.st_m2, p.st_idx + (long long)(g0 + 1) * p.st_ipg, p.Cin, p.st_ipg, stage + gstride, tid, 256);
+        __syncthreads();
+        for (int i = tid; i < 2 * p.Cin; i += 256) {
+            const int gi = i >= p.Cin ? 1 : 0, c = i - gi * p.Cin;
+            if (gi == 0 || bn_two) {
+                float mu, rs;
+                const float* sm = stage + gi * gstride;
+                combine_moments_lds(sm, sm + p.st_ipg * p.Cin, p.Cin, c, p.st_rows_per_img, p.st_ipg, p.bn_eps, mu, rs);
+                bn_tab[(gi * 2 + 0) * p.Cin + c] = mu;
+                bn_tab[(gi * 2 + 1) * p.Cin + c] = rs;
+            }
+            if (gi == 0) {
+                bn_tab[4 * p.Cin + c] = p.bn_gamma[c];
+                bn_tab[5 * p.Cin + c] = p.bn_beta[c];
+            }
+        }
+        __syncthreads();
+    }
     const int g_id = tid >> 5, g_rr = (tid >> 3) & 3;
     const int lrow = p.row_swz ? g_rr * 4 + (g_id & 3) + 16 * (g_id >> 2) : tid >> 3;
     const int c4 = (tid & 7) * 4;
@@ -491,12 +517,27 @@
     const __amdgpu_buffer_rsrc_t rB = __builtin_amdgcn_make_buffer_rsrc((void*)p.w3, 0, p.w_bytes, 0x00020000);
     int a_off[PA], a_oh[PA], a_lds[PA], a_tab[PA];
     bool a_ok[PA];
+    constexpr int ST_OFF = 0xfffff, ST_KH = 20, ST_IMG1 = 1 << 23, ST_GRP1 = 1 << 24;
+    int a_pk[PA];
+    const int HW = H * W;
+    const int img0 = STEM ? m0 / HW : 0, img_last = STEM ? p.M / HW - 1 : 0;
+    const float* const base0 = STEM ? p.in + (long long)p.st_idx[img0] * HW * p.ldi : nullptr;
+    const float* const base1 = STEM ? p.in + (long long)p.st_idx[img0 < img_last ? img0 + 1 : img_last] * HW * p.ldi : nullptr;
+    auto stem_pack = [&](int m, bool ok) {
+        if (!ok) return c4;
+        const bool second = m >= (img0 + 1) * HW;
+        const int fr = m / W, oh = fr - (fr / H) * H;
+        return ((m - (img0 + (second ? 1 : 0)) * HW) * p.ldi + c4) | (oh > 0 ? 1 << ST_KH : 0) | (2 << ST_KH) | (oh < H - 1 ? 4 << ST_KH : 0) |
+               (second ? ST_IMG1 : 0) | (m / p.rows_per_group > g0 ? ST_GRP1 : 0);
+    };
+    auto stem_word = [&](int pk) { asm volatile("" : "+v"(pk)); return pk; };
 #pragma unroll
     for (int j = 0; j < PA; ++j) {
         const int t = lrow + 32 * j, m = m0 + t;
         const int fr = m / W;
         a_ok[j] = m < p.M;
         a_oh[j] = fr - (fr / H) * H;
+        a_pk[j] = STEM ? stem_pack(m, a_ok[j]) : 0;
         a_off[j] = ((a_ok[j] ? m : 0) * p.ldi + c4) * 4;
         a_lds[j] = (t + 1) * RS + c4;
         a_tab[j] = BNIN ? ((a_ok[j] ? m / p.rows_per_group - g0 : 0) * 2 * p.Cin + c4) : 0;
@@ -506,6 +547,7 @@
     const int frh = (mh > 0 ? mh : 0) / W;
     const bool h_ok = tid < 16 && (hside ? (mh < p.M && mh - frh * W != 0) : (m0 > 0 && m0 - fr0 * W != 0));
     const int h_oh = frh - (frh / H) * H;
+    const int h_pk = STEM ? stem_pack(mh, h_ok) : 0;
     const int h_off = ((h_ok ? mh : 0) * p.ldi + c4) * 4;
     const int h_lds = (hside ? BM + 1 : 0) * RS + c4;
     const int h_tab = BNIN ? (((hside && h_ok) ? (m0 + BM - 1) / p.rows_per_group - g0 : 0) * 2 * p.Cin + c4) : 0;
@@ -553,6 +595,16 @@
     auto load_a = [&](int ms, Stage& S) {
         const int kh = ms / n_ci, ci0 = (ms - kh * n_ci) * 32;
         const int shift = ((kh - 1) * W * p.ldi + ci0) * 4;
+        if constexpr (STEM) {
+            const int eshift = (kh - 1) * W * p.ldi + ci0;
+            auto fetch = [&](int pk) {
+                return *(const f32x4*)(((pk & ST_IMG1) ? base1 : base0) + ((pk & ST_OFF) + (((pk >> (ST_KH + kh)) & 1) ? eshift : 0)));
+            };
+#pragma unroll
+            for (int j = 0; j < PA; ++j) S.ra[j] = fetch(stem_word(a_pk[j]));
+            S.rh = fetch(stem_word(h_pk));
+            return;
+        }
 #pragma unroll
         for (int j = 0; j < PA; ++j) {
             const bool ok = a_ok[j] && (unsigned)(a_oh[j] + kh - 1) < (unsigned)H;
@@ -590,8 +642,19 @@
         for (int e = 0; e < 4; ++e) o[e] = ok ? fmaxf(o[e], 0.f) : 0.f;
         return o;
     };
+    auto stem_relu = [&](const f32x4 v, int pk, int kh, int ci0) {
+        const float* row = bn_tab + ((pk & ST_GRP1) ? 2 * p.Cin : 0) + ci0 + c4;
+        const f32x4 o = pooled_bn_relu_value(v, *(const f32x4*)row, *(const f32x4*)(row + p.Cin),
+                                             *(const f32x4*)(bn_tab + 4 * p.Cin + ci0 + c4), *(const f32x4*)(bn_tab + 5 * p.Cin + ci0 + c4));
+        return ((pk >> (ST_KH + kh)) & 1) ? o : (f32x4){0.f, 0.f, 0.f, 0.f};
+    };
     auto store_a = [&](const Stage& S, int ms) {
-        if constexpr (BNIN) {
+        if constexpr (STEM) {
+            const int kh = ms / n_ci, ci0 = (ms - kh * n_ci) * 32;
+#pragma unroll
+            for (int j = 0; j < PA; ++j) put_a(stem_relu(S.ra[j], stem_word(a_pk[j]), kh, ci0), a_lds[j]);
+            if (tid < 16) put_a(stem_relu(S.rh, stem_word(h_pk), kh, ci0), h_lds);
+        } else if constexpr (BNIN) {
             const int kh = ms / n_ci, ci0 = (ms - kh * n_ci) * 32;
             const bool okh = h_ok && (unsigned)(h_oh + kh - 1) < (unsigned)H;
             if (!bn_two) {
@@ -787,6 +850,11 @@
     conv_x3_s1_body<BM, BN, true, NP, BDB>(p);
 }
 
+template <int BM, int BN>
+__global__ __launch_bounds__(256) __attribute__((amdgpu_waves_per_eu(3, 3))) void conv_x3_s1_stem_kernel(X3Args p) {
+    conv_x3_s1_body<BM, BN, false, 2, true, true>(p);
+}
+
 __global__ void x3_stats_finalize_kernel(const float* __restrict__ ws, int C, int M, int R, int BM, float eps,
                                          float* __restrict__ mean, float* __restrict__ rstd) {
     const int c = blockIdx.x * blockDim.x + threadIdx.x;
@@ -1030,6 +1098,7 @@
     X3Args p;
     p.bn_ws = bn_ws; p.bn_gamma = bn_gamma; p.bn_beta = bn_beta; p.bn_eps = bn_eps;
     p.bn_max_tiles = bn_ws ? mft_x3_max_group_tiles(rows_per_group, 128) : 0;
+    p.st_idx = nullptr; p.st_mean = nullptr; p.st_m2 = nullptr; p.st_rows_per_img = 0; p.st_ipg = 0;
     if (bn_ws != nullptr && (in3 != nullptr || !bn_gamma || !bn_beta || rows_per_group < 128 || KH != 3 || KW != 3 || stride != 1 ||
                              pad != 1 || x3_s1_lds(128, 64, W, Cin, np) > X3_S1_LDS_3PER_CU ||
                              2 * mft_x3_stage_bytes_host(p.bn_max_tiles, Cin) >
@@ -1211,6 +1280,42 @@
                            stats_ws, mean, rstd, stream);
 }
 
+extern "C" int mft_conv2d_nhwc_h2_stem_bnstats(const float* psel, const int* src_idx, const float* mean_img, const float* m2_img,
+                                               int rows_per_img, int imgs_per_group, const float* gamma, const float* beta, float eps,
+                                               const unsigned short* w2, long long plane_elems, float* out, int ldo, int n_img, int H,
+                                               int W, int Cin, int Cout, float* stats_ws, void* stream) {
+    if (!psel || !src_idx || !mean_img || !m2_img || !gamma || !beta || !w2 || !out || !stats_ws || n_img <= 0 || H <= 0 || W <= 0 ||
+        rows_per_img <= 0 || imgs_per_group <= 0 || n_img % imgs_per_group != 0 || Cin != 64 || Cout % 64 != 0 || ldo % 4 != 0)
+        return MFT_EINVAL;
+    if (!g_x3_s1 || !g_x3_bdb || g_x3_tile > 1 || g_x3_db || g_x3_pp || g_x3_dbg || g_x3_hoist || g_x3_row_swz == 2 || g_x3_min_lds_kb ||
+        g_x3_patch)
+        return MFT_EINVAL;
+    const long long M = (long long)n_img * H * W, R = (long long)imgs_per_group * H * W;
+    if (M > 0x7fffffffLL || R < 128 || H * W < 128 || (long long)H * W * Cin > 0xfffffLL || 2 * plane_elems * 2 >= 0x7fff0000LL) return MFT_EINVAL;
+    const size_t lds = x3_s1_lds(128, 64, W, 0, 2) + (size_t)6 * Cin * sizeof(float);
+    if (lds > X3_S1_LDS_3PER_CU || (size_t)2 * 2 * imgs_per_group * Cin * sizeof(float) > (size_t)2 * (128 + 18) * X3_RS * sizeof(unsigned short))
+        return MFT_EINVAL;
+    X3Args p;
+    p.in = psel; p.w3 = w2; p.plane = plane_elems; p.out = out; p.ldi = Cin; p.ldo = ldo;
+    p.H = H; p.W = W; p.Cin = Cin; p.OH = H; p.OW = W; p.Cout = Cout; p.KH = 3; p.KW = 3; p.stride = 1; p.pad = 1;
+    p.Kpad = 9 * Cin;
+    p.M = (int)M;
+    p.tiles_n = Cout / 64;
+    p.in_bytes = 0;
+    p.w_bytes = (unsigned)(2 * plane_elems * 2);
+    p.xcd_swizzle = g_x3_xcd;
+    p.row_swz = g_x3_row_swz != 0;
+    p.in3 = nullptr; p.in_plane_bytes = 0;
+    p.stats_ws = stats_ws;
+    p.rows_per_group = (int)R;
+    p.s1_rows = 128 + 18;
+    p.bn_ws = nullptr; p.bn_gamma = gamma; p.bn_beta = beta; p.bn_eps = eps; p.bn_max_tiles = 0;
+    p.st_idx = src_idx; p.st_mean = mean_img; p.st_m2 = m2_img; p.st_rows_per_img = rows_per_img; p.st_ipg = imgs_per_group;
+    const int tiles_m = (p.M + 127) / 128;
+    hipLaunchKernelGGL((conv_x3_s1_stem_kernel<128, 64>), dim3((unsigned)(tiles_m * p.tiles_n)), dim3(256), lds, (hipStream_t)stream, p);
+    return mft_launch_status();
+}
+
 extern "C" int mft_conv2d_nhwc_x3p_bnstats(const unsigned short* in_planes, long long in_plane_elems, int ldi,
                                            const unsigned short* w3, long long plane_elems, float* out, int ldo, int n_img,
                                            int H, int W, int Cin, int Cout, int KH, int KW, int stride, int pad,
diff --git a/meta-fine-tuning_amd/csrc/stem.hip b/meta-fine-tuning_amd/csrc/stem.hip
--- a/meta-fine-tuning_amd/csrc/stem.hip
+++ b/meta-fine-tuning_amd/csrc/stem.hip
@@ -1,4 +1,5 @@
 #include "mft_common.h"
+#include "bn_fold.h"
 
 namespace {
 
@@ -143,11 +144,11 @@
 }
 
 
-template <int W_>
+template <int W_, bool SEL>
 __global__ __launch_bounds__(256) __attribute__((amdgpu_waves_per_eu(2, 2))) void stem_cache_kernel(const float* __restrict__ in, const float* __restrict__ w_pk,
                                                          float* __restrict__ pmax, float* __restrict__ pmin,
                                                          float* __restrict__ mean_img, float* __restrict__ m2_img, int w_ld,
-                                                         int n_img) {
+                                                         int n_img, const float* __restrict__ sel_gamma) {
     constexpr int H_ = W_;
     constexpr int OW = W_ / 2, OH = H_ / 2;
     constexpr int PH = (OH + 2 - 3) / 2 + 1, PW = (OW + 2 - 3) / 2 + 1;
@@ -281,8 +282,15 @@
                     }
                 }
                 const long long o = ((img * PH + i) * PW + j) * 64 + c4;
-                *(f32x4*)(pmax + o) = hi;
-                *(f32x4*)(pmin + o) = lo;
+                if constexpr (SEL) {
+                    const f32x4 ga = *(const f32x4*)(sel_gamma + c4);
+#pragma unroll
+                    for (int e = 0; e < 4; ++e) hi[e] = pooled_takes_max(ga[e]) ? hi[e] : lo[e];
+                    *(f32x4*)(pmax + o) = hi;
+                } else {
+                    *(f32x4*)(pmax + o) = hi;
+                    *(f32x4*)(pmin + o) = lo;
+                }
             }
             if (t == 0) sh = *(const f32x4*)(S + cq * 4);
             const int p0 = TPX * t;
@@ -329,21 +337,37 @@
     return MFT_EINVAL;
 }
 
-extern "C" int mft_stem_cache_fill(const float* in, const float* w, int w_ld, int n_img, int H, int W, float* pmax, float* pmin,
-                                   float* mean_img, float* m2_img, void* stream) {
+static int stem_cache_fill(const float* in, const float* w, int w_ld, int n_img, int H, int W, float* pmax, float* pmin,
+                           const float* sel_gamma, float* mean_img, float* m2_img, void* stream) {
     if (H != 84 || W != 84 || n_img <= 0 || w_ld < 147) return MFT_EINVAL;
     constexpr int W_ = 84, PL = (W_ + 8) * 3, PR = 11, SROW = (W_ / 2) * 64;
     const size_t lds = (2ull * PR * PL + 5ull * SROW) * sizeof(float);
-    auto kern = stem_cache_kernel<W_>;
     static MftPerDeviceOnce attr_once;
     if (attr_once.need()) {
-        hipError_t e = hipFuncSetAttribute((const void*)kern, hipFuncAttributeMaxDynamicSharedMemorySize, (int)lds);
+        hipError_t e = hipFuncSetAttribute((const void*)stem_cache_kernel<W_, false>, hipFuncAttributeMaxDynamicSharedMemorySize, (int)lds);
+        if (e == hipSuccess)
+            e = hipFuncSetAttribute((const void*)stem_cache_kernel<W_, true>, hipFuncAttributeMaxDynamicSharedMemorySize, (int)lds);
         if (e != hipSuccess) return (int)e;
         attr_once.mark();
     }
     long long grid = 256LL * 2;
     if (grid > n_img) grid = n_img;
-    hipLaunchKernelGGL(kern, dim3((unsigned)grid), dim3(256), lds, (hipStream_t)stream, in, w, pmax, pmin, mean_img, m2_img, w_ld,
-                       n_img);
+    if (sel_gamma)
+        hipLaunchKernelGGL((stem_cache_kernel<W_, true>), dim3((unsigned)grid), dim3(256), lds, (hipStream_t)stream, in, w, pmax, pmin, mean_img,
+                           m2_img, w_ld, n_img, sel_gamma);
+    else
+        hipLaunchKernelGGL((stem_cache_kernel<W_, false>), dim3((unsigned)grid), dim3(256), lds, (hipStream_t)stream, in, w, pmax, pmin, mean_img,
+                           m2_img, w_ld, n_img, sel_gamma);
     return mft_launch_status();
 }
+
+extern "C" int mft_stem_cache_fill(const float* in, const float* w, int w_ld, int n_img, int H, int W, float* pmax, float* pmin,
+                                   float* mean_img, float* m2_img, void* stream) {
+    return stem_cache_fill(in, w, w_ld, n_img, H, W, pmax, pmin, nullptr, mean_img, m2_img, stream);
+}
+
+extern "C" int mft_stem_cache_fill_select(const float* in, const float* w, int w_ld, int n_img, int H, int W, const float* gamma,
+                                          float* psel, float* mean_img, float* m2_img, void* stream) {
+    if (!gamma || !psel) return MFT_EINVAL;
+    return stem_cache_fill(in, w, w_ld, n_img, H, W, psel, nullptr, gamma, mean_img, m2_img, stream);
+}
diff --git a/meta-fine-tuning_amd/engine.py b/meta-fine-tuning_amd/engine.py
--- a/meta-fine-tuning_amd/engine.py
+++ b/meta-fine-tuning_amd/engine.py
@@ -343,11 +343,13 @@
         self.y_support = (np.tile(ya, n_views + 1) if self.views else ya).astype(np.int32)
         if stem_cache:
             pooled_pref = False if Fn.X3_PLANES else None
-            need = Fn.StemCache.bytes_needed(self.E * self.n_total, image_size, pooled=pooled_pref)
+            need = Fn.StemCache.bytes_needed(self.E * self.n_total, image_size, pooled=pooled_pref, single=settings.current().stem_fold)
             total = torch.cuda.get_device_properties(self.dev).total_memory
             stem_cache = need <= 0.35 * total
         self._stem_pooled = False if Fn.X3_PLANES else None
-        self.stem = Fn.StemCache(self.W, self.E * self.n_total, image_size, self.dev, pooled=self._stem_pooled) if stem_cache else None
+        self._stem_single = settings.current().stem_fold
+        self.stem = (Fn.StemCache(self.W, self.E * self.n_total, image_size, self.dev, pooled=self._stem_pooled, single=self._stem_single)
+                     if stem_cache else None)
         self.fuse_next = fuse_next_policy(self._fuse_next_setting, self.E, self.stem is not None, image_size, self.W.f16x2)
 
     @_on_device
@@ -671,7 +673,8 @@
             if need > 0.8 * free:
                 return
             self._pre_bufs = {"Xs": torch.empty_like(self.Xs),
-                              "stem": Fn.StemCache(self.W, self.E * self.n_total, self.size, self.dev, pooled=self._stem_pooled),
+                              "stem": Fn.StemCache(self.W, self.E * self.n_total, self.size, self.dev, pooled=self._stem_pooled,
+                                                   single=self._stem_single),
                               "stream": torch.cuda.Stream(device=self.dev)}
         b = self._pre_bufs
         sp = b["stream"]
diff --git a/meta-fine-tuning_amd/functional.py b/meta-fine-tuning_amd/functional.py
--- a/meta-fine-tuning_amd/functional.py
+++ b/meta-fine-tuning_amd/functional.py
@@ -243,7 +243,7 @@
 
 class StemCache:
 
-    def __init__(self, W, n_slots, H, device, chunk=8192, pooled=None):
+    def __init__(self, W, n_slots, H, device, chunk=8192, pooled=None, single=False):
         self.W = W
         self.n_slots = n_slots
         self.OH = (H + 6 - 7) // 2 + 1
@@ -255,26 +255,33 @@
         self.mean = torch.empty((n_slots, 64), device=device)
         self.m2 = torch.empty((n_slots, 64), device=device)
         self.fused_fill = bool(self.pooled and cfg.stem_fused_fill and H == 84)
+        self.single = bool(single) and self.pooled
+        self.psel = None
         if self.pooled:
             self.c0 = None
             self._buf = None if self.fused_fill else torch.empty((self.chunk, self.OH, self.OH, 64), device=device)
-            self.pmax = torch.empty((n_slots, self.PH, self.PH, 64), device=device)
-            self.pmin = torch.empty((n_slots, self.PH, self.PH, 64), device=device)
+            if self.single:
+                self.psel = torch.empty((n_slots, self.PH, self.PH, 64), device=device)
+                self.pmax = self.pmin = self.psel
+            else:
+                self.pmax = torch.empty((n_slots, self.PH, self.PH, 64), device=device)
+                self.pmin = torch.empty((n_slots, self.PH, self.PH, 64), device=device)
         else:
             self.c0 = torch.empty((n_slots, self.OH, self.OH, 64), device=device)
 
     def nbytes(self):
-        ts = [self.mean, self.m2] + ([self._buf, self.pmax, self.pmin] if self.pooled else [self.c0])
+        ts = [self.mean, self.m2] + (([self._buf, self.psel] if self.single else [self._buf, self.pmax, self.pmin]) if self.pooled
+                                     else [self.c0])
         return sum(t.numel() * 4 for t in ts if t is not None)
 
     @staticmethod
-    def bytes_needed(n_slots, H, pooled=None, chunk=8192):
+    def bytes_needed(n_slots, H, pooled=None, chunk=8192, single=False):
         cfg = settings.current()
         pooled = cfg.stem_pooled if pooled is None else bool(pooled)
         chunk = min(chunk if cfg.stem_chunk is None else cfg.stem_chunk, n_slots)
         oh = (H + 6 - 7) // 2 + 1
         ph = (oh + 2 - 3) // 2 + 1
-        per = 2 * 64 + (2 * ph * ph * 64 if pooled else oh * oh * 64)
+        per = 2 * 64 + ((1 if single else 2) * ph * ph * 64 if pooled else oh * oh * 64)
         fused = bool(pooled and cfg.stem_fused_fill and H == 84)
         return 4 * (n_slots * per + (chunk * oh * oh * 64 if (pooled and not fused) else 0))
 
@@ -284,10 +291,15 @@
         assert n == self.n_slots
         if self.fused_fill:
             wpk = self.W.conv["trunk.0"]
-            rc = lib.mft_stem_cache_fill(ops._p(x_nhwc), ops._p(wpk), wpk.shape[-1], n, x_nhwc.shape[1], x_nhwc.shape[2],
-                                         ops._p(self.pmax), ops._p(self.pmin), ops._p(self.mean), ops._p(self.m2), ops._stream())
+            if self.single:
+                rc = lib.mft_stem_cache_fill_select(ops._p(x_nhwc), ops._p(wpk), wpk.shape[-1], n, x_nhwc.shape[1], x_nhwc.shape[2],
+                                                    ops._p(self.W.bn["trunk.1"][0]), ops._p(self.psel), ops._p(self.mean),
+                                                    ops._p(self.m2), ops._stream())
+            else:
+                rc = lib.mft_stem_cache_fill(ops._p(x_nhwc), ops._p(wpk), wpk.shape[-1], n, x_nhwc.shape[1], x_nhwc.shape[2],
+                                             ops._p(self.pmax), ops._p(self.pmin), ops._p(self.mean), ops._p(self.m2), ops._stream())
             if rc != ops._lib.MFT_EINVAL:
-                ops._lib.check(rc, "mft_stem_cache_fill")
+                ops._lib.check(rc, "mft_stem_cache_fill_select" if self.single else "mft_stem_cache_fill")
                 return
             self.fused_fill = False
             self._buf = torch.empty((self.chunk, self.OH, self.OH, 64), device=x_nhwc.device)
@@ -298,7 +310,10 @@
             ops._lib.check(lib.mft_bn_image_moments(ops._p(c0), 64, 64, self.OH * self.OH, j - i,
                                                     ops._p(self.mean[i:j]), ops._p(self.m2[i:j]), ops._stream()),
                            "mft_bn_image_moments")
-            if self.pooled:
+            if self.single:
+                ops._lib.check(lib.mft_pool_window_select(ops._p(c0), ops._p(self.W.bn["trunk.1"][0]), ops._p(self.psel[i:j]), j - i,
+                                                          self.OH, self.OH, 64, ops._stream()), "mft_pool_window_select")
+            elif self.pooled:
                 ops._lib.check(lib.mft_pool_window_minmax(ops._p(c0), ops._p(self.pmax[i:j]), ops._p(self.pmin[i:j]), j - i,
                                                           self.OH, self.OH, 64, ops._stream()), "mft_pool_window_minmax")
 
@@ -356,7 +371,14 @@
                 _, ap = r
                 OHb = (shape[1] + 2 - 3) // stride + 1
                 shape = (n, OHb, OHb, cout)
-        if fold:
+        a, first = None, 4
+        if (fold and cache.single and upto > 4 and X3_FUSED_STATS and ipg * PH * PH >= 128 and W.f16x2
+                and all(("trunk.4" + nm) in W.planes("trunk.4", ipg, PH) for nm in (".C1", ".C2"))):
+            a = _frozen_block_folded(W, "trunk.4", None, arena, ipg, 64, 64, 1, tag + ".trunk.4", stem=(cache, idx))
+            first = 5 if a is not None else 4
+        if a is not None:
+            pass
+        elif fold:
             a = cache.gather_moments(idx, n, g, b, ipg, arena.get(tag + ".p0", (n, PH, PH, 64)))
         else:
             a = cache.gather(idx, n, m, s, g, b, ipg, arena.get(tag + ".p0", (n, PH, PH, 64)))
@@ -366,11 +388,14 @@
         c0 = ops.conv2d(x, W.conv["trunk.0"], 64, 7, 7, 2, 3, out=arena.get(tag + ".c0", (n, (x.shape[1] + 6 - 7) // 2 + 1, (x.shape[2] + 6 - 7) // 2 + 1, 64)))
         m, s = _bn_stats4(arena, tag + ".bn0", c0, ipg, groups, run("trunk.1"), fix("trunk.1"))
         a = ops.bn_relu_maxpool(c0, m, s, g, b, imgs_per_group=ipg)
-    for idx in (4, 5, 6, 7):
-        if idx >= upto:
+        first = 4
+    for bi in (4, 5, 6, 7):
+        if bi >= upto:
             break
-        cin, cout, stride = STAGES[idx]
-        p = "trunk.%d" % idx
+        if bi < first:
+            continue
+        cin, cout, stride = STAGES[bi]
+        p = "trunk.%d" % bi
         a = simple_block(W, p, a, arena, ipg, cin, cout, stride, running, tag + "." + p, fixed=fixed)
     return a
 
@@ -537,8 +562,15 @@
 _X3WS_FITS = {}
 
 
-def _frozen_block_folded(W, p, x, arena, ipg, cin, cout, stride, tag):
-    n, H, _, _ = x.shape
+def _frozen_block_folded(W, p, x, arena, ipg, cin, cout, stride, tag, stem=None):
+    if stem is not None:
+        cache, sidx = stem
+        assert x is None and cin == cout and stride == 1 and cache.single
+        n, H = sidx.numel(), cache.PH
+        sg, sb = W.bn["trunk.1"]
+        srows = cache.OH * cache.OH
+    else:
+        n, H, _, _ = x.shape
     groups = n // ipg
     OH = (H + 2 - 3) // stride + 1
     rows = ipg * OH * OH
@@ -557,9 +589,14 @@
         return None if r is None else ws
 
     c1 = arena.get(tag + ".c1", (n, OH, OH, cout))
-    ws1 = partials(".C1", x, 3, stride, 1, c1, tag + ".bn1")
-    if ws1 is None:
-        return None
+    if stem is not None:
+        ws1 = arena.get(tag + ".bn1.statws", (int(lib.mft_conv2d_x3_stats_ws_floats(n, H, H, cout, 3, 3, 1, 1)),))
+        if ops.conv2d_h2_stem_bnstats(cache.psel, sidx, cache.mean, cache.m2, srows, ipg, sg, sb, w3[p + ".C1"], cout, c1, ws1) is None:
+            return None
+    else:
+        ws1 = partials(".C1", x, 3, stride, 1, c1, tag + ".bn1")
+        if ws1 is None:
+            return None
     c2 = arena.get(tag + ".c2", (n, OH, OH, cout))
     ws2 = arena.get(tag + ".bn2.statws", (int(lib.mft_conv2d_x3_stats_ws_floats(n, OH, OH, cout, 3, 3, 1, 1)),))
     if ops.conv2d_x3_bnin_bnstats(c1, ws1, g1, b1, w3[p + ".C2"], cout, ipg, c2, ws2) is None:
@@ -576,6 +613,11 @@
             raise RuntimeError("frozen block %s: shortcut outside the bf16x3 domain after C1 was inside it" % p)
         ops.bn_apply_x3ws(c2.view(-1, cout), cout, rows, groups, ws2, g2, b2, out, act=ops.ACT_RELU, res=sc.view(-1, cout),
                           res_ws=wss, res_gamma=gs, res_beta=bs)
+    elif stem is not None:
+        if ops.bn_apply_x3ws_stemres(c2.view(-1, cout), cout, ws2, g2, b2, out, cache.psel, sidx, cache.mean, cache.m2, srows, ipg,
+                                     sg, sb, act=ops.ACT_RELU) is None:
+            x = cache.gather_moments(sidx, n, sg, sb, ipg, arena.get(tag + ".p0", (n, H, H, cin)))
+            ops.bn_apply_x3ws(c2.view(-1, cout), cout, rows, groups, ws2, g2, b2, out, act=ops.ACT_RELU, res=x.view(-1, cin))
     else:
         ops.bn_apply_x3ws(c2.view(-1, cout), cout, rows, groups, ws2, g2, b2, out, act=ops.ACT_RELU, res=x.view(-1, cin))
     return out.view(n, OH, OH, cout)
diff --git a/meta-fine-tuning_amd/ops.py b/meta-fine-tuning_amd/ops.py
--- a/meta-fine-tuning_amd/ops.py
+++ b/meta-fine-tuning_amd/ops.py
@@ -277,6 +277,35 @@
                                       _p(beta), _p(res), 0 if res is None else res.shape[-1], _p(res_ws), _p(res_gamma),
                                       _p(res_beta), act, slope, eps, _p(m), _p(r), _p(rm), _p(rr), _stream())
     _lib.check(rc, "mft_bn_apply_x3ws")
+    return out
+
+
+def conv2d_h2_stem_bnstats(psel, idx, mean_img, m2_img, rows_per_img, imgs_per_group, gamma, beta, w2, Cout, out, ws, eps=BN_EPS):
+    _f32c(psel)
+    _, H, W, Cin = psel.shape
+    if int(w2.shape[0]) != 2:
+        return None
+    rc = _lib.lib().mft_conv2d_nhwc_h2_stem_bnstats(_p(psel), _p(idx), _p(mean_img), _p(m2_img), rows_per_img, imgs_per_group, _p(gamma),
+                                                    _p(beta), eps, _p(w2), w2.shape[1] * w2.shape[2], _p(out), Cout, idx.numel(), H, W,
+                                                    Cin, Cout, _p(ws), _stream())
+    if rc == _lib.MFT_EINVAL:
+        return None
+    _lib.check(rc, "mft_conv2d_nhwc_h2_stem_bnstats")
+    return out
+
+
+def bn_apply_x3ws_stemres(x2d, C, ws, gamma, beta, out, psel, idx, mean_img, m2_img, rows_per_img, imgs_per_group, res_gamma, res_beta,
+                          act=ACT_NONE, slope=LRELU_SLOPE, eps=BN_EPS, stats=None, res_stats=None):
+    _f32c(x2d)
+    m, r = stats if stats is not None else (None, None)
+    rm, rr = res_stats if res_stats is not None else (None, None)
+    rc = _lib.lib().mft_bn_apply_x3ws_stemres(_p(x2d), x2d.shape[-1], _p(out), out.shape[-1], C, idx.numel(), psel.shape[1] * psel.shape[2],
+                                              imgs_per_group, _p(ws), _p(gamma), _p(beta), _p(psel), _p(idx), _p(mean_img), _p(m2_img),
+                                              rows_per_img, _p(res_gamma), _p(res_beta), act, slope, eps, _p(m), _p(r), _p(rm), _p(rr),
+                                              _stream())
+    if rc == _lib.MFT_EINVAL:
+        return None
+    _lib.check(rc, "mft_bn_apply_x3ws_stemres")
     return out
 
 
diff --git a/meta-fine-tuning_amd/settings.py b/meta-fine-tuning_amd/settings.py
--- a/meta-fine-tuning_amd/settings.py
+++ b/meta-fine-tuning_amd/settings.py
@@ -44,6 +44,7 @@
     ("stem_pooled", "MFT_STEM_POOLED", _flag, True, "stem cache keeps per-window (max, min) instead of the full-resolution output"),
     ("stem_fused_fill", "MFT_STEM_FUSED_FILL", _flag, True, "stem cache filled by ONE launch (convolution + moments + window min/max; 0: three launches through a full-resolution buffer)"),
     ("stem_chunk", "MFT_STEM_CHUNK", _opt_int, None, "images per stem-cache fill launch (None: StemCache's default)"),
+    ("stem_fold", "MFT_STEM_FOLD", _flag, True, "engine's stem cache keeps ONE value per window (the extremum trunk.1's frozen gamma selects) and trunk.4 reads it directly (0: (max, min) pair + gather launch)"),
     ("fused_last_block", "MFT_FUSED_LAST_BLOCK", _flag, True, "conv + BatchNorm fusions of the adapted block (csrc/skinny.hip)"),
     ("small_groups", "MFT_SMALL_GROUPS", int, 12, "up to this many per-episode weight sets take the K-sliced GEMM route"),
     ("fused_pair_mlp", "MFT_FUSED_PAIR_MLP", _flag, True, "Wcompute on the fused upper-triangle pair-MLP kernels"),
@@ -93,6 +94,7 @@
     stem_pooled: bool = True
     stem_fused_fill: bool = True
     stem_chunk: "int | None" = None
+    stem_fold: bool = True
     fused_last_block: bool = True
     small_groups: int = 12
     fused_pair_mlp: bool = True
```
